# zoongahn/jodalroB-twoTower

Measured on AMD Instinct MI355X. Metric: training pairs/sec at batch 8192 (embedding-lookup HBM GB/s in roofline), higher is better.
Workload: dtype bf16 MFMA operands, f32 accumulate; f32 tables, master weights and activations (the tower input x, which the GEMMs round to bf16 anyway, is stored bf16)

## Files before the change

### include/twotower.h

```cpp
#ifndef TWOTOWER_H_
#define TWOTOWER_H_

#include <stddef.h>
#include <stdint.h>

#ifdef __cplusplus
extern "C" {
#endif

#define TT_ABI_VERSION 2

#define TT_OK 0
#define TT_ERR_INVALID_ARG (-1)
#define TT_ERR_HIP (-2)
#define TT_ERR_WORKSPACE (-3)
#define TT_ERR_UNSUPPORTED (-4)
#define TT_ERR_DEVICE (-5)

#define TT_F32 0
#define TT_BF16 1

#define TT_MAX_SIDES 4
#define TT_MAX_HIDDEN 8

typedef struct tt_ctx tt_ctx;
typedef void* tt_stream;

int tt_abi_version(void);
int tt_ctx_create(int device, tt_ctx** out);
int tt_ctx_destroy(tt_ctx* ctx);
const char* tt_last_error_string(void);
int tt_ctx_num_cus(const tt_ctx* ctx);
uint64_t tt_launch_count(void);

#define TT_OPT_DEFER_SLAB_REDUCE 1
#define TT_OPT_KEYED_PARTS 2
#define TT_OPT_SCORE_BWD_ROWS_MIN 3
#define TT_OPT_DEFER_RIDERS 4
#define TT_OPT_FP8_GRAD 5
#define TT_OPT_CHAINED 6
#define TT_OPT_LOOKUP_NT 7
#define TT_OPT_CHAIN_SPIN 8
#define TT_OPT_RETRIEVE_SPLITS 9
int tt_ctx_set_option(tt_ctx* ctx, int32_t option, int32_t value);
#define TT_DEVERR_CHAIN_TIMEOUT 1u
#define TT_DEVERR_ROW_RANGE 2u
int tt_ctx_check_device_errors(tt_ctx* ctx, tt_stream stream);
int tt_handover_retarget(tt_ctx* ctx, void* graph_exec, void* node);
int tt_handover_captured_node(tt_ctx* ctx, void** node);
int tt_flush_deferred(tt_ctx* ctx, tt_stream stream);
int tt_flush_deferred_slabs(tt_ctx* ctx, tt_stream stream);
int tt_deferred_pending(const tt_ctx* ctx);

typedef struct tt_embed_side {
  const int64_t* ids;
  const int64_t* key_row_offset;
  const int64_t* key_vocab;
  void* out;
  int64_t ld_out;
  int32_t K;
  int32_t out_dtype;
} tt_embed_side;

int tt_embed_lookup_set_profile(tt_ctx* ctx, uint64_t* ring_dev, int32_t n_slots);
int tt_embed_lookup_fwd(tt_ctx* ctx, const float* table, int64_t table_rows, int32_t E,
                        const tt_embed_side* sides, int32_t n_sides, int64_t B, int32_t* rows_out,
                        tt_stream stream);
int tt_embed_lookup_rows_fwd(tt_ctx* ctx, const float* table, int64_t table_rows, int32_t E,
                             const tt_embed_side* sides, int32_t n_sides, int64_t B, const int32_t* rows,
                             tt_stream stream);

size_t tt_dedup_workspace_bytes(int64_t M);
int tt_dedup_plan(tt_ctx* ctx, const int32_t* rows, int64_t M, int64_t table_rows,
                  int32_t* sorted_src, int32_t* unique_rows, int32_t* seg_offsets, int32_t* n_unique,
                  void* workspace, size_t workspace_bytes, tt_stream stream);

size_t tt_dedup_keyed_workspace_bytes(int64_t M, int32_t n_keys);
int tt_dedup_plan_keyed(tt_ctx* ctx, const int32_t* rows, const int32_t* side_K ,
                        int32_t n_sides, int64_t B, int32_t* sorted_src, int32_t* unique_rows,
                        int32_t* seg_offsets, int32_t* n_unique, void* workspace, size_t workspace_bytes,
                        tt_stream stream);

int tt_dedup_plan_keyed_km(tt_ctx* ctx, const int32_t* rows_km, const int32_t* side_K ,
                           int32_t n_sides, int64_t B, int32_t* sorted_src, int32_t* unique_rows,
                           int32_t* seg_offsets, int32_t* n_unique, void* workspace, size_t workspace_bytes,
                           tt_stream stream);

int tt_dedup_plan_keyed_long(tt_ctx* ctx, const int32_t* rows, int32_t rows_key_major, const int32_t* side_K ,
                             int32_t n_sides, int64_t B, int32_t E, int32_t* sorted_src, int32_t* unique_rows,
                             int32_t* seg_offsets, int32_t* n_unique, void* grad_workspace, size_t grad_workspace_bytes,
                             void* workspace, size_t workspace_bytes, tt_stream stream);

#define TT_GRAD_SPARSE 0
#define TT_GRAD_DENSE_SET 1
#define TT_GRAD_DENSE_ACC 2
#define TT_GRAD_SHORT_SEGMENTS 0x100
#define TT_GRAD_PLANNED 0x200
#define TT_GRAD_DEFER_FINISH 0x400

typedef struct tt_grad_src {
  const void* d_out;
  int64_t ld;
  int32_t K;
  int32_t dtype;
} tt_grad_src;

size_t tt_embed_grad_workspace_bytes(int64_t M, int32_t E);
int tt_embed_grad_bwd(tt_ctx* ctx, const tt_grad_src* srcs, int32_t n_srcs, int64_t B, int32_t E,
                      const int32_t* sorted_src, const int32_t* seg_offsets,
                      const int32_t* unique_rows, const int32_t* n_unique, int64_t M, int32_t mode,
                      float* out, int32_t* counters, void* workspace, size_t workspace_bytes, tt_stream stream);

void tt_adam_hparams(int64_t step, float lr, float beta1, float beta2, float eps, float weight_decay,
                     float out6[6]);
int tt_adam_dense_step(tt_ctx* ctx, float* p, const float* g, float* m, float* v, int64_t n,
                       int64_t step, float lr, float beta1, float beta2, float eps,
                       float weight_decay, const float* hparams_dev, tt_stream stream);
typedef struct tt_adam_tensor {
  float* p;
  const float* g;
  float* m;
  float* v;
  int64_t n;
} tt_adam_tensor;
int tt_adam_multi_step(tt_ctx* ctx, const tt_adam_tensor* tensors , int32_t n_tensors,
                       int64_t step, float lr, float beta1, float beta2, float eps,
                       float weight_decay, const float* hparams_dev, tt_stream stream);
int tt_sparse_adam_step(tt_ctx* ctx, float* table, float* m, float* v, int64_t table_rows, int32_t E,
                        const int32_t* unique_rows, const float* grad_rows, const int32_t* n_unique,
                        int64_t M, int64_t step, float lr, float beta1, float beta2, float eps,
                        float weight_decay, const float* hparams_dev, tt_stream stream);

int tt_adam_fused_step(tt_ctx* ctx, const tt_adam_tensor* tensors, int32_t n_tensors, float* table, float* m, float* v,
                       int64_t table_rows, int32_t E, const int32_t* unique_rows, const float* grad_rows, const int32_t* n_unique, int64_t M,
                       int64_t step, float lr, float beta1, float beta2, float eps, float weight_decay,
                       const float* hparams_dev, tt_stream stream);

int tt_adam_fused_step_finish(tt_ctx* ctx, const tt_adam_tensor* tensors, int32_t n_tensors, float* table, float* m, float* v,
                              int64_t table_rows, int32_t E, const int32_t* unique_rows, float* grad_rows, const int32_t* n_unique,
                              int64_t M, const int32_t* seg_offsets, void* grad_workspace, size_t grad_workspace_bytes,
                              int64_t step, float lr, float beta1, float beta2, float eps, float weight_decay,
                              const float* hparams_dev, tt_stream stream);

int tt_rowwise_adagrad_sparse_step(tt_ctx* ctx, float* table, float* sum, int64_t table_rows, int32_t E,
                                   const int32_t* unique_rows, const float* grad_rows, const int32_t* n_unique, int64_t M,
                                   float lr, float eps, float weight_decay, const float* hparams_dev, tt_stream stream);
int tt_rowwise_adagrad_dense_step(tt_ctx* ctx, float* table, float* sum, const float* grad, int64_t table_rows, int32_t E,
                                  float lr, float eps, float weight_decay, const float* hparams_dev, tt_stream stream);
int tt_adam_rowwise_adagrad_fused_step(tt_ctx* ctx, const tt_adam_tensor* tensors, int32_t n_tensors, int64_t step, float lr,
                                       float beta1, float beta2, float eps, float weight_decay, const float* hparams_dev,
                                       float* table, float* sum, int64_t table_rows, int32_t E, const int32_t* unique_rows,
                                       const float* grad_rows, const int32_t* n_unique, int64_t M, float table_lr,
                                       float table_eps, float table_weight_decay, const float* table_hparams_dev,
                                       tt_stream stream);
int tt_adam_rowwise_adagrad_fused_step_finish(tt_ctx* ctx, const tt_adam_tensor* tensors, int32_t n_tensors, int64_t step,
                                              float lr, float beta1, float beta2, float eps, float weight_decay,
                                              const float* hparams_dev, float* table, float* sum, int64_t table_rows, int32_t E,
                                              const int32_t* unique_rows, float* grad_rows, const int32_t* n_unique, int64_t M,
                                              const int32_t* seg_offsets, void* grad_workspace, size_t grad_workspace_bytes,
                                              float table_lr, float table_eps, float table_weight_decay,
                                              const float* table_hparams_dev, tt_stream stream);
int tt_embed_grad_finish(tt_ctx* ctx, int32_t E, const int32_t* seg_offsets, int64_t M, float* out, void* workspace,
                         size_t workspace_bytes, tt_stream stream);

typedef struct tt_tower_params {
  int32_t din, h0, kcat_e, n_hidden, d_out;
  int32_t hidden[TT_MAX_HIDDEN];
  const float* w_proj;
  const float* b_proj;
  const float* w[TT_MAX_HIDDEN];
  const float* b[TT_MAX_HIDDEN];
  const float* bn_w[TT_MAX_HIDDEN];
  const float* bn_b[TT_MAX_HIDDEN];
  float* bn_rm[TT_MAX_HIDDEN];
  float* bn_rv[TT_MAX_HIDDEN];
  int64_t* bn_nbt[TT_MAX_HIDDEN];
  const float* w_out;
  const float* b_out;
  int32_t compute_dtype;
  int32_t x_dtype;
  int32_t dx_dtype;
  int32_t flags;
  int32_t sync_phase;
  int32_t sync_ranks;
  int64_t rng_row_offset;
  const void* w_proj_bf16;
  const void* w_bf16[TT_MAX_HIDDEN];
} tt_tower_params;
#define TT_TOWER_UNFUSED_TAIL 1
#define TT_TOWER_UNFUSED_FRONT 2
#define TT_TOWER_UNFUSED_BACK 4

typedef struct tt_tower_acts {
  const float* dense;
  void* x;
  float* pre[TT_MAX_HIDDEN];
  float* act[TT_MAX_HIDDEN];
  float* mean[TT_MAX_HIDDEN];
  float* rstd[TT_MAX_HIDDEN];
  float* y;
  float* emb;
  void* emb_packed;
  float emb_pack_scale;
  float* bn_sync_local;
  const float* bn_sync_all;
  int64_t bn_sync_stride;
} tt_tower_acts;

typedef struct tt_tower_grads {
  float* w_proj;
  float* b_proj;
  float* w[TT_MAX_HIDDEN];
  float* b[TT_MAX_HIDDEN];
  float* bn_w[TT_MAX_HIDDEN];
  float* bn_b[TT_MAX_HIDDEN];
  float* w_out;
  float* b_out;
  void* d_x;
  float* scratch[TT_MAX_HIDDEN];
  float* d_y;
  float* s_sync_local;
  const float* s_sync_all;
  int64_t s_sync_stride;
} tt_tower_grads;

size_t tt_tower_workspace_bytes(const tt_tower_params* p, int64_t B);
int tt_tower_mlp_fwd(tt_ctx* ctx, const tt_tower_params* p, const tt_tower_acts* a, int64_t B,
                     int32_t train, float dropout_p, uint64_t seed, const uint64_t* seed_dev,
                     void* workspace, size_t workspace_bytes, tt_stream stream);
int tt_tower_mlp_bwd(tt_ctx* ctx, const tt_tower_params* p, const tt_tower_acts* a,
                     const float* d_emb, const tt_tower_grads* g, int64_t B, int32_t train,
                     float dropout_p, uint64_t seed, const uint64_t* seed_dev, void* workspace,
                     size_t workspace_bytes, tt_stream stream);

int tt_towers_mlp_fwd(tt_ctx* ctx, int32_t n, const tt_tower_params* const* p, const tt_tower_acts* const* a,
                      int64_t B, int32_t train, float dropout_p, uint64_t seed, const uint64_t* seed_dev,
                      void* const* workspaces, const size_t* workspace_bytes, tt_stream stream);
int tt_towers_mlp_bwd(tt_ctx* ctx, int32_t n, const tt_tower_params* const* p, const tt_tower_acts* const* a,
                      const float* const* d_emb, const tt_tower_grads* const* g, int64_t B, int32_t train,
                      float dropout_p, uint64_t seed, const uint64_t* seed_dev, void* const* workspaces,
                      const size_t* workspace_bytes, tt_stream stream);

int tt_score_dir_fwd(tt_ctx* ctx, const float* A, const float* Bm, int64_t Ra, int64_t Rb, int32_t D,
                     float inv_t, float shift, int64_t diag_offset, float* sumexp, float* diag,
                     int32_t* rank, float* sumscore ,
                     tt_stream stream);
int tt_score_loss_finish(tt_ctx* ctx, int64_t B, float shift, const float* rowsum,
                         const float* colsum, const float* diag, const int32_t* row_rank,
                         const int32_t* col_rank, const float* sumscore, float* out8,
                         float* loss_out , tt_stream stream);
int tt_score_dir_bwd(tt_ctx* ctx, const float* A, const float* Bm, int64_t Ra, int64_t Rb, int32_t D,
                     float inv_t, float shift, int64_t diag_offset, const float* sumexp_a,
                     const float* sumexp_b, const float* d_loss, float scale, float* dA,
                     tt_stream stream);
typedef struct tt_score_fwd_dir {
  const void* A_packed;
  const void* B_packed;
  int64_t Ra, Rb, diag_offset;
  float* sumexp;
  float* diag;
  int32_t* rank;
  float* sumscore;
  int32_t rank_mode;
  float ab_scale;
  float* inv_sumexp;
} tt_score_fwd_dir;
typedef struct tt_score_bwd_dir {
  const void* A_packed;
  const void* B_packed;
  int64_t Ra, Rb, diag_offset;
  const float* sumexp_a;
  const float* sumexp_b;
  float* dA;
  float ab_scale;
  float b_scale;
  const float* inv_a;
  const float* inv_b;
} tt_score_bwd_dir;
size_t tt_score_pack_bytes(int64_t R, int32_t D);
float tt_score_unit_scale(float inv_t);
int tt_score_pack_bf16(tt_ctx* ctx, const float* X, int64_t R, int32_t D, float scale, void* packed, tt_stream stream);
int tt_score_pack2_bf16(tt_ctx* ctx, const float* X0, int64_t R0, void* packed0, const float* X1, int64_t R1,
                        void* packed1, int32_t D, float scale0, float scale1, tt_stream stream);
int tt_score_fwd_bf16(tt_ctx* ctx, const tt_score_fwd_dir* dirs, int32_t n_dirs, int32_t D, float inv_t,
                      float shift, tt_stream stream);
int tt_score_bwd_bf16(tt_ctx* ctx, const tt_score_bwd_dir* dirs, int32_t n_dirs, int32_t D, float inv_t,
                      float shift, const float* d_loss, float scale, tt_stream stream);
size_t tt_score_fwd_sym_workspace_bytes(int64_t B, int32_t D);
int tt_score_fwd_sym_bf16(tt_ctx* ctx, const void* N_packed, const void* C_packed, int64_t B, int32_t D, float inv_t,
                          float shift, float ab_scale, int32_t want_rank, float* rowsum, float* colsum, float* inv_row,
                          float* inv_col, float* diag, int32_t* row_rank, float* out8, float* loss_out, void* workspace,
                          size_t workspace_bytes, tt_stream stream);
size_t tt_score_pack_fp8_bytes(int64_t R, int32_t D);
int tt_score_pack2_fp8(tt_ctx* ctx, const float* X0, int64_t R0, void* packed0, const float* X1, int64_t R1,
                       void* packed1, int32_t D, float scale0, float scale1, tt_stream stream);
// ... 118 lines not shown
```

### jodalrob-twotower_amd/_lib.py

```python
from __future__ import annotations

import ctypes as C
from pathlib import Path
from typing import Optional

import torch

_PKG = Path(__file__).resolve().parent
LIB_PATH = _PKG / "libtwotower_hip.so"

TT_F32, TT_BF16 = 0, 1
TT_MAX_SIDES, TT_MAX_HIDDEN = 4, 8
TT_GRAD_SPARSE, TT_GRAD_DENSE_SET, TT_GRAD_DENSE_ACC = 0, 1, 2
TT_TOWER_UNFUSED_TAIL = 1
TT_TOWER_UNFUSED_FRONT = 2
TT_TOWER_UNFUSED_BACK = 4
TT_GRAD_SHORT_SEGMENTS = 0x100
TT_GRAD_PLANNED = 0x200
TT_GRAD_DEFER_FINISH = 0x400

vp = C.c_void_p
i32, i64, f32, u64, sz = C.c_int32, C.c_int64, C.c_float, C.c_uint64, C.c_size_t


class EmbedSide(C.Structure):
    _fields_ = [("ids", vp), ("key_row_offset", vp), ("key_vocab", vp), ("out", vp), ("ld_out", i64),
                ("K", i32), ("out_dtype", i32)]


class StoreSide(C.Structure):
    _fields_ = [("entity", vp), ("entity_stride", i64), ("dense_store", vp), ("cat_store", vp), ("dense_out", vp), ("ids_out", vp),
                ("dense_dim", i32), ("n_rows", i32)]


TT_MAX_CVT = 8


class CvtList(C.Structure):
    _fields_ = [("n", i32), ("reserved", i32), ("src", vp * TT_MAX_CVT), ("dst", vp * TT_MAX_CVT), ("count", i64 * TT_MAX_CVT)]


class IngestLookup(C.Structure):
    _fields_ = [("table", vp), ("table_rows", i64), ("E", i32), ("reserved", i32)]


class GradSrc(C.Structure):
    _fields_ = [("d_out", vp), ("ld", i64), ("K", i32), ("dtype", i32)]


class AdamTensor(C.Structure):
    _fields_ = [("p", vp), ("g", vp), ("m", vp), ("v", vp), ("n", i64)]


class ScoreFwdDir(C.Structure):
    _fields_ = [("A_packed", vp), ("B_packed", vp), ("Ra", i64), ("Rb", i64), ("diag_offset", i64),
                ("sumexp", vp), ("diag", vp), ("rank", vp), ("sumscore", vp), ("rank_mode", i32), ("ab_scale", f32), ("inv_sumexp", vp)]


class ScoreBwdDir(C.Structure):
    _fields_ = [("A_packed", vp), ("B_packed", vp), ("Ra", i64), ("Rb", i64), ("diag_offset", i64),
                ("sumexp_a", vp), ("sumexp_b", vp), ("dA", vp), ("ab_scale", f32), ("b_scale", f32), ("inv_a", vp), ("inv_b", vp)]


_H = vp * TT_MAX_HIDDEN


class TowerParams(C.Structure):
    _fields_ = [("din", i32), ("h0", i32), ("kcat_e", i32), ("n_hidden", i32), ("d_out", i32),
                ("hidden", i32 * TT_MAX_HIDDEN),
                ("w_proj", vp), ("b_proj", vp), ("w", _H), ("b", _H), ("bn_w", _H), ("bn_b", _H),
                ("bn_rm", _H), ("bn_rv", _H), ("bn_nbt", _H), ("w_out", vp), ("b_out", vp), ("compute_dtype", i32),
                ("x_dtype", i32), ("dx_dtype", i32), ("flags", i32),
                ("sync_phase", i32), ("sync_ranks", i32), ("rng_row_offset", i64),
                ("w_proj_bf16", vp), ("w_bf16", _H)]


class TowerActs(C.Structure):
    _fields_ = [("dense", vp), ("x", vp), ("pre", _H), ("act", _H), ("mean", _H), ("rstd", _H), ("y", vp), ("emb", vp), ("emb_packed", vp), ("emb_pack_scale", f32),
                ("bn_sync_local", vp), ("bn_sync_all", vp), ("bn_sync_stride", i64)]


class TowerGrads(C.Structure):
    _fields_ = [("w_proj", vp), ("b_proj", vp), ("w", _H), ("b", _H), ("bn_w", _H), ("bn_b", _H),
                ("w_out", vp), ("b_out", vp), ("d_x", vp), ("scratch", _H), ("d_y", vp), ("s_sync_local", vp), ("s_sync_all", vp), ("s_sync_stride", i64)]


SIGNATURES = {
    "tt_abi_version": (C.c_int, []),
    "tt_ctx_create": (C.c_int, [C.c_int, C.POINTER(vp)]),
    "tt_ctx_destroy": (C.c_int, [vp]),
    "tt_last_error_string": (C.c_char_p, []),
    "tt_ctx_num_cus": (C.c_int, [vp]),
    "tt_embed_lookup_set_profile": (C.c_int, [vp, vp, i32]),
    "tt_embed_lookup_fwd": (C.c_int, [vp, vp, i64, i32, C.POINTER(EmbedSide), i32, i64, vp, vp]),
    "tt_embed_lookup_rows_fwd": (C.c_int, [vp, vp, i64, i32, C.POINTER(EmbedSide), i32, i64, vp, vp]),
    "tt_dedup_workspace_bytes": (sz, [i64]),
    "tt_dedup_plan": (C.c_int, [vp, vp, i64, i64, vp, vp, vp, vp, vp, sz, vp]),
    "tt_dedup_keyed_workspace_bytes": (sz, [i64, i32]),
    "tt_dedup_plan_keyed": (C.c_int, [vp, vp, C.POINTER(i32), i32, i64, vp, vp, vp, vp, vp, sz, vp]),
    "tt_dedup_plan_keyed_km": (C.c_int, [vp, vp, C.POINTER(i32), i32, i64, vp, vp, vp, vp, vp, sz, vp]),
    "tt_dedup_plan_keyed_long": (C.c_int, [vp, vp, i32, C.POINTER(i32), i32, i64, i32, vp, vp, vp, vp, vp, sz, vp, sz, vp]),
    "tt_embed_grad_workspace_bytes": (sz, [i64, i32]),
    "tt_embed_grad_bwd": (C.c_int, [vp, C.POINTER(GradSrc), i32, i64, i32, vp, vp, vp, vp, i64, i32, vp, vp, vp, sz, vp]),
    "tt_adam_hparams": (None, [i64, f32, f32, f32, f32, f32, C.POINTER(f32 * 6)]),
    "tt_adam_dense_step": (C.c_int, [vp, vp, vp, vp, vp, i64, i64, f32, f32, f32, f32, f32, vp, vp]),
    "tt_adam_multi_step": (C.c_int, [vp, C.POINTER(AdamTensor), i32, i64, f32, f32, f32, f32, f32, vp, vp]),
    "tt_sparse_adam_step": (C.c_int, [vp, vp, vp, vp, i64, i32, vp, vp, vp, i64, i64, f32, f32, f32, f32, f32, vp, vp]),
    "tt_adam_fused_step": (C.c_int, [vp, C.POINTER(AdamTensor), i32, vp, vp, vp, i64, i32, vp, vp, vp, i64, i64, f32, f32, f32, f32,
                                     f32, vp, vp]),
    "tt_adam_fused_step_finish": (C.c_int, [vp, C.POINTER(AdamTensor), i32, vp, vp, vp, i64, i32, vp, vp, vp, i64, vp, vp, sz, i64, f32,
                                            f32, f32, f32, f32, vp, vp]),
    "tt_rowwise_adagrad_sparse_step": (C.c_int, [vp, vp, vp, i64, i32, vp, vp, vp, i64, f32, f32, f32, vp, vp]),
    "tt_rowwise_adagrad_dense_step": (C.c_int, [vp, vp, vp, vp, i64, i32, f32, f32, f32, vp, vp]),
    "tt_adam_rowwise_adagrad_fused_step": (C.c_int, [vp, C.POINTER(AdamTensor), i32, i64, f32, f32, f32, f32, f32, vp, vp, vp, i64, i32,
                                                     vp, vp, vp, i64, f32, f32, f32, vp, vp]),
    "tt_adam_rowwise_adagrad_fused_step_finish": (C.c_int, [vp, C.POINTER(AdamTensor), i32, i64, f32, f32, f32, f32, f32, vp, vp, vp,
                                                            i64, i32, vp, vp, vp, i64, vp, vp, sz, f32, f32, f32, vp, vp]),
    "tt_embed_grad_finish": (C.c_int, [vp, i32, vp, i64, vp, vp, sz, vp]),
    "tt_ctx_set_option": (C.c_int, [vp, i32, i32]),
    "tt_flush_deferred": (C.c_int, [vp, vp]),
    "tt_ctx_check_device_errors": (C.c_int, [vp, vp]),
    "tt_handover_retarget": (C.c_int, [vp, vp, vp]),
    "tt_handover_captured_node": (C.c_int, [vp, C.POINTER(vp)]),
    "tt_deferred_pending": (C.c_int, [vp]),
    "tt_launch_count": (C.c_uint64, []),
    "tt_flush_deferred_slabs": (C.c_int, [vp, vp]),
    "tt_tower_workspace_bytes": (sz, [C.POINTER(TowerParams), i64]),
    "tt_tower_mlp_fwd": (C.c_int, [vp, C.POINTER(TowerParams), C.POINTER(TowerActs), i64, i32, f32, u64, vp, vp, sz, vp]),
    "tt_tower_mlp_bwd": (C.c_int, [vp, C.POINTER(TowerParams), C.POINTER(TowerActs), vp, C.POINTER(TowerGrads), i64, i32,
                                   f32, u64, vp, vp, sz, vp]),
    "tt_towers_mlp_fwd": (C.c_int, [vp, i32, C.POINTER(C.POINTER(TowerParams)), C.POINTER(C.POINTER(TowerActs)), i64, i32, f32, u64,
                                    vp, C.POINTER(vp), C.POINTER(sz), vp]),
    "tt_towers_mlp_bwd": (C.c_int, [vp, i32, C.POINTER(C.POINTER(TowerParams)), C.POINTER(C.POINTER(TowerActs)), C.POINTER(vp),
                                    C.POINTER(C.POINTER(TowerGrads)), i64, i32, f32, u64, vp, C.POINTER(vp), C.POINTER(sz), vp]),
    "tt_score_dir_fwd": (C.c_int, [vp, vp, vp, i64, i64, i32, f32, f32, i64, vp, vp, vp, vp, vp]),
    "tt_score_loss_finish": (C.c_int, [vp, i64, f32, vp, vp, vp, vp, vp, vp, vp, vp, vp]),
    "tt_score_dir_bwd": (C.c_int, [vp, vp, vp, i64, i64, i32, f32, f32, i64, vp, vp, vp, f32, vp, vp]),
    "tt_score_pack_bytes": (sz, [i64, i32]),
    "tt_score_unit_scale": (f32, [f32]),
    "tt_score_pack_bf16": (C.c_int, [vp, vp, i64, i32, f32, vp, vp]),
    "tt_score_pack2_bf16": (C.c_int, [vp, vp, i64, vp, vp, i64, vp, i32, f32, f32, vp]),
    "tt_score_fwd_bf16": (C.c_int, [vp, C.POINTER(ScoreFwdDir), i32, i32, f32, f32, vp]),
    "tt_score_bwd_bf16": (C.c_int, [vp, C.POINTER(ScoreBwdDir), i32, i32, f32, f32, vp, f32, vp]),
    "tt_score_pack_fp8_bytes": (sz, [i64, i32]),
    "tt_score_pack2_fp8": (C.c_int, [vp, vp, i64, vp, vp, i64, vp, i32, f32, f32, vp]),
    "tt_score_fwd_sym_fp8": (C.c_int, [vp, vp, vp, i64, i32, f32, f32, f32, i32, vp, vp, vp, vp, vp, vp, vp, vp, vp, sz, vp]),
    "tt_score_bwd_fp8": (C.c_int, [vp, C.POINTER(ScoreBwdDir), i32, i32, f32, f32, vp, f32, vp]),
    "tt_score_fwd_sym_workspace_bytes": (sz, [i64, i32]),
    "tt_score_fwd_sym_bf16": (C.c_int, [vp, vp, vp, i64, i32, f32, f32, f32, i32, vp, vp, vp, vp, vp, vp, vp, vp, vp, sz, vp]),
    "tt_score_pack_x3_bytes": (sz, [i64, i32]),
    "tt_score_pack2_bf16x3": (C.c_int, [vp, vp, i64, vp, vp, i64, vp, i32, f32, f32, vp]),
    "tt_score_fwd_sym_bf16x3": (C.c_int, [vp, vp, vp, i64, i32, f32, f32, f32, i32, vp, vp, vp, vp, vp, vp, vp, vp, vp, sz, vp]),
    "tt_score_fwd_bf16x3": (C.c_int, [vp, C.POINTER(ScoreFwdDir), i32, i32, f32, f32, vp]),
    "tt_score_bwd_bf16x3": (C.c_int, [vp, C.POINTER(ScoreBwdDir), i32, i32, f32, f32, vp, f32, vp]),
    "tt_score_matrix": (C.c_int, [vp, vp, vp, i64, i64, i32, f32, vp, i64, vp]),
    "tt_score_dense_workspace_bytes": (sz, [i64, i32]),
    "tt_score_dense_fwd": (C.c_int, [vp, vp, vp, i64, i32, f32, i32, f32, vp, vp, vp, vp, vp, vp]),
    "tt_score_dense_bwd": (C.c_int, [vp, vp, vp, i64, i32, f32, i32, f32, vp, vp, vp, vp, vp, vp, sz, vp]),
    "tt_diag_rank_rows": (C.c_int, [vp, vp, i64, i64, i64, i64, vp, vp]),
    "tt_topk_rows": (C.c_int, [vp, vp, i64, i64, i64, i32, vp, vp, vp]),
    "tt_retrieve_workspace_bytes": (sz, [i64, i64, i32, i32]),
    "tt_retrieve_topk_bf16": (C.c_int, [vp, vp, i64, vp, i64, i32, i32, vp, i32, vp, vp, vp, vp, sz, vp]),
    "tt_retrieve_topk_f32": (C.c_int, [vp, vp, i64, vp, i64, i32, f32, i32, vp, i32, vp, vp, vp, vp, sz, vp]),
    "tt_linear_fwd": (C.c_int, [vp, vp, i64, vp, vp, vp, i64, i64, i32, i32, i32, vp]),
    "tt_route_workspace_bytes": (sz, [i64, i32]),
    "tt_route_bucket": (C.c_int, [vp, vp, vp, i64, i32, i32, C.POINTER(i32), i32, vp, vp, vp, vp, vp, vp, sz, vp]),
    "tt_route_expand": (C.c_int, [vp, vp, vp, vp, vp, i64, vp, vp]),
    "tt_route_bucket_expand": (C.c_int, [vp, vp, vp, i64, i32, i32, C.POINTER(i32), i32, vp, vp, vp, vp, vp, vp, sz, vp, vp, vp, vp]),
    "tt_dedup_plan_runs": (C.c_int, [vp, vp, i32, i64, i64, vp, vp, vp, vp, vp, sz, vp]),
    "tt_gather_rows": (C.c_int, [vp, vp, i64, i32, vp, i64, vp, i32, vp]),
    "tt_copy_multi": (C.c_int, [vp, i32, C.POINTER(vp), C.POINTER(vp), C.POINTER(i64), vp]),
    "tt_batch_ingest": (C.c_int, [vp, i32, C.POINTER(vp), C.POINTER(vp), C.POINTER(i64), C.POINTER(EmbedSide), i32, i64, vp, vp, i64, C.POINTER(CvtList), vp]),
    "tt_batch_gather": (C.c_int, [vp, vp, i64, vp, i32, vp, i32, vp, vp, vp]),
    "tt_batch_ingest_store": (C.c_int, [vp, i32, C.POINTER(vp), C.POINTER(vp), C.POINTER(i64), C.POINTER(EmbedSide), C.POINTER(StoreSide), i32,
                                        i64, vp, vp, vp, i64, C.POINTER(CvtList), vp]),
    "tt_batch_ingest_lookup": (C.c_int, [vp, i32, C.POINTER(vp), C.POINTER(vp), C.POINTER(i64), C.POINTER(EmbedSide), i32, i64, vp,
                                         C.POINTER(IngestLookup), C.POINTER(CvtList), vp]),
    "tt_batch_ingest_store_lookup": (C.c_int, [vp, i32, C.POINTER(vp), C.POINTER(vp), C.POINTER(i64), C.POINTER(EmbedSide), C.POINTER(StoreSide),
                                               i32, i64, vp, vp, C.POINTER(IngestLookup), C.POINTER(CvtList), vp]),
}

_lib: Optional[C.CDLL] = None
_ctxs: dict = {}
_defer_on: set = set()
_riders_on: dict = {}
_workspaces: dict = {}


class TwoTowerHipError(RuntimeError):
    pass


def load() -> C.CDLL:
    global _lib
    if _lib is None:
        if not LIB_PATH.exists():
            raise TwoTowerHipError(
                f"{LIB_PATH} is missing: build it with `python -c 'import __graft_entry__ as g; g.build()'` "
                "(hipcc --offload-arch=gfx950).  There is no CPU fallback for the two-tower hot path.")
        lib = C.CDLL(str(LIB_PATH))
        for name, (res, args) in SIGNATURES.items():
            fn = getattr(lib, name)
            fn.restype, fn.argtypes = res, args
        _lib = lib
    return _lib


def check(rc: int, what: str = ""):
    if rc != 0:
        msg = load().tt_last_error_string().decode("utf-8", "replace")
        raise TwoTowerHipError(f"{what or 'twotower call'} failed (status {rc}): {msg}")


def ctx(device: torch.device) -> vp:
    device = torch.device(device)
    if device.type != "cuda":
        raise TwoTowerHipError(f"the two-tower hot path runs on MI355X only; got tensors on '{device}' "
                               "(no CPU fallback exists)")
    idx = device.index if device.index is not None else torch.cuda.current_device()
    if idx not in _ctxs:
        h = vp()
        check(load().tt_ctx_create(idx, C.byref(h)), "tt_ctx_create")
        _ctxs[idx] = h
    return _ctxs[idx]


def stream(device: torch.device) -> vp:
    return vp(torch.cuda.current_stream(device).cuda_stream)


def ptr(t: Optional[torch.Tensor]) -> vp:
    return vp(0 if t is None else t.data_ptr())


TT_OPT_DEFER_SLAB_REDUCE = 1
TT_OPT_KEYED_PARTS = 2
TT_OPT_SCORE_BWD_ROWS_MIN = 3
TT_OPT_DEFER_RIDERS = 4
TT_OPT_FP8_GRAD = 5
TT_OPT_CHAINED = 6
TT_OPT_LOOKUP_NT = 7
TT_OPT_CHAIN_SPIN = 8
TT_OPT_RETRIEVE_SPLITS = 9


def set_option(device: torch.device, option: int, value: int):
    check(load().tt_ctx_set_option(ctx(device), int(option), int(value)), "tt_ctx_set_option")


def set_defer_slab_reduce(device: torch.device, on: bool):
    check(load().tt_ctx_set_option(ctx(device), TT_OPT_DEFER_SLAB_REDUCE, 1 if on else 0), "tt_ctx_set_option")
    idx = torch.device(device).index
    (_defer_on.add if on else _defer_on.discard)(idx if idx is not None else torch.cuda.current_device())
    if not on:
        flush_deferred(device)


def set_defer_riders(device: torch.device, on, loss_only: bool = False):
    mask = (2 if loss_only else 3) if on else 0
    check(load().tt_ctx_set_option(ctx(device), TT_OPT_DEFER_RIDERS, mask), "tt_ctx_set_option")
    idx = torch.device(device).index
    idx = idx if idx is not None else torch.cuda.current_device()
    if mask:
        _riders_on[idx] = mask
    else:
        _riders_on.pop(idx, None)
        flush_deferred(device)


def riders_deferred(device: torch.device, which: int = 3) -> bool:
    idx = torch.device(device).index
    return bool(_riders_on.get(idx if idx is not None else torch.cuda.current_device(), 0) & which)


def check_device_errors(device: torch.device):
    device = torch.device(device)
    idx = device.index if device.index is not None else (torch.cuda.current_device() if device.type == "cuda" else None)
    if device.type != "cuda" or idx not in _ctxs:
        return
    check(load().tt_ctx_check_device_errors(_ctxs[idx], stream(device)), "tt_ctx_check_device_errors")


def handover_captured_node(device: torch.device) -> Optional[int]:
    h = vp()
    check(load().tt_handover_captured_node(ctx(device), C.byref(h)), "tt_handover_captured_node")
    return h.value


class handover_retarget:

    def __init__(self, device: torch.device, graph_exec: int, node: int):
        self.device, self.exec, self.node = device, graph_exec, node

    def __enter__(self):
        check(load().tt_handover_retarget(ctx(self.device), vp(self.exec), vp(self.node)), "tt_handover_retarget")
        return self

    def __exit__(self, *exc):
        check(load().tt_handover_retarget(ctx(self.device), vp(0), vp(0)), "tt_handover_retarget")
        return False


def flush_deferred(device: torch.device):
    lib = load()
    c = ctx(device)
    if lib.tt_deferred_pending(c):
        check(lib.tt_flush_deferred(c, stream(device)), "tt_flush_deferred")


def workspace(device: torch.device, nbytes: int) -> torch.Tensor:
    if _defer_on:
        lib, c = load(), ctx(device)
        if lib.tt_deferred_pending(c) & 1:
            check(lib.tt_flush_deferred_slabs(c, stream(device)), "tt_flush_deferred_slabs")
    key = (torch.device(device).index, torch.cuda.current_stream(device).cuda_stream)
    buf = _workspaces.get(key)
    if buf is None or buf.numel() < nbytes:
        buf = torch.empty(max(int(nbytes), 1 << 20), dtype=torch.uint8, device=device)
        _workspaces[key] = buf
    return buf


def num_cus(device: torch.device) -> int:
    return int(load().tt_ctx_num_cus(ctx(device)))


def no_dynamo(fn):
    try:
        import torch._dynamo as _d
        return _d.disable(fn)
    except Exception:
        return fn
```

### jodalrob-twotower_amd/cat_embed.py

```python
from __future__ import annotations

from pathlib import Path
from typing import Dict, List, Optional, Union

import torch
from ._lib import no_dynamo as _no_dynamo
import torch.nn as nn

from . import ops
from .config import settings
from .schema import category_counts


class EmbeddingStore:

    def __init__(self, E: int, device, grad_mode: str = "dense"):
        if grad_mode not in ("dense", "sparse"):
            raise ValueError(f"embedding_grad must be 'dense' or 'sparse', got {grad_mode!r}")
        self.E = E
        self.device = torch.device(device)
        self.grad_mode = grad_mode
        self.weight: Optional[torch.Tensor] = None
        self.grad: Optional[torch.Tensor] = None
        self.sparse_grad = None
        self.defer_long_finish = False
        self.members: List["CategoricalEmbedder"] = []
        self.version = 0
        self._grad_counters = None
        self.ingest = None
        self.ingest_x_fresh = False

    def rows_km_for(self, id_tensors) -> Optional[torch.Tensor]:
        reg = self.ingest
        if reg is None or len(reg[0]) != len(id_tensors):
            return None
        for t, r, v in zip(id_tensors, reg[0], reg[1]):
            if t.data_ptr() != r.data_ptr() or t.numel() != r.numel() or r._version != v:
                return None
        return reg[2]

    def rows_sm_for(self, id_tensors) -> Optional[torch.Tensor]:
        reg = self.ingest
        if reg is None or len(reg) < 5 or reg[4] is None or self.rows_km_for(id_tensors) is None:
            return None
        return reg[4]

    def x_for(self, id_tensors, shapes) -> Optional[list]:
        reg = self.ingest
        if reg is None or len(reg) < 4 or reg[3] is None or not self.ingest_x_fresh or self.rows_km_for(id_tensors) is None:
            return None
        xs = reg[3]
        if len(xs) != len(shapes) or any(tuple(x.shape) != (b, w) or x.dtype != dt for x, (b, w, dt) in zip(xs, shapes)):
            return None
        self.ingest_x_fresh = False
        return xs

    def grad_counters(self) -> Optional[torch.Tensor]:
        if self._grad_counters is None or self._grad_counters.device != self.device:
            if self.device.type != "cuda" or torch.cuda.is_current_stream_capturing():
                return None
            self._grad_counters = torch.zeros(4, dtype=torch.int32, device=self.device)
        return self._grad_counters

    @property
    def rows(self) -> int:
        return 0 if self.weight is None else self.weight.shape[0]

    def append_rows(self, n: int) -> int:
        new = torch.empty((n, self.E), dtype=torch.float32, device=self.device)
        nn.init.normal_(new)
        base = self.rows
        self.weight = new if self.weight is None else torch.cat([self.weight, new])
        self.grad, self.sparse_grad = None, None
        self.version += 1
        return base

    def apply(self, fn):
        new = fn(self.weight)
        if new is not self.weight:
            if new.dtype != torch.float32:
                raise TypeError("embedding tables are kept in float32")
            self.weight = new
            self.device = new.device
            self.grad = None if self.grad is None else fn(self.grad)
            self.sparse_grad = None
            self.version += 1

    @staticmethod
    def fuse(stores: List["EmbeddingStore"]) -> "EmbeddingStore":
        uniq = []
        for s in stores:
            if all(s is not u for u in uniq):
                uniq.append(s)
        if len(uniq) == 1:
            return uniq[0]
        first = uniq[0]
        if any(s.E != first.E for s in uniq):
            raise ValueError("cannot fuse embedding stores of different embedding_dim")
        fused = EmbeddingStore(first.E, first.device, first.grad_mode)
        fused.weight = torch.cat([s.weight.to(first.device) for s in uniq])
        base = 0
        for s in uniq:
            for m in s.members:
                m._rebind(fused, m.row_base + base)
            base += s.rows
        return fused

    def optim_parameters(self):
        return [p for m in self.members for p in m.table_parameters()]

    def bind_grads(self):
        for m in self.members:
            m._bind_grads()

    def accumulate_grad(self, plan: ops.DedupPlan, srcs, B: int, short_segments: bool = False):
        if self.grad_mode == "sparse":
            grad_rows = torch.empty((max(plan.M, 1), self.E), dtype=torch.float32, device=self.device)
            ops.embed_grad(plan, srcs, B, self.E, ops.TT_GRAD_SPARSE, grad_rows, short_segments, self.grad_counters(),
                           defer_finish=self.defer_long_finish)
            self.sparse_grad = (plan, grad_rows)
            return
        params = self.optim_parameters()
        fresh = any(p.grad is None for p in params) or self.grad is None
        if self.grad is None:
            self.grad = torch.empty_like(self.weight)
        if fresh:
            self.grad.zero_()
            ops.embed_grad(plan, srcs, B, self.E, ops.TT_GRAD_DENSE_SET, self.grad, counters=self.grad_counters())
            self.bind_grads()
        else:
            ops.embed_grad(plan, srcs, B, self.E, ops.TT_GRAD_DENSE_ACC, self.grad, counters=self.grad_counters())


class _Table(nn.Module):

    def __init__(self, view: torch.Tensor):
        super().__init__()
        self.weight = nn.Parameter(view)

    @property
    def num_embeddings(self):
        return self.weight.shape[0]

    @property
    def embedding_dim(self):
        return self.weight.shape[1]


class CategoricalEmbedder(nn.Module):
    def __init__(self, keys: List[str], metadata_path: Union[str, Path], table_name: str, embedding_dim: int = 64,
                 device: Optional[str] = "cuda:0", safety_margin: int = 10, embedding_grad: Optional[str] = None,
                 materialize: bool = True):
        super().__init__()
        self.keys = list(keys)
        self.materialize = materialize
        self.embedding_dim = embedding_dim
        self.device_str = str(device or "cuda:0")
        self.safety_margin = safety_margin
        self.vocab_sizes = self._extract_vocab_sizes(metadata_path, table_name, self.keys)
        print(f"[CategoricalEmbedder] Initializing with {len(self.keys)} features")
        mode = embedding_grad or settings.embedding_grad
        self.store = EmbeddingStore(embedding_dim, torch.device(self.device_str), mode)
        self.embeddings = nn.ModuleDict()
        offs = []
        if materialize:
            self.row_base = self.store.append_rows(sum(self.vocab_sizes[k] for k in self.keys)) if self.keys else 0
            self.store.members.append(self)
            off = self.row_base
            for k in self.keys:
                v = self.vocab_sizes[k]
                self.embeddings[k] = _Table(self.store.weight[off:off + v])
                offs.append(off)
                off += v
        else:
            self.row_base, off = 0, 0
            for k in self.keys:
                offs.append(off)
                off += self.vocab_sizes[k]
        dev = self.store.device
        self.register_buffer("_key_row_offset", torch.tensor(offs, dtype=torch.int64, device=dev), persistent=False)
        self.register_buffer("_key_vocab", torch.tensor([self.vocab_sizes[k] for k in self.keys], dtype=torch.int64,
                                                        device=dev), persistent=False)
        self._bound_version = self.store.version

    def _extract_vocab_sizes(self, metadata_path, table_name: str, keys: List[str]) -> Dict[str, int]:
        try:
            counts = category_counts(table_name, metadata_path)
        except Exception as e:
            print(f"[ERROR] Failed to extract vocab_sizes from metadata: {e}")
            print("[FALLBACK] Using default vocab_size=1000 for all keys")
            return {k: 1000 for k in keys}
        out = {}
        for k in keys:
            if k not in counts:
                print(f"[WARNING] Column '{k}' not found in metadata, using default vocab_size=1000")
                out[k] = 1000
            elif counts[k] is None:
                print(f"[WARNING] No category count info for '{k}', using default vocab_size=1000")
                out[k] = 1000
            else:
                out[k] = int(counts[k]) + self.safety_margin
        return out

    def table_parameters(self):
        return [self.embeddings[k].weight for k in self.keys] if self.materialize else []

    @property
    def total_rows(self) -> int:
        return sum(self.vocab_sizes[k] for k in self.keys)

    def set_row_base(self, base: int):
        off, offs = base, []
        for k in self.keys:
            offs.append(off)
            off += self.vocab_sizes[k]
        self.row_base = base
        self._key_row_offset = torch.tensor(offs, dtype=torch.int64, device=self._key_row_offset.device)

    def _rebind(self, store: Optional[EmbeddingStore] = None, row_base: Optional[int] = None):
        if store is not None and store is not self.store:
            self.store = store
            if self not in store.members:
                store.members.append(self)
        if row_base is not None:
            self.row_base = row_base
        off = self.row_base
        offs = []
        for k in self.keys:
            v = self.vocab_sizes[k]
            self.embeddings[k].weight.data = self.store.weight[off:off + v]
            self.embeddings[k].weight.grad = None
            offs.append(off)
            off += v
        dev = self.store.device
        self._key_row_offset = torch.tensor(offs, dtype=torch.int64, device=dev)
        self._key_vocab = self._key_vocab.to(dev)
        self._bound_version = self.store.version
        if self.store.grad is not None:
            self._bind_grads()

    def _bind_grads(self):
        off = self.row_base
        for k in self.keys:
            v = self.vocab_sizes[k]
            self.embeddings[k].weight.grad = self.store.grad[off:off + v]
            off += v

    def _apply(self, fn, recurse=True):
        if not self.materialize:
            dev = fn(torch.empty(0, device=self._key_vocab.device)).device
            self._key_row_offset, self._key_vocab = self._key_row_offset.to(dev), self._key_vocab.to(dev)
            self.store.device = dev
            return self
        self.store.apply(fn)
        for s_member in self.store.members:
            if s_member._bound_version != s_member.store.version:
                s_member._rebind()
        self._key_row_offset = self._key_row_offset.to(self.store.device)
        self._key_vocab = self._key_vocab.to(self.store.device)
        return self

    def load_state_dict(self, state_dict, strict: bool = True, assign: bool = False):
        return super().load_state_dict(state_dict, strict=strict, assign=False)

    def lookup_side(self, values: torch.Tensor, out_view: torch.Tensor) -> ops.LookupSide:
        return ops.LookupSide(values, self._key_row_offset, self._key_vocab, out_view, len(self.keys))

    @_no_dynamo
    def forward(self, kjt, return_dict: bool = True):
        K, E = len(self.keys), self.embedding_dim
        if kjt is None:
            dev = self.store.device
# ... 39 lines not shown
```

### jodalrob-twotower_amd/csrc/tt_common.h

```cpp
#pragma once
#include <hip/hip_runtime.h>
#include <stdint.h>
#include <stdio.h>
#include <stdarg.h>
#include <atomic>

#include "twotower.h"

struct tt_ctx {
  int device;
  int num_cus;
  size_t lds_per_block;
  unsigned long long* lookup_stamps;
  int lookup_stamp_slots;
  int defer_slab_reduce;
  struct TnPending* deferred;
  int keyed_parts;
  int score_bwd_rows_min;
  int defer_riders;
  int fp8_grad;
  struct tt_riders* riders;
  uint32_t* chain;
  int chain_words;
  void* chain_stream[16];
  int chain_used;
  int chained;
  uint32_t* dev_err;
  int chain_spin;
  int retrieve_splits;
  int lookup_nt;
  void* ho_exec;
  void* ho_node;
  void* ho_last;
};

constexpr uint32_t kChainReady = 0x80000000u;
constexpr int kChainWords = 1 << 16, kChainSlices = 16;
uint32_t* tt_chain_for(tt_ctx* ctx, hipStream_t stream);

void tt_set_error(const char* fmt, ...);

#define TT_CHECK_ARG(cond, ...)         \
  do {                                  \
    if (!(cond)) {                      \
      tt_set_error(__VA_ARGS__);        \
      return TT_ERR_INVALID_ARG;        \
    }                                   \
  } while (0)

#define TT_HIP(expr)                                                                   \
  do {                                                                                 \
    hipError_t _e = (expr);                                                            \
    if (_e != hipSuccess) {                                                            \
      tt_set_error("%s failed: %s (%s:%d)", #expr, hipGetErrorString(_e), __FILE__, __LINE__); \
      return TT_ERR_HIP;                                                               \
    }                                                                                  \
  } while (0)

extern std::atomic<uint64_t> tt_launches;
#define TT_LAUNCH_CHECK()                                    \
  do {                                                       \
    tt_launches.fetch_add(1, std::memory_order_relaxed);     \
    TT_HIP(hipGetLastError());                               \
  } while (0)

#define TT_LDS_ONCE(bytes, ...)                                                                                     \
  do {                                                                                                              \
    static std::atomic<uint64_t> tt_lds_done{0};                                                                    \
    const uint64_t tt_bit = 1ull << (ctx->device & 63);                                                             \
    if (!(tt_lds_done.load(std::memory_order_acquire) & tt_bit)) {                                                  \
      TT_HIP(hipFuncSetAttribute(reinterpret_cast<const void*>(__VA_ARGS__), hipFuncAttributeMaxDynamicSharedMemorySize, (int)(bytes))); \
      tt_lds_done.fetch_or(tt_bit, std::memory_order_release);                                                      \
    }                                                                                                               \
  } while (0)

static inline int64_t tt_cdiv(int64_t a, int64_t b) { return (a + b - 1) / b; }
static inline bool tt_aligned(const void* p, size_t a) { return (reinterpret_cast<uintptr_t>(p) % a) == 0; }

__device__ __forceinline__ uint16_t tt_f2bf(float x) {
  __bf16 b = static_cast<__bf16>(x);
  return __builtin_bit_cast(uint16_t, b);
}
__device__ __forceinline__ float tt_bf2f(uint16_t h) {
  return __builtin_bit_cast(float, static_cast<uint32_t>(h) << 16);
}

__device__ __forceinline__ uint32_t tt_mix32(uint32_t x) {
  x ^= x >> 16;
  x *= 0x7feb352dU;
  x ^= x >> 15;
  x *= 0x846ca68bU;
  x ^= x >> 16;
  return x;
}
__device__ __forceinline__ float tt_uniform01(uint64_t seed, uint64_t idx) {
  const uint32_t lo = static_cast<uint32_t>(idx), hi = static_cast<uint32_t>(idx >> 32);
  const uint32_t h = tt_mix32(lo ^ static_cast<uint32_t>(seed) ^ ((hi ^ static_cast<uint32_t>(seed >> 32)) * 0x9E3779B9U));
  return static_cast<float>(h >> 8) * (1.0f / 16777216.0f);
}
```

### jodalrob-twotower_amd/csrc/tt_ctx.hip

```cpp
#include "tt_common.h"
#include "tt_gemm.h"
#include "tt_riders.h"

#include <mutex>

#include <string.h>

static thread_local char g_err[512] = "";
std::atomic<uint64_t> tt_launches{0};

namespace {
__global__ __launch_bounds__(kRiderThreads) void riders_kernel(tt_riders r) {
  if ((int)blockIdx.x < r.c_wg) compact_body(r.c, blockIdx.x);
  else finish2_body(r.f);
}
}

uint32_t* tt_chain_for(tt_ctx* ctx, hipStream_t stream) {
  static std::mutex mu;
  if (!ctx || !ctx->chained || !ctx->chain) return nullptr;
  std::lock_guard<std::mutex> lock(mu);
  for (int i = 0; i < ctx->chain_used; ++i)
    if (ctx->chain_stream[i] == static_cast<void*>(stream)) return ctx->chain + (size_t)i * kChainWords;
  if (ctx->chain_used == kChainSlices) return nullptr;
  ctx->chain_stream[ctx->chain_used] = static_cast<void*>(stream);
  return ctx->chain + (size_t)(ctx->chain_used++) * kChainWords;
}

int tt_riders_flush(tt_ctx* ctx, hipStream_t st) {
  if (!ctx || !ctx->riders || (ctx->riders->c_wg == 0 && ctx->riders->f_wg == 0)) return TT_OK;
  riders_kernel<<<ctx->riders->c_wg + ctx->riders->f_wg, kRiderThreads, 0, st>>>(*ctx->riders);
  ctx->riders->c_wg = ctx->riders->f_wg = 0;
  TT_LAUNCH_CHECK();
  return TT_OK;
}

void tt_set_error(const char* fmt, ...) {
  va_list ap;
  va_start(ap, fmt);
  vsnprintf(g_err, sizeof(g_err), fmt, ap);
  va_end(ap);
}

extern "C" {

int tt_abi_version(void) { return TT_ABI_VERSION; }

const char* tt_last_error_string(void) { return g_err; }

int tt_ctx_create(int device, tt_ctx** out) {
  TT_CHECK_ARG(out != nullptr, "tt_ctx_create: out is NULL");
  int n = 0;
  TT_HIP(hipGetDeviceCount(&n));
  TT_CHECK_ARG(device >= 0 && device < n, "tt_ctx_create: device %d out of range (%d devices)", device, n);
  hipDeviceProp_t prop;
  TT_HIP(hipGetDeviceProperties(&prop, device));
  if (strncmp(prop.gcnArchName, "gfx950", 6) != 0) {
    tt_set_error("tt_ctx_create: device %d is %s; this library is built for gfx950 (MI355X) only", device,
                 prop.gcnArchName);
    return TT_ERR_UNSUPPORTED;
  }
  tt_ctx* c = new tt_ctx();
  c->device = device;
  c->num_cus = prop.multiProcessorCount;
  c->lds_per_block = prop.sharedMemPerBlock;
  c->lookup_stamps = nullptr;
  c->lookup_stamp_slots = 0;
  c->defer_slab_reduce = 0;
  c->deferred = nullptr;
  c->keyed_parts = 0;
  c->score_bwd_rows_min = 32768;
  c->defer_riders = 0;
  c->fp8_grad = 1;
  c->riders = new tt_riders();
  c->riders->c_wg = c->riders->f_wg = 0;
  c->chain = nullptr;
  c->chain_words = 0;
  c->chain_used = 0;
  c->chained = 1;
  c->chain_spin = 1 << 22;
  c->retrieve_splits = 0;
  c->dev_err = nullptr;
  c->ho_exec = c->ho_node = c->ho_last = nullptr;
  {
    int prev = 0;
    TT_HIP(hipGetDevice(&prev));
    TT_HIP(hipSetDevice(device));
    hipError_t e = hipMalloc(reinterpret_cast<void**>(&c->chain), sizeof(uint32_t) * (kChainWords * kChainSlices + 64));
    if (e == hipSuccess) e = hipMemset(c->chain, 0, sizeof(uint32_t) * (kChainWords * kChainSlices + 64));
    if (e == hipSuccess) c->dev_err = c->chain + (size_t)kChainWords * kChainSlices;
    (void)hipSetDevice(prev);
    if (e != hipSuccess) {
      tt_set_error("tt_ctx_create: %s", hipGetErrorString(e));
      delete c->riders;
      delete c;
      return TT_ERR_HIP;
    }
    c->chain_words = kChainWords;
  }
  *out = c;
  return TT_OK;
}

int tt_ctx_destroy(tt_ctx* ctx) {
  if (ctx && ctx->deferred) tt_gemm_tn_pending_destroy(ctx->deferred);
  if (ctx) delete ctx->riders;
  if (ctx && ctx->chain) (void)hipFree(ctx->chain);
  delete ctx;
  return TT_OK;
}

int tt_ctx_set_option(tt_ctx* ctx, int32_t option, int32_t value) {
  TT_CHECK_ARG(ctx != nullptr, "tt_ctx_set_option: NULL context");
  switch (option) {
    case TT_OPT_DEFER_SLAB_REDUCE: ctx->defer_slab_reduce = value != 0; break;
    case TT_OPT_KEYED_PARTS:
      TT_CHECK_ARG(value >= 0, "tt_ctx_set_option: TT_OPT_KEYED_PARTS needs a value >= 0");
      ctx->keyed_parts = value;
      break;
    case TT_OPT_SCORE_BWD_ROWS_MIN:
      TT_CHECK_ARG(value >= 1, "tt_ctx_set_option: TT_OPT_SCORE_BWD_ROWS_MIN needs a value >= 1");
      ctx->score_bwd_rows_min = value;
      break;
    case TT_OPT_DEFER_RIDERS:
      TT_CHECK_ARG(value >= 0 && value <= 3, "tt_ctx_set_option: TT_OPT_DEFER_RIDERS takes 0 .. 3");
      ctx->defer_riders = value == 1 ? 3 : value;
      break;
    case TT_OPT_FP8_GRAD: ctx->fp8_grad = value != 0; break;
    case TT_OPT_CHAINED: ctx->chained = value != 0; break;
    case TT_OPT_LOOKUP_NT: ctx->lookup_nt = value != 0; break;
    case TT_OPT_CHAIN_SPIN:
      TT_CHECK_ARG(value >= 1, "tt_ctx_set_option: TT_OPT_CHAIN_SPIN needs a value >= 1");
      ctx->chain_spin = value;
      break;
    case TT_OPT_RETRIEVE_SPLITS:
      TT_CHECK_ARG(value >= 0, "tt_ctx_set_option: TT_OPT_RETRIEVE_SPLITS needs a value >= 0");
      ctx->retrieve_splits = value;
      break;
    default: tt_set_error("tt_ctx_set_option: unknown option %d", option); return TT_ERR_INVALID_ARG;
  }
  return TT_OK;
}

int tt_ctx_check_device_errors(tt_ctx* ctx, tt_stream stream) {
  TT_CHECK_ARG(ctx != nullptr, "tt_ctx_check_device_errors: NULL context");
  if (!ctx->dev_err) return TT_OK;
  hipStream_t st = reinterpret_cast<hipStream_t>(stream);
  uint32_t word = 0;
  TT_HIP(hipMemcpyAsync(&word, ctx->dev_err, sizeof(word), hipMemcpyDeviceToHost, st));
  TT_HIP(hipStreamSynchronize(st));
  if (word == 0) return TT_OK;
  TT_HIP(hipMemsetAsync(ctx->chain, 0, sizeof(uint32_t) * ((size_t)kChainWords * kChainSlices + 64), st));
  TT_HIP(hipStreamSynchronize(st));
  tt_set_error("device error word 0x%x:%s%s the steps since the last check are invalid (they must be rejected)", word,
               (word & TT_DEVERR_CHAIN_TIMEOUT) ? " a chained segment-head launch gave up waiting for a predecessor tile (tt_dedup_plan / tt_dedup_plan_runs);" : "",
               (word & TT_DEVERR_ROW_RANGE) ? " a lookup decoded rows outside its table (key offsets / vocabularies that belong to another table; tt_embed_lookup_fwd / "
                                              "tt_embed_lookup_rows_fwd / tt_batch_ingest_lookup) and read the last row instead;" : "");
  return TT_ERR_DEVICE;
}

int tt_handover_retarget(tt_ctx* ctx, void* graph_exec, void* node) {
  TT_CHECK_ARG(ctx != nullptr && ((graph_exec == nullptr) == (node == nullptr)), "tt_handover_retarget: NULL context / one of (graph_exec, node) NULL");
  ctx->ho_exec = graph_exec;
  ctx->ho_node = node;
  return TT_OK;
}

int tt_handover_captured_node(tt_ctx* ctx, void** node) {
  TT_CHECK_ARG(ctx != nullptr && node != nullptr, "tt_handover_captured_node: NULL argument");
  *node = ctx->ho_last;
  ctx->ho_last = nullptr;
  return TT_OK;
}

int tt_flush_deferred(tt_ctx* ctx, tt_stream stream) {
  TT_CHECK_ARG(ctx != nullptr, "tt_flush_deferred: NULL context");
  if (int rc = tt_riders_flush(ctx, reinterpret_cast<hipStream_t>(stream))) return rc;
  return tt_gemm_deferred_flush(ctx, reinterpret_cast<hipStream_t>(stream));
}

int tt_flush_deferred_slabs(tt_ctx* ctx, tt_stream stream) {
  TT_CHECK_ARG(ctx != nullptr, "tt_flush_deferred_slabs: NULL context");
  return tt_gemm_deferred_flush(ctx, reinterpret_cast<hipStream_t>(stream));
}

int tt_deferred_pending(const tt_ctx* ctx) {
  if (!ctx) return 0;
  return ((ctx->deferred && ctx->deferred->n > 0) ? 1 : 0) | ((ctx->riders && (ctx->riders->c_wg > 0 || ctx->riders->f_wg > 0)) ? 2 : 0);
}

int tt_ctx_num_cus(const tt_ctx* ctx) { return ctx ? ctx->num_cus : 0; }

uint64_t tt_launch_count(void) { return tt_launches.load(std::memory_order_relaxed); }

}
```

### jodalrob-twotower_amd/csrc/tt_embed.hip

```cpp
#include "tt_common.h"
#include "tt_gemm.h"
#include "tt_riders.h"

#include <stdlib.h>
#include <type_traits>

namespace {

constexpr int kThreads = 256;

struct SideDev {
  const int64_t* ids;
  const int64_t* off;
  const int64_t* vocab;
  char* out;
  int64_t ld;
  uint32_t slot_base;
  int32_t K;
  int32_t dtype;
  uint32_t magic;
};

struct SideSet {
  SideDev s[TT_MAX_SIDES];
// ... 670 lines not shown
    __syncthreads();
    for (int d = tid; d < 16 * 256; d += kKeyedThreads) (&peers_mask[0][0])[d] = 0ull;
    __syncthreads();
  }
  if (!sorted_by_buckets) {
    e_lo = 0;
    e_hi = part == 0 ? B : 0;
    if (part != 0) {
      if (tid == 0) { ucount[blockIdx.x] = 0; ubase[blockIdx.x] = ki * B; uend[blockIdx.x] = ki * B; }
      return;
    }
  }
  for (int p = 0; p < (sorted_by_buckets ? 0 : passes); ++p) {
    const int shift = dbits * p;
    for (int d = tid; d < 16 * 256; d += kKeyedThreads) (&whist[0][0])[d] = 0;
    uint32_t kreg[NB];
    uint16_t vreg[NB];
#pragma unroll
    for (int q = 0; q < NB; ++q) {
      const int i = wlo + q * 64 + lane;
      kreg[q] = i < whi ? keys[cur][i] : 0u;
      vreg[q] = i < whi ? vals[cur][i] : (uint16_t)0;
    }
    uint64_t peers[NB];
#pragma unroll
    for (int q = 0; q < NB; ++q) {
      const bool valid = wlo + q * 64 + lane < whi;
      const uint32_t d = ((kreg[q] - lo) >> shift) & dmask;
      if (valid) __hip_atomic_fetch_or(const_cast<unsigned long long*>(&pm[wave][d]), 1ull << lane, __ATOMIC_RELAXED, __HIP_MEMORY_SCOPE_WAVEFRONT);
      __builtin_amdgcn_wave_barrier();
      peers[q] = valid ? pm[wave][d] : 0ull;
      __builtin_amdgcn_wave_barrier();
      if (valid) pm[wave][d] = 0ull;
      __builtin_amdgcn_wave_barrier();
    }
    __syncthreads();
#pragma unroll
    for (int q = 0; q < NB; ++q) {
      const uint32_t d = ((kreg[q] - lo) >> shift) & dmask;
      const bool leader = peers[q] != 0ull && (peers[q] & lt_mask) == 0ull;
      if (leader) atomicAdd(&whist[wave][d], (uint32_t)__popcll(peers[q]));
    }
    __syncthreads();
    {
      const int d = tid >> 2, w0 = (tid & 3) * 4;
      uint32_t c4[4], tot = 0;
#pragma unroll
      for (int j = 0; j < 4; ++j) { c4[j] = whist[w0 + j][d]; tot += c4[j]; }
      uint32_t x = tot;
#pragma unroll
      for (int o = 1; o < 64; o <<= 1) {
        const uint32_t y = __shfl_up(x, o);
        if (lane >= o) x += y;
      }
      if (lane == 63) red[wave] = x;
      __syncthreads();
      uint32_t run = x - tot;
      for (int w = 0; w < wave; ++w) run += red[w];
#pragma unroll
      for (int j = 0; j < 4; ++j) { whist[w0 + j][d] = run; run += c4[j]; }
    }
    __syncthreads();
    uint32_t base[NB];
#pragma unroll
    for (int q = 0; q < NB; ++q) {
      const uint32_t d = ((kreg[q] - lo) >> shift) & dmask;
      const bool leader = peers[q] != 0ull && (peers[q] & lt_mask) == 0ull;
      base[q] = 0;
      if (leader) base[q] = atomicAdd(const_cast<uint32_t*>(&wh[wave][d]), (uint32_t)__popcll(peers[q]));
    }
#pragma unroll
    for (int q = 0; q < NB; ++q) {
      const bool valid = peers[q] != 0ull;
      const int leader_lane = valid ? (int)__builtin_ctzll(peers[q]) : lane;
      const uint32_t b0 = (uint32_t)__builtin_amdgcn_ds_bpermute(leader_lane << 2, (int)base[q]);
      if (valid) {
        const uint32_t pos = b0 + (uint32_t)__popcll(peers[q] & lt_mask);
        keys[cur ^ 1][pos] = kreg[q];
        vals[cur ^ 1][pos] = vreg[q];
      }
    }
    __syncthreads();
    cur ^= 1;
  }
  const int64_t gbase = (int64_t)ki * B;
  constexpr int PER = kKeyedB / kKeyedThreads;
  const int i_lo = e_lo + tid * PER;
  uint32_t flags = 0, c = 0;
#pragma unroll
  for (int j = 0; j < PER; ++j) {
    const int i = i_lo + j;
    if (i < e_hi) {
      sorted_src[gbase + i] = sbase + (int)vals[cur][i] * K + k;
      if (i == e_lo || keys[cur][i] != keys[cur][i - 1]) { flags |= 1u << j; ++c; }
    }
  }
  uint32_t x = c;
#pragma unroll
  for (int o = 1; o < 64; o <<= 1) {
    const uint32_t y = __shfl_up(x, o);
    if (lane >= o) x += y;
  }
  __syncthreads();
  if (lane == 63) red[wave] = x;
  __syncthreads();
  uint32_t u = x - c;
  for (int w = 0; w < wave; ++w) u += red[w];
#pragma unroll
  for (int j = 0; j < PER; ++j) {
    if (flags & (1u << j)) {
      uniq_stage[gbase + e_lo + u] = (int32_t)keys[cur][i_lo + j];
      seg_stage[gbase + e_lo + u] = (int32_t)(gbase + i_lo + j);
      ++u;
    }
  }
  if (tid == kKeyedThreads - 1) {
    ucount[blockIdx.x] = (int32_t)u;
    ubase[blockIdx.x] = (int32_t)(gbase + e_lo);
    uend[blockIdx.x] = (int32_t)(gbase + e_hi);
  }
}

__global__ __launch_bounds__(kKeyedThreads) void keyed_compact_kernel(CompactRider cr) { compact_body(cr, blockIdx.x); }

constexpr int kLongSeg = 64;
static_assert(kPlanLongSeg == kLongSeg, "the plan's compaction and the reduction must cut long rows into the same chunks");

struct GradWs {
  int32_t* counters;
  int32_t* long_row;
  int32_t* long_base;
  int32_t* chunk_lo;
  int32_t* chunk_hi;
  float* chunk_partial;
};

__global__ void zero_words_kernel(int32_t* __restrict__ p, int n) {
  if ((int)threadIdx.x < n) p[threadIdx.x] = 0;
}
__global__ void zero_two_words_kernel(int32_t* __restrict__ a, int32_t* __restrict__ b) {
  if (threadIdx.x == 0) a[0] = 0;
  if (threadIdx.x == 1) b[0] = 0;
}

template <int VEC>
struct Acc {
  float v[VEC];
  __device__ __forceinline__ void zero() {
#pragma unroll
    for (int i = 0; i < VEC; ++i) v[i] = 0.f;
  }
};

template <int VEC, int ESZ>
__device__ __forceinline__ const char* grad_addr(const SideSet& a, uint32_t slot, uint32_t chunk) {
  const char* base = a.s[0].out;
  int64_t ld = a.s[0].ld;
  uint32_t sb = 0, K = (uint32_t)a.s[0].K, magic = a.s[0].magic;
#pragma unroll
  for (int i = 1; i < TT_MAX_SIDES; ++i) {
    const bool sel = i < a.n && slot >= a.s[i].slot_base;
    base = sel ? a.s[i].out : base;
    ld = sel ? a.s[i].ld : ld;
    sb = sel ? a.s[i].slot_base : sb;
    K = sel ? (uint32_t)a.s[i].K : K;
    magic = sel ? a.s[i].magic : magic;
  }
  const uint32_t local = slot - sb;
  uint32_t b = __umulhi(local, magic);
  uint32_t k = local - b * K;
  if (k >= K) { k -= K; ++b; }
  return base + ((int64_t)b * ld + (int64_t)(k * (uint32_t)a.E + chunk * VEC)) * ESZ;
}

template <int VEC, int DT>
__device__ __forceinline__ void load_grad_chunk(const SideSet& a, uint32_t slot, uint32_t chunk, float* o) {
  if (DT == TT_F32) {
    const float* p = reinterpret_cast<const float*>(grad_addr<VEC, 4>(a, slot, chunk));
    if (VEC == 4) {
      const float4 t = *reinterpret_cast<const float4*>(p);
      o[0] = t.x; o[1 % VEC] = t.y; o[2 % VEC] = t.z; o[3 % VEC] = t.w;
    } else {
      o[0] = p[0];
    }
  } else {
    const uint16_t* p = reinterpret_cast<const uint16_t*>(grad_addr<VEC, 2>(a, slot, chunk));
    if (VEC == 4) {
      const ushort4 t = *reinterpret_cast<const ushort4*>(p);
      o[0] = tt_bf2f(t.x); o[1 % VEC] = tt_bf2f(t.y); o[2 % VEC] = tt_bf2f(t.z); o[3 % VEC] = tt_bf2f(t.w);
    } else {
      o[0] = tt_bf2f(p[0]);
    }
  }
}

constexpr int kBatch = 16;
#define TT_GLOBAL __attribute__((address_space(1)))
using tt_u32x4 = __attribute__((ext_vector_type(4))) uint32_t;
using tt_u32x2 = __attribute__((ext_vector_type(2))) uint32_t;

__device__ __forceinline__ uint64_t shfl_u64(uint64_t v, int src, int width) {
  const uint32_t lo = __shfl((uint32_t)v, src, width), hi = __shfl((uint32_t)(v >> 32), src, width);
  return ((uint64_t)hi << 32) | lo;
}

template <int VEC, int DT, int LGT>
__device__ __forceinline__ void sum_range(const SideSet& a, const int32_t* __restrict__ sorted_src, int32_t lo, int32_t hi,
                                          uint32_t chunk, uint32_t lig, Acc<VEC>& acc) {
  constexpr int ESZ = DT == TT_F32 ? 4 : 2;
  if (LGT > 0) {
    constexpr int PER = LGT > 0 ? kBatch / (LGT > 0 ? LGT : 1) : 1;
    int32_t idx[PER];
#pragma unroll
    for (int p = 0; p < PER; ++p) {
      const int32_t s = lo + p * LGT + (int32_t)lig;
      idx[p] = s < hi ? sorted_src[s] : 0;
    }
    for (int32_t i = lo; i < hi; i += kBatch) {
      const int32_t n = hi - i;
      uint64_t mine[PER];
#pragma unroll
      for (int p = 0; p < PER; ++p) mine[p] = reinterpret_cast<uint64_t>(grad_addr<VEC, ESZ>(a, (uint32_t)idx[p], 0));
#pragma unroll
      for (int p = 0; p < PER; ++p) {
        const int32_t s = i + kBatch + p * LGT + (int32_t)lig;
        idx[p] = s < hi ? sorted_src[s] : 0;
      }
      constexpr int RW = VEC * ESZ >= 4 ? VEC * ESZ / 4 : 1;
      uint32_t raw[kBatch][RW];
#pragma unroll
      for (int j = 0; j < kBatch; ++j) {
        const uint64_t ptr = shfl_u64(mine[j / LGT], j % LGT, LGT) + (uint64_t)chunk * VEC * ESZ;
        if (j < n) {
          if (RW == 4) {
            const tt_u32x4 q = *reinterpret_cast<const TT_GLOBAL tt_u32x4*>(ptr);
            raw[j][0] = q.x; raw[j][1 % RW] = q.y; raw[j][2 % RW] = q.z; raw[j][3 % RW] = q.w;
          } else if (RW == 2) {
            const tt_u32x2 q = *reinterpret_cast<const TT_GLOBAL tt_u32x2*>(ptr);
            raw[j][0] = q.x; raw[j][1 % RW] = q.y;
          } else if (ESZ == 4) {
            raw[j][0] = *reinterpret_cast<const TT_GLOBAL uint32_t*>(ptr);
          } else {
            raw[j][0] = *reinterpret_cast<const TT_GLOBAL uint16_t*>(ptr);
          }
        } else {
#pragma unroll
          for (int e = 0; e < RW; ++e) raw[j][e] = 0u;
        }
      }
#pragma unroll
      for (int j = 0; j < kBatch; ++j)
        if (j < n) {
#pragma unroll
          for (int e = 0; e < VEC; ++e) {
            float f;
            if (DT == TT_F32) f = __uint_as_float(raw[j][e % RW]);
            else f = __uint_as_float((e & 1) ? (raw[j][(e / 2) % RW] & 0xffff0000u) : (raw[j][(e / 2) % RW] << 16));
            acc.v[e] += f;
          }
        }
    }
    return;
  }
  int32_t i = lo;
  if (i + kBatch <= hi) {
    int32_t idx[kBatch];
#pragma unroll
    for (int j = 0; j < kBatch; ++j) idx[j] = sorted_src[i + j];
    for (; i + kBatch <= hi; i += kBatch) {
      float t[kBatch][VEC];
#pragma unroll
      for (int j = 0; j < kBatch; ++j) load_grad_chunk<VEC, DT>(a, (uint32_t)idx[j], chunk, t[j]);
      if (i + 2 * kBatch <= hi) {
#pragma unroll
        for (int j = 0; j < kBatch; ++j) idx[j] = sorted_src[i + kBatch + j];
      }
#pragma unroll
      for (int j = 0; j < kBatch; ++j)
#pragma unroll
        for (int e = 0; e < VEC; ++e) acc.v[e] += t[j][e];
    }
  }
  for (; i + 4 <= hi; i += 4) {
    float t[4][VEC];
#pragma unroll
    for (int j = 0; j < 4; ++j) load_grad_chunk<VEC, DT>(a, (uint32_t)sorted_src[i + j], chunk, t[j]);
#pragma unroll
    for (int j = 0; j < 4; ++j)
#pragma unroll
      for (int e = 0; e < VEC; ++e) acc.v[e] += t[j][e];
  }
  for (; i < hi; ++i) {
    float t[VEC];
    load_grad_chunk<VEC, DT>(a, (uint32_t)sorted_src[i], chunk, t);
#pragma unroll
    for (int e = 0; e < VEC; ++e) acc.v[e] += t[e];
  }
}

template <int VEC>
__device__ __forceinline__ void write_row(float* __restrict__ out, int64_t row, int32_t E, uint32_t chunk, const Acc<VEC>& acc,
                                          bool accumulate) {
  float* p = out + row * E + chunk * VEC;
  if (VEC == 4) {
    float4 t = make_float4(acc.v[0], acc.v[1 % VEC], acc.v[2 % VEC], acc.v[3 % VEC]);
    if (accumulate) {
      const float4 q = *reinterpret_cast<float4*>(p);
      t.x += q.x; t.y += q.y; t.z += q.z; t.w += q.w;
    }
    *reinterpret_cast<float4*>(p) = t;
  } else {
    p[0] = accumulate ? p[0] + acc.v[0] : acc.v[0];
  }
}

template <int VEC, int DT, int LGT>
__device__ __forceinline__ void seg_reduce_body(const SideSet& a, const int32_t* __restrict__ sorted_src,
                                                const int32_t* __restrict__ seg, const int32_t* __restrict__ unique_rows,
                                                const int32_t* __restrict__ n_unique, int32_t mode,
                                                float* __restrict__ out, const GradWs& ws, uint32_t LG, bool all_short, bool planned,
                                                uint32_t bid, uint32_t nblocks) {
  const uint32_t U = (uint32_t)*n_unique;
  const uint32_t gthread = bid * blockDim.x + threadIdx.x;
  const uint32_t lig = gthread % LG;
  const uint32_t ngroups = nblocks * blockDim.x / LG;
  for (uint32_t u = gthread / LG; u < U; u += ngroups) {
    const int32_t s0 = seg[u], s1 = seg[u + 1];
    if (planned && s1 - s0 > kLongSeg) continue;
    if (!all_short && s1 - s0 > kLongSeg) {
      const int32_t nch = (s1 - s0 + kLongSeg - 1) / kLongSeg;
      int32_t base = 0;
      if (lig == 0) {
        base = atomicAdd(&ws.counters[0], nch);
        const int32_t li = atomicAdd(&ws.counters[1], 1);
        ws.long_row[li] = (int32_t)u;
        ws.long_base[li] = base;
      }
      base = __shfl(base, 0, (int)LG);
      for (int32_t c = (int32_t)lig; c < nch; c += (int32_t)LG) {
        ws.chunk_lo[base + c] = s0 + c * kLongSeg;
        ws.chunk_hi[base + c] = min(s1, s0 + (c + 1) * kLongSeg);
      }
      continue;
    }
    const int64_t orow = mode == TT_GRAD_SPARSE ? (int64_t)u : (int64_t)unique_rows[u];
    for (uint32_t chunk = lig; chunk < a.C; chunk += LG) {
      Acc<VEC> acc;
      acc.zero();
      sum_range<VEC, DT, LGT>(a, sorted_src, s0, s1, chunk, lig, acc);
      write_row<VEC>(out, orow, a.E, chunk, acc, mode == TT_GRAD_DENSE_ACC);
    }
  }
}

template <int VEC, int DT, int LGT>
__global__ __launch_bounds__(kThreads) void seg_reduce_kernel(SideSet a, const int32_t* __restrict__ sorted_src,
                                                             const int32_t* __restrict__ seg, const int32_t* __restrict__ unique_rows,
                                                             const int32_t* __restrict__ n_unique, int32_t mode,
                                                             float* __restrict__ out, GradWs ws, uint32_t LG, bool all_short) {
  seg_reduce_body<VEC, DT, LGT>(a, sorted_src, seg, unique_rows, n_unique, mode, out, ws, LG, all_short, false, blockIdx.x, gridDim.x);
}

template <int VEC, int DT, int LGT>
__device__ __forceinline__ void seg_chunk_body(const SideSet& a, const int32_t* __restrict__ sorted_src, const GradWs& ws, uint32_t LG,
                                               uint32_t bid, uint32_t nblocks) {
  const uint32_t nchunks = (uint32_t)ws.counters[0];
  if (bid == 0 && threadIdx.x == 0) ws.counters[2] = ws.counters[1];
  const uint32_t gthread = bid * blockDim.x + threadIdx.x;
  const uint32_t lig = gthread % LG;
  const uint32_t ngroups = nblocks * blockDim.x / LG;
  for (uint32_t c = gthread / LG; c < nchunks; c += ngroups) {
    for (uint32_t chunk = lig; chunk < a.C; chunk += LG) {
      Acc<VEC> acc;
      acc.zero();
      sum_range<VEC, DT, LGT>(a, sorted_src, ws.chunk_lo[c], ws.chunk_hi[c], chunk, lig, acc);
      write_row<VEC>(ws.chunk_partial, (int64_t)c, a.E, chunk, acc, false);
    }
  }
}

template <int VEC, int DT, int LGT>
__global__ __launch_bounds__(kThreads) void seg_chunk_kernel(SideSet a, const int32_t* __restrict__ sorted_src, GradWs ws, uint32_t LG) {
  seg_chunk_body<VEC, DT, LGT>(a, sorted_src, ws, LG, blockIdx.x, gridDim.x);
}

template <int VEC, int DT, int LGT>
__global__ __launch_bounds__(kThreads) void seg_reduce_chunk_kernel(SideSet a, const int32_t* __restrict__ sorted_src,
                                                                   const int32_t* __restrict__ seg, const int32_t* __restrict__ unique_rows,
                                                                   const int32_t* __restrict__ n_unique, int32_t mode,
                                                                   float* __restrict__ out, GradWs ws, uint32_t LG, uint32_t g1) {
  if (blockIdx.x < g1) seg_reduce_body<VEC, DT, LGT>(a, sorted_src, seg, unique_rows, n_unique, mode, out, ws, LG, false, true, blockIdx.x, g1);
  else seg_chunk_body<VEC, DT, LGT>(a, sorted_src, ws, LG, blockIdx.x - g1, gridDim.x - g1);
}

#ifdef TT_SEG_STAMPS
__device__ unsigned long long g_seg_stamps[4096 * 4];
#define TT_SEG_STAMP(i, role) do { __builtin_amdgcn_s_waitcnt(0); __syncthreads(); if (threadIdx.x == 0 && blockIdx.x < 4096) { \
  g_seg_stamps[blockIdx.x * 4 + (i)] = __builtin_amdgcn_s_memrealtime(); g_seg_stamps[blockIdx.x * 4 + 2] = (role) + 1; } } while (0)
#else
#define TT_SEG_STAMP(i, role) do { } while (0)
#endif

constexpr uint32_t kChunkFirst = 8;
#ifndef TT_SEG_THREADS
#define TT_SEG_THREADS 256
#endif
constexpr int kSegThreads = TT_SEG_THREADS;
#ifdef TT_SEG_WAVES
#define TT_SEG_OCC __attribute__((amdgpu_waves_per_eu(1, TT_SEG_WAVES)))
#else
#define TT_SEG_OCC
#endif
template <int VEC, int DT, int LGT>
__global__ __launch_bounds__(kSegThreads) TT_SEG_OCC void seg_reduce_chunk_slab_kernel(SideSet a, const int32_t* __restrict__ sorted_src,
                                                                        const int32_t* __restrict__ seg, const int32_t* __restrict__ unique_rows,
                                                                        const int32_t* __restrict__ n_unique, int32_t mode,
                                                                        float* __restrict__ out, GradWs ws, uint32_t LG, uint32_t g1,
                                                                        SlabBatch sb, uint32_t nsx, uint32_t n_items, uint32_t ns) {
  const uint32_t g2 = gridDim.x - g1 - ns;
  const uint32_t gc = g2 < kChunkFirst ? g2 : kChunkFirst;
#ifndef TT_SEG_LAYOUT
#define TT_SEG_LAYOUT 4
#endif
  const uint32_t r1 = TT_SEG_LAYOUT == 2 ? (g1 + 1) / 2 : (TT_SEG_LAYOUT == 3 ? g1 : 0u);
  uint32_t b = blockIdx.x;
  if (b < gc) {
    TT_SEG_STAMP(0, 2);
    seg_chunk_body<VEC, DT, LGT>(a, sorted_src, ws, LG, b, g2);
    TT_SEG_STAMP(1, 2);
    return;
  }
  b -= gc;
  if (b < r1) {
    TT_SEG_STAMP(0, 1);
    seg_reduce_body<VEC, DT, LGT>(a, sorted_src, seg, unique_rows, n_unique, mode, out, ws, LG, false, true, b, g1);
    TT_SEG_STAMP(1, 1);
    return;
  }
  b -= r1;
  if (b < ns) {
    TT_SEG_STAMP(0, 0);
    int item, bx;
    if (slab_role_locate(sb, (int)n_items, (int)nsx, (int)b, item, bx)) slab_reduce_block(sb, bx, (int)nsx, item);
    TT_SEG_STAMP(1, 0);
    return;
  }
  b -= ns;
  if (b < g1 - r1) {
    TT_SEG_STAMP(0, 1);
    seg_reduce_body<VEC, DT, LGT>(a, sorted_src, seg, unique_rows, n_unique, mode, out, ws, LG, false, true, r1 + b, g1);
    TT_SEG_STAMP(1, 1);
    return;
  }
  b -= g1 - r1;
  TT_SEG_STAMP(0, 2);
  seg_chunk_body<VEC, DT, LGT>(a, sorted_src, ws, LG, gc + b, g2);
  TT_SEG_STAMP(1, 2);
}

constexpr int kFinishMaxFloats = 4096;
struct NoRowDone {
  __device__ void operator()(int32_t) const {}
};
template <int VEC, typename EMIT, typename DONE = NoRowDone>
__device__ __forceinline__ void long_rows_finish(int32_t E, uint32_t C, const int32_t* __restrict__ seg, const GradWs& ws, uint32_t LG,
                                                 uint32_t bid, uint32_t nblocks, float* __restrict__ part, EMIT&& emit,
                                                 DONE&& done = DONE{}) {
  const uint32_t nlong = (uint32_t)ws.counters[2];
  const uint32_t grp = threadIdx.x / LG, lig = threadIdx.x % LG, ngrp = blockDim.x / LG;
  for (uint32_t li = bid; li < nlong; li += nblocks) {
    const int32_t u = ws.long_row[li], base = ws.long_base[li];
    const int32_t nch = (seg[u + 1] - seg[u] + kLongSeg - 1) / kLongSeg;
    const int32_t per = (nch + (int32_t)ngrp - 1) / (int32_t)ngrp;
    const int32_t c0 = min(nch, (int32_t)grp * per), c1 = min(nch, c0 + per);
    for (uint32_t chunk = lig; chunk < C; chunk += LG) {
      Acc<VEC> acc;
      acc.zero();
      const float* p0 = ws.chunk_partial + (int64_t)base * E + chunk * VEC;
      int32_t c = c0;
      for (; c + 8 <= c1; c += 8) {
        float t[8][VEC];
#pragma unroll
        for (int j = 0; j < 8; ++j)
#pragma unroll
          for (int e = 0; e < VEC; ++e) t[j][e] = p0[(int64_t)(c + j) * E + e];
#pragma unroll
        for (int j = 0; j < 8; ++j)
#pragma unroll
          for (int e = 0; e < VEC; ++e) acc.v[e] += t[j][e];
      }
      for (; c < c1; ++c) {
#pragma unroll
        for (int e = 0; e < VEC; ++e) acc.v[e] += p0[(int64_t)c * E + e];
      }
#pragma unroll
      for (int e = 0; e < VEC; ++e) part[grp * E + chunk * VEC + e] = acc.v[e];
    }
    __syncthreads();
    for (int32_t col = threadIdx.x; col < E; col += blockDim.x) {
      float tot = 0.f;
      for (uint32_t g = 0; g < ngrp; ++g) tot += part[g * E + col];
      emit(u, col, tot);
    }
    __syncthreads();
    done(u);
  }
}

template <int VEC>
__global__ __launch_bounds__(kThreads) void seg_long_finish_kernel(int32_t E, uint32_t C, const int32_t* __restrict__ seg,
                                                                  const int32_t* __restrict__ unique_rows, int32_t mode,
                                                                  float* __restrict__ out, GradWs ws, uint32_t LG) {
  __shared__ float part[kFinishMaxFloats];
  if (blockIdx.x == 0 && threadIdx.x == 0) { ws.counters[0] = 0; ws.counters[1] = 0; }
  long_rows_finish<VEC>(E, C, seg, ws, LG, blockIdx.x, gridDim.x, part, [&](int32_t u, int32_t col, float tot) {
    const int64_t orow = mode == TT_GRAD_SPARSE ? (int64_t)u : (int64_t)unique_rows[u];
    float* o = out + orow * E + col;
    *o = mode == TT_GRAD_DENSE_ACC ? *o + tot : tot;
  });
}

struct AdamK {
  float lr_over_bc1, inv_sqrt_bc2, b1, b2, eps, wd;
  const float* dev;
};

__device__ __forceinline__ AdamK adam_resolve(const AdamK& k) {
  if (k.dev == nullptr) return k;
  AdamK r;
  r.lr_over_bc1 = k.dev[0]; r.inv_sqrt_bc2 = k.dev[1]; r.b1 = k.dev[2]; r.b2 = k.dev[3]; r.eps = k.dev[4]; r.wd = k.dev[5];
  r.dev = nullptr;
  return r;
}

__device__ __forceinline__ void adam1(float& p, float g, float& m, float& v, const AdamK& k) {
  g = k.wd != 0.f ? __builtin_fmaf(k.wd, p, g) : g;
  m = __builtin_fmaf(k.b1, m, (1.f - k.b1) * g);
  v = __builtin_fmaf(k.b2, v, (1.f - k.b2) * g * g);
  const float denom = __builtin_fmaf(sqrtf(v), k.inv_sqrt_bc2, k.eps);
  p = __builtin_fmaf(-k.lr_over_bc1, m / denom, p);
}

__global__ __launch_bounds__(kThreads) void adam_dense_kernel(float* __restrict__ p, const float* __restrict__ g,
                                                             float* __restrict__ m, float* __restrict__ v, int64_t n, AdamK k0) {
  const AdamK k = adam_resolve(k0);
  const int64_t stride = (int64_t)gridDim.x * blockDim.x;
  for (int64_t i = (int64_t)blockIdx.x * blockDim.x + threadIdx.x; i < n; i += stride) {
    float pp = p[i], mm = m[i], vv = v[i];
    adam1(pp, g[i], mm, vv, k);
    p[i] = pp; m[i] = mm; v[i] = vv;
  }
}

__global__ __launch_bounds__(kThreads) void adam_dense_vec4_kernel(float4* __restrict__ p, const float4* __restrict__ g,
                                                                  float4* __restrict__ m, float4* __restrict__ v, int64_t n4, AdamK k0) {
  const AdamK k = adam_resolve(k0);
  const int64_t stride = (int64_t)gridDim.x * blockDim.x;
  for (int64_t i = (int64_t)blockIdx.x * blockDim.x + threadIdx.x; i < n4; i += stride) {
    float4 pp = p[i], mm = m[i], vv = v[i];
    const float4 gg = g[i];
    adam1(pp.x, gg.x, mm.x, vv.x, k); adam1(pp.y, gg.y, mm.y, vv.y, k);
    adam1(pp.z, gg.z, mm.z, vv.z, k); adam1(pp.w, gg.w, mm.w, vv.w, k);
    p[i] = pp; m[i] = mm; v[i] = vv;
  }
}

constexpr int kAdamMulti = 32;
struct AdamMultiArgs {
  tt_adam_tensor t[kAdamMulti];
};

__global__ __launch_bounds__(kThreads) void adam_multi_kernel(AdamMultiArgs a, AdamK k0) {
  const AdamK k = adam_resolve(k0);
  const tt_adam_tensor& t = a.t[blockIdx.y];
  const int64_t stride = (int64_t)gridDim.x * blockDim.x;
  for (int64_t i = (int64_t)blockIdx.x * blockDim.x + threadIdx.x; i < t.n; i += stride) {
    float pp = t.p[i], mm = t.m[i], vv = t.v[i];
    adam1(pp, t.g[i], mm, vv, k);
    t.p[i] = pp; t.m[i] = mm; t.v[i] = vv;
  }
}

template <int VEC>
__global__ __launch_bounds__(kThreads) void adam_sparse_kernel(float* __restrict__ table, float* __restrict__ m, float* __restrict__ v,
                                                              int32_t E, uint32_t C, const int32_t* __restrict__ unique_rows,
                                                              const float* __restrict__ grad_rows, const int32_t* __restrict__ n_unique,
                                                              AdamK k0, uint32_t LG, int64_t table_rows) {
  const AdamK k = adam_resolve(k0);
  const uint32_t U = (uint32_t)*n_unique;
  const uint32_t gthread = blockIdx.x * blockDim.x + threadIdx.x;
  const uint32_t lig = gthread % LG;
  const uint32_t ngroups = gridDim.x * blockDim.x / LG;
  for (uint32_t u = gthread / LG; u < U; u += ngroups) {
    const int64_t row = unique_rows[u];
    if (row >= table_rows) continue;
    for (uint32_t chunk = lig; chunk < C; chunk += LG) {
      const int64_t o = row * E + chunk * VEC;
      const float* gp = grad_rows + (int64_t)u * E + chunk * VEC;
      if (VEC == 4) {
        float4 pp = *reinterpret_cast<float4*>(table + o), mm = *reinterpret_cast<float4*>(m + o),
               vv = *reinterpret_cast<float4*>(v + o);
        const float4 gg = *reinterpret_cast<const float4*>(gp);
        adam1(pp.x, gg.x, mm.x, vv.x, k); adam1(pp.y, gg.y, mm.y, vv.y, k);
        adam1(pp.z, gg.z, mm.z, vv.z, k); adam1(pp.w, gg.w, mm.w, vv.w, k);
        *reinterpret_cast<float4*>(table + o) = pp;
        *reinterpret_cast<float4*>(m + o) = mm;
        *reinterpret_cast<float4*>(v + o) = vv;
      } else {
        float pp = table[o], mm = m[o], vv = v[o];
        adam1(pp, gp[0], mm, vv, k);
        table[o] = pp; m[o] = mm; v[o] = vv;
      }
    }
  }
}

struct AdamFusedArgs {
  tt_adam_tensor t[kAdamMulti];
  int32_t blk0[kAdamMulti + 1];
  int32_t n;
};

template <int VEC, bool LONG>
__global__ __launch_bounds__(kThreads) void adam_fused_kernel(AdamFusedArgs a, float* __restrict__ table, float* __restrict__ m,
                                                             float* __restrict__ v, int32_t E, uint32_t C,
                                                             const int32_t* __restrict__ unique_rows, float* __restrict__ grad_rows,
                                                             const int32_t* __restrict__ n_unique, AdamK k0, uint32_t LG, int64_t table_rows,
                                                             const int32_t* __restrict__ seg, GradWs ws, int nlb) {
  const AdamK k = adam_resolve(k0);
  const int nd = a.blk0[a.n];
  if ((int)blockIdx.x < nd) {
    int ti = 0;
    for (int i = 1; i < a.n; ++i)
      if ((int)blockIdx.x >= a.blk0[i]) ti = i;
    const tt_adam_tensor t = a.t[ti];
    const int64_t nb = a.blk0[ti + 1] - a.blk0[ti];
    const int64_t stride = nb * blockDim.x;
    for (int64_t i = (int64_t)((int)blockIdx.x - a.blk0[ti]) * blockDim.x + threadIdx.x; i < t.n; i += stride) {
      float pp = t.p[i], mm = t.m[i], vv = t.v[i];
      adam1(pp, t.g[i], mm, vv, k);
      t.p[i] = pp; t.m[i] = mm; t.v[i] = vv;
    }
    return;
  }
  const int first = nd + (LONG ? nlb : 0);
  if (LONG && (int)blockIdx.x < first) {
    __shared__ float part[kFinishMaxFloats];
    long_rows_finish<VEC>(E, C, seg, ws, LG, blockIdx.x - nd, (uint32_t)nlb, part, [&](int32_t u, int32_t col, float tot) {
      grad_rows[(int64_t)u * E + col] = tot;
      const int64_t row = unique_rows[u];
      if (row >= table_rows) return;
      const int64_t o = row * E + col;
      float pp = table[o], mm = m[o], vv = v[o];
      adam1(pp, tot, mm, vv, k);
      table[o] = pp; m[o] = mm; v[o] = vv;
    });
    return;
  }
  const uint32_t U = (uint32_t)*n_unique;
  const uint32_t gthread = (blockIdx.x - first) * blockDim.x + threadIdx.x;
  const uint32_t lig = gthread % LG;
  const uint32_t ngroups = (gridDim.x - first) * blockDim.x / LG;
  for (uint32_t u = gthread / LG; u < U; u += ngroups) {
    const int64_t row = unique_rows[u];
    if (row >= table_rows) continue;
    if (LONG && seg[u + 1] - seg[u] > kLongSeg) continue;
    for (uint32_t chunk = lig; chunk < C; chunk += LG) {
      const int64_t o = row * E + chunk * VEC;
      const float* gp = grad_rows + (int64_t)u * E + chunk * VEC;
      if (VEC == 4) {
        float4 pp = *reinterpret_cast<float4*>(table + o), mm = *reinterpret_cast<float4*>(m + o),
               vv = *reinterpret_cast<float4*>(v + o);
        const float4 gg = *reinterpret_cast<const float4*>(gp);
        adam1(pp.x, gg.x, mm.x, vv.x, k); adam1(pp.y, gg.y, mm.y, vv.y, k);
        adam1(pp.z, gg.z, mm.z, vv.z, k); adam1(pp.w, gg.w, mm.w, vv.w, k);
        *reinterpret_cast<float4*>(table + o) = pp;
        *reinterpret_cast<float4*>(m + o) = mm;
        *reinterpret_cast<float4*>(v + o) = vv;
      } else {
        float pp = table[o], mm = m[o], vv = v[o];
        adam1(pp, gp[0], mm, vv, k);
        table[o] = pp; m[o] = mm; v[o] = vv;
      }
    }
  }
}

struct AdagradK {
  float lr, eps, wd;
  const float* dev;
};

__device__ __forceinline__ AdagradK adagrad_resolve(const AdagradK& k) {
// ... 807 lines not shown
  TT_CHECK_ARG(table_rows >= 1 && table_rows <= INT32_MAX, "tt_dedup_plan: table_rows=%lld out of range", (long long)table_rows);
  hipStream_t st = reinterpret_cast<hipStream_t>(stream);
  if (M == 0) {
    zero_two_words_kernel<<<1, 64, 0, st>>>(n_unique, seg_offsets);
    TT_LAUNCH_CHECK();
    return TT_OK;
  }
  TT_CHECK_ARG(rows && workspace, "tt_dedup_plan: NULL rows/workspace");
  if (workspace_bytes < tt_dedup_workspace_bytes(M)) {
    tt_set_error("tt_dedup_plan: workspace %zu < required %zu", workspace_bytes, tt_dedup_workspace_bytes(M));
    return TT_ERR_WORKSPACE;
  }
  DedupWs w = dedup_layout(reinterpret_cast<char*>(workspace), M);
  const uint32_t nblk = (uint32_t)tt_cdiv(M, kSortTile);
  int bits = 1;
  while (((int64_t)1 << bits) < table_rows) ++bits;
  int digit = 8, passes = (bits + 7) / 8;
  if ((bits + 10) / 11 < passes) { digit = 11; passes = (bits + 10) / 11; }
  const uint32_t* kin = reinterpret_cast<const uint32_t*>(rows);
  const uint32_t* vin = nullptr;
  for (int p = 0; p < passes; ++p) {
    const bool last_to_A = ((passes - 1 - p) % 2) == 0;
    uint32_t* kout = last_to_A ? w.keysA : w.keysB;
    uint32_t* vout = last_to_A ? reinterpret_cast<uint32_t*>(sorted_src) : w.valsB;
    int rc = digit == 8 ? sort_pass<8>(st, kin, vin, kout, vout, (uint32_t)M, p * digit, w.hist, w.total, nblk)
                        : sort_pass<11>(st, kin, vin, kout, vout, (uint32_t)M, p * digit, w.hist, w.total, nblk);
    if (rc != TT_OK) return rc;
    kin = kout;
    vin = vout;
  }
  return launch_heads(ctx, st, w, M, nblk, n_unique, unique_rows, seg_offsets, 0xFFFFFFFFu);
}

int tt_dedup_plan_runs(tt_ctx* ctx, const int32_t* rows, int32_t G, int64_t C, int64_t row_limit, int32_t* sorted_src,
                       int32_t* unique_rows, int32_t* seg_offsets, int32_t* n_unique, void* workspace, size_t workspace_bytes,
                       tt_stream stream) {
  TT_CHECK_ARG(ctx && rows && sorted_src && unique_rows && seg_offsets && n_unique && workspace, "tt_dedup_plan_runs: NULL argument");
  TT_CHECK_ARG(G >= 1 && G <= TT_MAX_RANKS && C >= 1 && (int64_t)G * C < ((int64_t)1 << 31) - kSortTile, "tt_dedup_plan_runs: bad G / C");
  const int64_t M = (int64_t)G * C;
  if (workspace_bytes < tt_dedup_workspace_bytes(M)) {
    tt_set_error("tt_dedup_plan_runs: workspace %zu < required %zu", workspace_bytes, tt_dedup_workspace_bytes(M));
    return TT_ERR_WORKSPACE;
  }
  hipStream_t st = reinterpret_cast<hipStream_t>(stream);
  DedupWs w = dedup_layout(reinterpret_cast<char*>(workspace), M);
  const uint32_t nblk = (uint32_t)tt_cdiv(M, kSortTile);
  merge_runs_kernel<<<grid_for(ctx, M), kThreads, 0, st>>>(rows, (uint32_t)G, (uint32_t)C, w.keysA, sorted_src);
  TT_LAUNCH_CHECK();
  return launch_heads(ctx, st, w, M, nblk, n_unique, unique_rows, seg_offsets,
                      row_limit > 0 && row_limit < (int64_t)0xFFFFFFFFll ? (uint32_t)row_limit : 0xFFFFFFFFu);
}

size_t tt_dedup_keyed_workspace_bytes(int64_t M, int32_t n_keys) {
  return align256(sizeof(int32_t) * (size_t)(M > 0 ? M : 1)) * 2 +
         3 * align256(sizeof(int32_t) * (size_t)(n_keys > 0 ? n_keys : 1) * kKeyedMaxParts);
}

static int dedup_plan_keyed_impl(tt_ctx* ctx, const int32_t* rows, const int32_t* side_K, int32_t n_sides, int64_t B, int32_t* sorted_src,
                                 int32_t* unique_rows, int32_t* seg_offsets, int32_t* n_unique, void* workspace, size_t workspace_bytes,
                                 tt_stream stream, bool key_major, int32_t E = 0, void* grad_ws = nullptr, size_t grad_ws_bytes = 0) {
  TT_CHECK_ARG(ctx && rows && side_K && sorted_src && unique_rows && seg_offsets && n_unique && workspace, "tt_dedup_plan_keyed: NULL argument");
  TT_CHECK_ARG(n_sides >= 1 && n_sides <= TT_MAX_SIDES, "tt_dedup_plan_keyed: n_sides=%d", n_sides);
  if (B < 1 || B > kKeyedB) {
    tt_set_error("tt_dedup_plan_keyed: B=%lld not in [1, %d]; use tt_dedup_plan", (long long)B, kKeyedB);
    return TT_ERR_UNSUPPORTED;
  }
  KeyedArgs a{};
  a.n_sides = n_sides;
  a.B = (int32_t)B;
  int n_keys = 0;
  int64_t slots = 0;
  for (int i = 0; i < n_sides; ++i) {
    TT_CHECK_ARG(side_K[i] >= 0, "tt_dedup_plan_keyed: negative K");
    a.side_base[i] = (int32_t)slots;
    a.key_base[i] = n_keys;
    a.K[i] = side_K[i];
    n_keys += side_K[i];
    slots += B * side_K[i];
  }
  a.side_base[n_sides] = (int32_t)slots;
  a.key_base[n_sides] = n_keys;
  TT_CHECK_ARG(slots < ((int64_t)1 << 31), "tt_dedup_plan_keyed: too many slots");
  hipStream_t st = reinterpret_cast<hipStream_t>(stream);
  if (n_keys == 0) {
    zero_two_words_kernel<<<1, 64, 0, st>>>(n_unique, seg_offsets);
    TT_LAUNCH_CHECK();
    return TT_OK;
  }
  if (workspace_bytes < tt_dedup_keyed_workspace_bytes(slots, n_keys)) {
    tt_set_error("tt_dedup_plan_keyed: workspace %zu < required %zu", workspace_bytes, tt_dedup_keyed_workspace_bytes(slots, n_keys));
    return TT_ERR_WORKSPACE;
  }
  char* w = reinterpret_cast<char*>(workspace);
  int32_t* uniq_stage = reinterpret_cast<int32_t*>(w);
  int32_t* seg_stage = reinterpret_cast<int32_t*>(w + align256(sizeof(int32_t) * (size_t)slots));
  int32_t* ucount = reinterpret_cast<int32_t*>(w + 2 * align256(sizeof(int32_t) * (size_t)slots));
  int32_t* ubase = reinterpret_cast<int32_t*>(w + 2 * align256(sizeof(int32_t) * (size_t)slots) +
                                              align256(sizeof(int32_t) * (size_t)n_keys * kKeyedMaxParts));
  int32_t* uend = reinterpret_cast<int32_t*>(w + 2 * align256(sizeof(int32_t) * (size_t)slots) +
                                             2 * align256(sizeof(int32_t) * (size_t)n_keys * kKeyedMaxParts));
  PlanLong pl{};
  if (grad_ws) {
    if (E < 1 || grad_ws_bytes < tt_embed_grad_workspace_bytes(slots, E)) {
      tt_set_error("tt_dedup_plan_keyed_long: gradient workspace %zu < required %zu", grad_ws_bytes, tt_embed_grad_workspace_bytes(slots, E));
      return TT_ERR_WORKSPACE;
    }
    const GradLayout gl = grad_layout(reinterpret_cast<char*>(grad_ws), slots, E);
    pl = PlanLong{gl.ws.counters, gl.ws.long_row, gl.ws.long_base, gl.ws.chunk_lo, gl.ws.chunk_hi};
  }
  int parts = ctx->keyed_parts > 0 ? ctx->keyed_parts : (B >= 2048 ? 6 : 1);
  if (parts > kKeyedMaxParts) parts = kKeyedMaxParts;
  while (parts > 1 && (int64_t)n_keys * parts > (int64_t)ctx->num_cus) --parts;
  a.parts = parts;
  keyed_sort_kernel<<<n_keys * parts, kKeyedThreads, 0, st>>>(a, rows, sorted_src, uniq_stage, seg_stage, ucount, ubase, uend, key_major,
                                                              pl.counters);
  TT_LAUNCH_CHECK();
  const CompactRider cr{uniq_stage, seg_stage, ucount, ubase, uend, pl, n_keys * parts, slots, unique_rows, seg_offsets, n_unique};
  if (ctx->defer_riders & 1) {
    if (ctx->riders->c_wg > 0)
      if (int rc = tt_riders_flush(ctx, st)) return rc;
    ctx->riders->c = cr;
    ctx->riders->c_wg = n_keys * parts;
    return TT_OK;
  }
  keyed_compact_kernel<<<n_keys * parts, kKeyedThreads, 0, st>>>(cr);
  TT_LAUNCH_CHECK();
  return TT_OK;
}

int tt_dedup_plan_keyed(tt_ctx* ctx, const int32_t* rows, const int32_t* side_K, int32_t n_sides, int64_t B, int32_t* sorted_src,
                        int32_t* unique_rows, int32_t* seg_offsets, int32_t* n_unique, void* workspace, size_t workspace_bytes,
                        tt_stream stream) {
  return dedup_plan_keyed_impl(ctx, rows, side_K, n_sides, B, sorted_src, unique_rows, seg_offsets, n_unique, workspace, workspace_bytes,
                               stream, false);
}

int tt_dedup_plan_keyed_long(tt_ctx* ctx, const int32_t* rows, int32_t rows_key_major, const int32_t* side_K, int32_t n_sides, int64_t B,
                             int32_t E, int32_t* sorted_src, int32_t* unique_rows, int32_t* seg_offsets, int32_t* n_unique,
                             void* grad_workspace, size_t grad_workspace_bytes, void* workspace, size_t workspace_bytes, tt_stream stream) {
  TT_CHECK_ARG(grad_workspace, "tt_dedup_plan_keyed_long: NULL gradient workspace");
  return dedup_plan_keyed_impl(ctx, rows, side_K, n_sides, B, sorted_src, unique_rows, seg_offsets, n_unique, workspace, workspace_bytes,
                               stream, rows_key_major != 0, E, grad_workspace, grad_workspace_bytes);
}

int tt_dedup_plan_keyed_km(tt_ctx* ctx, const int32_t* rows_km, const int32_t* side_K, int32_t n_sides, int64_t B, int32_t* sorted_src,
                           int32_t* unique_rows, int32_t* seg_offsets, int32_t* n_unique, void* workspace, size_t workspace_bytes,
                           tt_stream stream) {
  return dedup_plan_keyed_impl(ctx, rows_km, side_K, n_sides, B, sorted_src, unique_rows, seg_offsets, n_unique, workspace, workspace_bytes,
                               stream, true);
}

size_t tt_embed_grad_workspace_bytes(int64_t M, int32_t E) { return grad_layout(nullptr, M > 0 ? M : 1, E > 0 ? E : 1).bytes; }

int tt_embed_grad_bwd(tt_ctx* ctx, const tt_grad_src* srcs, int32_t n_srcs, int64_t B, int32_t E, const int32_t* sorted_src,
                      const int32_t* seg_offsets, const int32_t* unique_rows, const int32_t* n_unique, int64_t M, int32_t mode,
                      float* out, int32_t* counters, void* workspace, size_t workspace_bytes, tt_stream stream) {
  TT_CHECK_ARG(ctx && srcs && out, "tt_embed_grad_bwd: NULL argument");
  TT_CHECK_ARG(n_srcs >= 1 && n_srcs <= TT_MAX_SIDES, "tt_embed_grad_bwd: n_srcs=%d", n_srcs);
  const bool all_short = (mode & TT_GRAD_SHORT_SEGMENTS) != 0;
  const bool planned = (mode & TT_GRAD_PLANNED) != 0 && !all_short;
  const bool defer = (mode & TT_GRAD_DEFER_FINISH) != 0;
  mode &= ~(TT_GRAD_SHORT_SEGMENTS | TT_GRAD_PLANNED | TT_GRAD_DEFER_FINISH);
  TT_CHECK_ARG(!defer || (planned && mode == TT_GRAD_SPARSE), "tt_embed_grad_bwd: TT_GRAD_DEFER_FINISH needs TT_GRAD_PLANNED | TT_GRAD_SPARSE");
  TT_CHECK_ARG(mode >= TT_GRAD_SPARSE && mode <= TT_GRAD_DENSE_ACC, "tt_embed_grad_bwd: bad mode %d", mode);
  TT_CHECK_ARG(E >= 1 && B >= 0, "tt_embed_grad_bwd: bad E/B");
  if (M == 0) return TT_OK;
  TT_CHECK_ARG(sorted_src && seg_offsets && unique_rows && n_unique && workspace, "tt_embed_grad_bwd: NULL plan/workspace");
  if (workspace_bytes < tt_embed_grad_workspace_bytes(M, E)) {
    tt_set_error("tt_embed_grad_bwd: workspace %zu < required %zu", workspace_bytes, tt_embed_grad_workspace_bytes(M, E));
    return TT_ERR_WORKSPACE;
  }
  SideSet a{};
  a.n = n_srcs;
  a.E = E;
  bool vec4 = (E % 4 == 0) && tt_aligned(out, 16);
  int64_t slots = 0;
  for (int i = 0; i < n_srcs; ++i) {
    const tt_grad_src& s = srcs[i];
    TT_CHECK_ARG(s.K == 0 || s.d_out, "tt_embed_grad_bwd: src %d NULL", i);
    TT_CHECK_ARG(s.dtype == TT_F32 || s.dtype == TT_BF16, "tt_embed_grad_bwd: src %d bad dtype", i);
    TT_CHECK_ARG(s.dtype == srcs[0].dtype, "tt_embed_grad_bwd: all sources must share one dtype (src %d differs)", i);
    a.s[i] = SideDev{nullptr, nullptr, nullptr, const_cast<char*>(reinterpret_cast<const char*>(s.d_out)), s.ld, (uint32_t)slots, s.K, s.dtype, s.K > 1 ? (uint32_t)(0x100000000ull / (uint64_t)s.K) : 0xFFFFFFFFu};
    const size_t esz = s.dtype == TT_BF16 ? 2 : 4;
    vec4 = vec4 && (s.ld % 4 == 0) && tt_aligned(s.d_out, 4 * esz);
    slots += B * s.K;
  }
  TT_CHECK_ARG(slots == M, "tt_embed_grad_bwd: sum(B*K)=%lld != M=%lld", (long long)slots, (long long)M);
  a.C = (uint32_t)(vec4 ? E / 4 : E);
  a.total_slots = (uint32_t)slots;
  const uint32_t LG = pow2_at_least(a.C) > 64 ? 64 : pow2_at_least(a.C);
  const int dt = srcs[0].dtype;
  GradLayout gl = grad_layout(reinterpret_cast<char*>(workspace), M, E);
  hipStream_t st = reinterpret_cast<hipStream_t>(stream);
  if (int rc = tt_riders_flush(ctx, st)) return rc;
  if (planned) {
  } else if (counters) {
    gl.ws.counters = counters;
  } else if (!all_short) {
    zero_words_kernel<<<1, 64, 0, st>>>(gl.ws.counters, 2);
    TT_LAUNCH_CHECK();
  }
  TnPending* slabs = (ctx->deferred && ctx->deferred->n > 0) ? ctx->deferred : nullptr;
  if (slabs && !planned) {
    if (int rc = tt_gemm_deferred_flush(ctx, st)) return rc;
    slabs = nullptr;
  }
  const int nsx = slabs ? tt_slab_role_blocks_x(slabs) : 0;
  const int g1 = grid_for(ctx, M * LG);
  const int g2 = grid_for(ctx, gl.max_chunks * LG);
  const int g3 = (int)(gl.max_long < (int64_t)ctx->num_cus * 8 ? gl.max_long : (int64_t)ctx->num_cus * 8);
  if ((int64_t)(kThreads / LG) * E > kFinishMaxFloats) {
    tt_set_error("tt_embed_grad_bwd: E=%d too wide for the long-row finish (max %d)", E, kFinishMaxFloats * (int)LG / kThreads);
    return TT_ERR_UNSUPPORTED;
  }
#define TT_SEG_LAUNCH(V, D, G)                                                                                                  \
  do {                                                                                                                          \
    if (planned && slabs) {                                                                                                     \
      const int sc = kSegThreads / kThreads;                                                                                  \
      const int g1s = (int)tt_cdiv(g1, sc), g2s = (int)tt_cdiv(g2, sc), nsxs = (int)tt_cdiv(nsx, sc);                           \
      const int nss = tt_slab_role_blocks(slabs, nsxs);                                                                         \
      seg_reduce_chunk_slab_kernel<V, D, G><<<nss + g1s + g2s, kSegThreads, 0, st>>>(                                           \
          a, sorted_src, seg_offsets, unique_rows, n_unique, mode, out, gl.ws, LG, (uint32_t)g1s, slabs->sb, (uint32_t)nsxs,    \
          (uint32_t)slabs->n, (uint32_t)nss);                                                                                   \
      TT_LAUNCH_CHECK();                                                                                                        \
      slabs->n = 0;                                                                                                             \
      slabs->maxtotal = 1;                                                                                                      \
      if (!defer) seg_long_finish_kernel<V><<<g3, kThreads, 0, st>>>(E, a.C, seg_offsets, unique_rows, mode, out, gl.ws, LG);   \
      break;                                                                                                                    \
    }                                                                                                                           \
    if (planned) {                                                                                                              \
      seg_reduce_chunk_kernel<V, D, G><<<g1 + g2, kThreads, 0, st>>>(a, sorted_src, seg_offsets, unique_rows, n_unique, mode,   \
                                                                     out, gl.ws, LG, (uint32_t)g1);                             \
      TT_LAUNCH_CHECK();                                                                                                        \
      if (!defer) seg_long_finish_kernel<V><<<g3, kThreads, 0, st>>>(E, a.C, seg_offsets, unique_rows, mode, out, gl.ws, LG);   \
      break;                                                                                                                    \
    }                                                                                                                           \
    seg_reduce_kernel<V, D, G><<<g1, kThreads, 0, st>>>(a, sorted_src, seg_offsets, unique_rows, n_unique, mode, out, gl.ws, LG, \
                                                        all_short);                                                             \
    TT_LAUNCH_CHECK();                                                                                                          \
    if (all_short) break;                                                                                                       \
    seg_chunk_kernel<V, D, G><<<g2, kThreads, 0, st>>>(a, sorted_src, gl.ws, LG);                                                \
    TT_LAUNCH_CHECK();                                                                                                          \
    seg_long_finish_kernel<V><<<g3, kThreads, 0, st>>>(E, a.C, seg_offsets, unique_rows, mode, out, gl.ws, LG);                 \
  } while (0)
#define TT_SEG_LAUNCH_G(V, D)                              \
  do {                                                     \
    if (lgt == 8) TT_SEG_LAUNCH(V, D, 8);                  \
    else if (lgt == 16) TT_SEG_LAUNCH(V, D, 16);           \
    else if (lgt == 4) TT_SEG_LAUNCH(V, D, 4);             \
    else TT_SEG_LAUNCH(V, D, 0);                           \
  } while (0)
  const int lgt = (vec4 && a.C == LG && (LG == 4 || LG == 8 || LG == 16)) ? (int)LG : 0;
  if (vec4 && dt == TT_F32) TT_SEG_LAUNCH_G(4, TT_F32);
  else if (vec4) TT_SEG_LAUNCH_G(4, TT_BF16);
  else if (dt == TT_F32) TT_SEG_LAUNCH(1, TT_F32, 0);
  else TT_SEG_LAUNCH(1, TT_BF16, 0);
#undef TT_SEG_LAUNCH_G
#undef TT_SEG_LAUNCH
  TT_LAUNCH_CHECK();
  return TT_OK;
}

void tt_adam_hparams(int64_t step, float lr, float beta1, float beta2, float eps, float weight_decay, float out6[6]) {
  const AdamK k = make_adam(step < 1 ? 1 : step, lr, beta1, beta2, eps, weight_decay, nullptr);
  out6[0] = k.lr_over_bc1; out6[1] = k.inv_sqrt_bc2; out6[2] = k.b1; out6[3] = k.b2; out6[4] = k.eps; out6[5] = k.wd;
}

int tt_adam_dense_step(tt_ctx* ctx, float* p, const float* g, float* m, float* v, int64_t n, int64_t step, float lr, float beta1,
                       float beta2, float eps, float weight_decay, const float* hparams_dev, tt_stream stream) {
  if (int rc = tt_riders_flush(ctx, reinterpret_cast<hipStream_t>(stream))) return rc;
  if (ctx && ctx->deferred && ctx->deferred->n > 0)
    if (int rc = tt_gemm_deferred_flush(ctx, reinterpret_cast<hipStream_t>(stream))) return rc;
  TT_CHECK_ARG(ctx && (n == 0 || (p && g && m && v)), "tt_adam_dense_step: NULL argument");
  TT_CHECK_ARG(step >= 1 && n >= 0, "tt_adam_dense_step: step must be >= 1");
  if (n == 0) return TT_OK;
  const AdamK k = make_adam(step, lr, beta1, beta2, eps, weight_decay, hparams_dev);
  hipStream_t st = reinterpret_cast<hipStream_t>(stream);
  if (n % 4 == 0 && tt_aligned(p, 16) && tt_aligned(g, 16) && tt_aligned(m, 16) && tt_aligned(v, 16)) {
    adam_dense_vec4_kernel<<<grid_for(ctx, n / 4), kThreads, 0, st>>>(reinterpret_cast<float4*>(p), reinterpret_cast<const float4*>(g),
                                                                      reinterpret_cast<float4*>(m), reinterpret_cast<float4*>(v), n / 4, k);
  } else {
    adam_dense_kernel<<<grid_for(ctx, n), kThreads, 0, st>>>(p, g, m, v, n, k);
  }
  TT_LAUNCH_CHECK();
  return TT_OK;
}

int tt_adam_multi_step(tt_ctx* ctx, const tt_adam_tensor* tensors, int32_t n_tensors, int64_t step, float lr, float beta1,
                       float beta2, float eps, float weight_decay, const float* hparams_dev, tt_stream stream) {
  if (int rc = tt_riders_flush(ctx, reinterpret_cast<hipStream_t>(stream))) return rc;
  if (ctx && ctx->deferred && ctx->deferred->n > 0)
    if (int rc = tt_gemm_deferred_flush(ctx, reinterpret_cast<hipStream_t>(stream))) return rc;
  TT_CHECK_ARG(ctx && (n_tensors == 0 || tensors), "tt_adam_multi_step: NULL argument");
  TT_CHECK_ARG(step >= 1 && n_tensors >= 0, "tt_adam_multi_step: step must be >= 1");
  const AdamK k = make_adam(step, lr, beta1, beta2, eps, weight_decay, hparams_dev);
  hipStream_t st = reinterpret_cast<hipStream_t>(stream);
  for (int base = 0; base < n_tensors; base += kAdamMulti) {
    AdamMultiArgs a{};
    const int cnt = n_tensors - base < kAdamMulti ? n_tensors - base : kAdamMulti;
    int64_t nmax = 1;
    for (int i = 0; i < cnt; ++i) {
      const tt_adam_tensor& t = tensors[base + i];
      TT_CHECK_ARG(t.n >= 0 && (t.n == 0 || (t.p && t.g && t.m && t.v)), "tt_adam_multi_step: tensor %d has NULL pointers", base + i);
      a.t[i] = t;
      nmax = t.n > nmax ? t.n : nmax;
    }
    int64_t gx = tt_cdiv(nmax, kThreads);
    if (gx > 64) gx = 64;
    adam_multi_kernel<<<dim3((unsigned)gx, (unsigned)cnt), kThreads, 0, st>>>(a, k);
    TT_LAUNCH_CHECK();
  }
  return TT_OK;
}

int tt_sparse_adam_step(tt_ctx* ctx, float* table, float* m, float* v, int64_t table_rows, int32_t E, const int32_t* unique_rows,
                        const float* grad_rows, const int32_t* n_unique, int64_t M, int64_t step, float lr, float beta1, float beta2, float eps,
                        float weight_decay, const float* hparams_dev, tt_stream stream) {
  if (int rc = tt_riders_flush(ctx, reinterpret_cast<hipStream_t>(stream))) return rc;
  if (ctx && ctx->deferred && ctx->deferred->n > 0)
    if (int rc = tt_gemm_deferred_flush(ctx, reinterpret_cast<hipStream_t>(stream))) return rc;
  TT_CHECK_ARG(ctx && table && m && v, "tt_sparse_adam_step: NULL state");
  TT_CHECK_ARG(step >= 1 && E >= 1 && M >= 0 && table_rows >= 1, "tt_sparse_adam_step: bad step/E/M/table_rows");
  if (M == 0) return TT_OK;
  TT_CHECK_ARG(unique_rows && grad_rows && n_unique, "tt_sparse_adam_step: NULL plan");
  const AdamK k = make_adam(step, lr, beta1, beta2, eps, weight_decay, hparams_dev);
  const bool vec4 = (E % 4 == 0) && tt_aligned(table, 16) && tt_aligned(m, 16) && tt_aligned(v, 16) && tt_aligned(grad_rows, 16);
  const uint32_t C = vec4 ? E / 4 : E;
  const uint32_t LG = pow2_at_least(C) > 64 ? 64 : pow2_at_least(C);
  hipStream_t st = reinterpret_cast<hipStream_t>(stream);
  const int grid = grid_for(ctx, M * LG);
  if (vec4) adam_sparse_kernel<4><<<grid, kThreads, 0, st>>>(table, m, v, E, C, unique_rows, grad_rows, n_unique, k, LG, table_rows);
  else adam_sparse_kernel<1><<<grid, kThreads, 0, st>>>(table, m, v, E, C, unique_rows, grad_rows, n_unique, k, LG, table_rows);
  TT_LAUNCH_CHECK();
  return TT_OK;
}

static int adam_fused_impl(tt_ctx* ctx, const tt_adam_tensor* tensors, int32_t n_tensors, float* table, float* m, float* v,
                           int64_t table_rows, int32_t E, const int32_t* unique_rows, float* grad_rows, const int32_t* n_unique, int64_t M,
                           const int32_t* seg_offsets, void* grad_workspace, size_t grad_workspace_bytes, int64_t step, float lr,
                           float beta1, float beta2, float eps, float weight_decay, const float* hparams_dev, tt_stream stream,
                           const char* who) {
  if (int rc = tt_riders_flush(ctx, reinterpret_cast<hipStream_t>(stream))) return rc;
  if (ctx && ctx->deferred && ctx->deferred->n > 0)
    if (int rc = tt_gemm_deferred_flush(ctx, reinterpret_cast<hipStream_t>(stream))) return rc;
  TT_CHECK_ARG(ctx && tensors && table && m && v && unique_rows && grad_rows && n_unique, "%s: NULL argument", who);
  TT_CHECK_ARG(n_tensors >= 1 && n_tensors <= kAdamMulti, "%s: n_tensors=%d not in [1,%d]", who, n_tensors, kAdamMulti);
  TT_CHECK_ARG(step >= 1 && E >= 1 && M >= 1 && table_rows >= 1, "%s: bad step/E/M/table_rows", who);
  AdamFusedArgs a{};
  a.n = n_tensors;
  int nd = 0;
  for (int i = 0; i < n_tensors; ++i) {
    const tt_adam_tensor& t = tensors[i];
    TT_CHECK_ARG(t.n >= 0 && (t.n == 0 || (t.p && t.g && t.m && t.v)), "%s: tensor %d has NULL pointers", who, i);
    a.t[i] = t;
    a.blk0[i] = nd;
    int64_t nb = tt_cdiv(t.n > 0 ? t.n : 1, kThreads);
    nd += (int)(nb > 64 ? 64 : nb);
  }
  a.blk0[n_tensors] = nd;
  const AdamK k = make_adam(step, lr, beta1, beta2, eps, weight_decay, hparams_dev);
  const bool vec4 = (E % 4 == 0) && tt_aligned(table, 16) && tt_aligned(m, 16) && tt_aligned(v, 16) && tt_aligned(grad_rows, 16);
  const uint32_t C = vec4 ? E / 4 : E;
  const uint32_t LG = pow2_at_least(C) > 64 ? 64 : pow2_at_least(C);
  hipStream_t st = reinterpret_cast<hipStream_t>(stream);
  if (grad_workspace) {
    TT_CHECK_ARG(seg_offsets, "%s: NULL seg_offsets", who);
    if (grad_workspace_bytes < tt_embed_grad_workspace_bytes(M, E)) {
      tt_set_error("%s: gradient workspace %zu < required %zu", who, grad_workspace_bytes, tt_embed_grad_workspace_bytes(M, E));
      return TT_ERR_WORKSPACE;
    }
    if ((int64_t)(kThreads / LG) * E > kFinishMaxFloats) {
      tt_set_error("%s: E=%d too wide for the long-row finish (max %d)", who, E, kFinishMaxFloats * (int)LG / kThreads);
      return TT_ERR_UNSUPPORTED;
    }
    const GradLayout gl = grad_layout(reinterpret_cast<char*>(grad_workspace), M, E);
    const int nlb = (int)(gl.max_long < (int64_t)ctx->num_cus * 8 ? gl.max_long : (int64_t)ctx->num_cus * 8);
    const int grid = nd + nlb + grid_for(ctx, M * LG);
    if (vec4) adam_fused_kernel<4, true><<<grid, kThreads, 0, st>>>(a, table, m, v, E, C, unique_rows, grad_rows, n_unique, k, LG, table_rows, seg_offsets, gl.ws, nlb);
    else adam_fused_kernel<1, true><<<grid, kThreads, 0, st>>>(a, table, m, v, E, C, unique_rows, grad_rows, n_unique, k, LG, table_rows, seg_offsets, gl.ws, nlb);
    TT_LAUNCH_CHECK();
    return TT_OK;
  }
  const int grid = nd + grid_for(ctx, M * LG);
  if (vec4) adam_fused_kernel<4, false><<<grid, kThreads, 0, st>>>(a, table, m, v, E, C, unique_rows, grad_rows, n_unique, k, LG, table_rows, nullptr, GradWs{}, 0);
  else adam_fused_kernel<1, false><<<grid, kThreads, 0, st>>>(a, table, m, v, E, C, unique_rows, grad_rows, n_unique, k, LG, table_rows, nullptr, GradWs{}, 0);
  TT_LAUNCH_CHECK();
  return TT_OK;
}

int tt_adam_fused_step(tt_ctx* ctx, const tt_adam_tensor* tensors, int32_t n_tensors, float* table, float* m, float* v, int64_t table_rows,
                       int32_t E,
                       const int32_t* unique_rows, const float* grad_rows, const int32_t* n_unique, int64_t M, int64_t step, float lr,
                       float beta1, float beta2, float eps, float weight_decay, const float* hparams_dev, tt_stream stream) {
  return adam_fused_impl(ctx, tensors, n_tensors, table, m, v, table_rows, E, unique_rows, const_cast<float*>(grad_rows), n_unique, M,
                         nullptr, nullptr, 0, step, lr, beta1, beta2, eps, weight_decay, hparams_dev, stream, "tt_adam_fused_step");
}

int tt_adam_fused_step_finish(tt_ctx* ctx, const tt_adam_tensor* tensors, int32_t n_tensors, float* table, float* m, float* v,
                              int64_t table_rows, int32_t E, const int32_t* unique_rows, float* grad_rows, const int32_t* n_unique,
                              int64_t M, const int32_t* seg_offsets, void* grad_workspace, size_t grad_workspace_bytes, int64_t step,
                              float lr, float beta1, float beta2, float eps, float weight_decay, const float* hparams_dev,
                              tt_stream stream) {
  TT_CHECK_ARG(grad_workspace, "tt_adam_fused_step_finish: NULL gradient workspace");
  return adam_fused_impl(ctx, tensors, n_tensors, table, m, v, table_rows, E, unique_rows, grad_rows, n_unique, M, seg_offsets,
                         grad_workspace, grad_workspace_bytes, step, lr, beta1, beta2, eps, weight_decay, hparams_dev, stream,
                         "tt_adam_fused_step_finish");
}

static AdagradK make_adagrad(float lr, float eps, float wd, const float* dev) {
  AdagradK k;
  k.lr = lr; k.eps = eps; k.wd = wd;
  k.dev = dev;
  return k;
}

static bool adagrad_mapping(const char* who, int32_t E, bool vec4, uint32_t* C, uint32_t* LG) {
  *C = vec4 ? E / 4 : E;
  *LG = pow2_at_least(*C) > 64 ? 64 : pow2_at_least(*C);
  if (*C > (uint32_t)kAdagradMaxChunks * *LG) {
    tt_set_error("%s: E=%d too wide (max %d, or %d when E %% 4 != 0)", who, E, kAdagradMaxChunks * 64 * 4, kAdagradMaxChunks * 64);
    return false;
  }
  return true;
}

static int flush_before_optimiser(tt_ctx* ctx, tt_stream stream) {
  if (int rc = tt_riders_flush(ctx, reinterpret_cast<hipStream_t>(stream))) return rc;
  if (ctx && ctx->deferred && ctx->deferred->n > 0)
    if (int rc = tt_gemm_deferred_flush(ctx, reinterpret_cast<hipStream_t>(stream))) return rc;
  return TT_OK;
}

int tt_rowwise_adagrad_sparse_step(tt_ctx* ctx, float* table, float* sum, int64_t table_rows, int32_t E, const int32_t* unique_rows,
                                   const float* grad_rows, const int32_t* n_unique, int64_t M, float lr, float eps, float weight_decay,
                                   const float* hparams_dev, tt_stream stream) {
  if (int rc = flush_before_optimiser(ctx, stream)) return rc;
  TT_CHECK_ARG(ctx && table && sum, "tt_rowwise_adagrad_sparse_step: NULL state");
  TT_CHECK_ARG(E >= 1 && M >= 0 && table_rows >= 1, "tt_rowwise_adagrad_sparse_step: bad E/M/table_rows");
  if (M == 0) return TT_OK;
  TT_CHECK_ARG(unique_rows && grad_rows && n_unique, "tt_rowwise_adagrad_sparse_step: NULL plan");
  const AdagradK k = make_adagrad(lr, eps, weight_decay, hparams_dev);
  const bool vec4 = (E % 4 == 0) && tt_aligned(table, 16) && tt_aligned(grad_rows, 16);
  uint32_t C, LG;
  if (!adagrad_mapping("tt_rowwise_adagrad_sparse_step", E, vec4, &C, &LG)) return TT_ERR_UNSUPPORTED;
  hipStream_t st = reinterpret_cast<hipStream_t>(stream);
  const int grid = grid_for(ctx, M * LG);
  if (vec4) adagrad_sparse_kernel<4><<<grid, kThreads, 0, st>>>(table, sum, E, C, unique_rows, grad_rows, n_unique, k, LG, table_rows);
  else adagrad_sparse_kernel<1><<<grid, kThreads, 0, st>>>(table, sum, E, C, unique_rows, grad_rows, n_unique, k, LG, table_rows);
  TT_LAUNCH_CHECK();
  return TT_OK;
}

int tt_rowwise_adagrad_dense_step(tt_ctx* ctx, float* table, float* sum, const float* grad, int64_t table_rows, int32_t E, float lr,
                                  float eps, float weight_decay, const float* hparams_dev, tt_stream stream) {
  if (int rc = flush_before_optimiser(ctx, stream)) return rc;
  TT_CHECK_ARG(ctx && table && sum && grad, "tt_rowwise_adagrad_dense_step: NULL state");
  TT_CHECK_ARG(E >= 1 && table_rows >= 1, "tt_rowwise_adagrad_dense_step: bad E/table_rows");
  const AdagradK k = make_adagrad(lr, eps, weight_decay, hparams_dev);
  const bool vec4 = (E % 4 == 0) && tt_aligned(table, 16) && tt_aligned(grad, 16);
  uint32_t C, LG;
  if (!adagrad_mapping("tt_rowwise_adagrad_dense_step", E, vec4, &C, &LG)) return TT_ERR_UNSUPPORTED;
  hipStream_t st = reinterpret_cast<hipStream_t>(stream);
  const int grid = grid_for(ctx, table_rows * LG);
  if (vec4) adagrad_dense_kernel<4><<<grid, kThreads, 0, st>>>(table, sum, grad, table_rows, E, C, k, LG);
  else adagrad_dense_kernel<1><<<grid, kThreads, 0, st>>>(table, sum, grad, table_rows, E, C, k, LG);
  TT_LAUNCH_CHECK();
  return TT_OK;
}

static int adam_adagrad_fused_impl(tt_ctx* ctx, const tt_adam_tensor* tensors, int32_t n_tensors, int64_t step, float lr, float beta1,
                                   float beta2, float eps, float weight_decay, const float* hparams_dev, float* table, float* sum,
                                   int64_t table_rows, int32_t E, const int32_t* unique_rows, float* grad_rows, const int32_t* n_unique,
                                   int64_t M, const int32_t* seg_offsets, void* grad_workspace, size_t grad_workspace_bytes,
                                   float table_lr, float table_eps, float table_weight_decay, const float* table_hparams_dev,
                                   tt_stream stream, const char* who) {
  if (int rc = flush_before_optimiser(ctx, stream)) return rc;
  TT_CHECK_ARG(ctx && tensors && table && sum && unique_rows && grad_rows && n_unique, "%s: NULL argument", who);
  TT_CHECK_ARG(n_tensors >= 1 && n_tensors <= kAdamMulti, "%s: n_tensors=%d not in [1,%d]", who, n_tensors, kAdamMulti);
  TT_CHECK_ARG(step >= 1 && E >= 1 && M >= 1 && table_rows >= 1, "%s: bad step/E/M/table_rows", who);
  AdamFusedArgs a{};
  a.n = n_tensors;
  int nd = 0;
  for (int i = 0; i < n_tensors; ++i) {
    const tt_adam_tensor& t = tensors[i];
    TT_CHECK_ARG(t.n >= 0 && (t.n == 0 || (t.p && t.g && t.m && t.v)), "%s: tensor %d has NULL pointers", who, i);
    a.t[i] = t;
    a.blk0[i] = nd;
    int64_t nb = tt_cdiv(t.n > 0 ? t.n : 1, kThreads);
    nd += (int)(nb > 64 ? 64 : nb);
  }
  a.blk0[n_tensors] = nd;
  const AdamK ak = make_adam(step, lr, beta1, beta2, eps, weight_decay, hparams_dev);
  const AdagradK gk = make_adagrad(table_lr, table_eps, table_weight_decay, table_hparams_dev);
  const bool vec4 = (E % 4 == 0) && tt_aligned(table, 16) && tt_aligned(grad_rows, 16);
  uint32_t C, LG;
  if (!adagrad_mapping(who, E, vec4, &C, &LG)) return TT_ERR_UNSUPPORTED;
  hipStream_t st = reinterpret_cast<hipStream_t>(stream);
  if (grad_workspace) {
    TT_CHECK_ARG(seg_offsets, "%s: NULL seg_offsets", who);
    if (grad_workspace_bytes < tt_embed_grad_workspace_bytes(M, E)) {
      tt_set_error("%s: gradient workspace %zu < required %zu", who, grad_workspace_bytes, tt_embed_grad_workspace_bytes(M, E));
      return TT_ERR_WORKSPACE;
    }
    if ((int64_t)(kThreads / LG) * E > kFinishMaxFloats) {
      tt_set_error("%s: E=%d too wide for the long-row finish (max %d)", who, E, kFinishMaxFloats * (int)LG / kThreads);
      return TT_ERR_UNSUPPORTED;
    }
    const GradLayout gl = grad_layout(reinterpret_cast<char*>(grad_workspace), M, E);
    const int nlb = (int)(gl.max_long < (int64_t)ctx->num_cus * 8 ? gl.max_long : (int64_t)ctx->num_cus * 8);
    const int grid = nd + nlb + grid_for(ctx, M * LG);
    if (vec4) adam_adagrad_fused_kernel<4, true><<<grid, kThreads, 0, st>>>(a, ak, table, sum, E, C, unique_rows, grad_rows, n_unique, gk, LG, table_rows, seg_offsets, gl.ws, nlb);
    else adam_adagrad_fused_kernel<1, true><<<grid, kThreads, 0, st>>>(a, ak, table, sum, E, C, unique_rows, grad_rows, n_unique, gk, LG, table_rows, seg_offsets, gl.ws, nlb);
    TT_LAUNCH_CHECK();
    return TT_OK;
  }
  const int grid = nd + grid_for(ctx, M * LG);
  if (vec4) adam_adagrad_fused_kernel<4, false><<<grid, kThreads, 0, st>>>(a, ak, table, sum, E, C, unique_rows, grad_rows, n_unique, gk, LG, table_rows, nullptr, GradWs{}, 0);
  else adam_adagrad_fused_kernel<1, false><<<grid, kThreads, 0, st>>>(a, ak, table, sum, E, C, unique_rows, grad_rows, n_unique, gk, LG, table_rows, nullptr, GradWs{}, 0);
  TT_LAUNCH_CHECK();
  return TT_OK;
}

int tt_adam_rowwise_adagrad_fused_step(tt_ctx* ctx, const tt_adam_tensor* tensors, int32_t n_tensors, int64_t step, float lr,
                                       float beta1, float beta2, float eps, float weight_decay, const float* hparams_dev, float* table,
                                       float* sum, int64_t table_rows, int32_t E, const int32_t* unique_rows, const float* grad_rows,
                                       const int32_t* n_unique, int64_t M, float table_lr, float table_eps, float table_weight_decay,
                                       const float* table_hparams_dev, tt_stream stream) {
  return adam_adagrad_fused_impl(ctx, tensors, n_tensors, step, lr, beta1, beta2, eps, weight_decay, hparams_dev, table, sum, table_rows,
                                 E, unique_rows, const_cast<float*>(grad_rows), n_unique, M, nullptr, nullptr, 0, table_lr, table_eps,
                                 table_weight_decay, table_hparams_dev, stream, "tt_adam_rowwise_adagrad_fused_step");
}

int tt_adam_rowwise_adagrad_fused_step_finish(tt_ctx* ctx, const tt_adam_tensor* tensors, int32_t n_tensors, int64_t step, float lr,
                                              float beta1, float beta2, float eps, float weight_decay, const float* hparams_dev,
                                              float* table, float* sum, int64_t table_rows, int32_t E, const int32_t* unique_rows,
                                              float* grad_rows, const int32_t* n_unique, int64_t M, const int32_t* seg_offsets,
                                              void* grad_workspace, size_t grad_workspace_bytes, float table_lr, float table_eps,
                                              float table_weight_decay, const float* table_hparams_dev, tt_stream stream) {
  TT_CHECK_ARG(grad_workspace, "tt_adam_rowwise_adagrad_fused_step_finish: NULL gradient workspace");
  return adam_adagrad_fused_impl(ctx, tensors, n_tensors, step, lr, beta1, beta2, eps, weight_decay, hparams_dev, table, sum, table_rows,
                                 E, unique_rows, grad_rows, n_unique, M, seg_offsets, grad_workspace, grad_workspace_bytes, table_lr,
                                 table_eps, table_weight_decay, table_hparams_dev, stream, "tt_adam_rowwise_adagrad_fused_step_finish");
}

int tt_embed_grad_finish(tt_ctx* ctx, int32_t E, const int32_t* seg_offsets, int64_t M, float* out, void* workspace,
                         size_t workspace_bytes, tt_stream stream) {
  TT_CHECK_ARG(ctx && seg_offsets && out && workspace, "tt_embed_grad_finish: NULL argument");
  TT_CHECK_ARG(E >= 1 && M >= 1, "tt_embed_grad_finish: bad E/M");
  if (workspace_bytes < tt_embed_grad_workspace_bytes(M, E)) {
    tt_set_error("tt_embed_grad_finish: workspace %zu < required %zu", workspace_bytes, tt_embed_grad_workspace_bytes(M, E));
    return TT_ERR_WORKSPACE;
  }
  const bool vec4 = (E % 4 == 0) && tt_aligned(out, 16);
  const uint32_t C = vec4 ? E / 4 : E;
  const uint32_t LG = pow2_at_least(C) > 64 ? 64 : pow2_at_least(C);
  const GradLayout gl = grad_layout(reinterpret_cast<char*>(workspace), M, E);
  const int g3 = (int)(gl.max_long < (int64_t)ctx->num_cus * 8 ? gl.max_long : (int64_t)ctx->num_cus * 8);
  hipStream_t st = reinterpret_cast<hipStream_t>(stream);
  if (vec4) seg_long_finish_kernel<4><<<g3, kThreads, 0, st>>>(E, C, seg_offsets, nullptr, TT_GRAD_SPARSE, out, gl.ws, LG);
// ... 316 lines not shown
```

### jodalrob-twotower_amd/graph.py

```python
from __future__ import annotations

from typing import Dict, Optional

import torch

from . import _lib as L
from . import ops
from .config import settings
from .kjt import KeyedJaggedTensor
from .optim import FusedAdam


class GraphedTrainStep:
    _steps_per_replay = 1

    def __init__(self, task, optimizer: FusedAdam, example_batch: Dict, return_metrics: bool = True, warmup: int = 3,
                 defer_long: bool = True, defer_slabs: bool = True, defer_riders: bool = True, preserve_state: bool = True,
                 accumulate_metrics: bool = False, metric_sums: Optional[torch.Tensor] = None):
        if not isinstance(optimizer, FusedAdam):
            raise TypeError("GraphedTrainStep needs jodalrob_twotower_amd.optim.FusedAdam (device-side hyper-parameters)")
        self.task, self.opt, self.return_metrics = task, optimizer, return_metrics
        self._defer_long, self._defer_slabs, self._defer_riders = bool(defer_long), bool(defer_slabs), bool(defer_riders)
        dev = example_batch["notice"]["dense"].device
        self.static = {side: {"dense": example_batch[side]["dense"].clone(),
                              "kjt": KeyedJaggedTensor(example_batch[side]["kjt"].keys(), example_batch[side]["kjt"].values().clone())}
                       for side in ("notice", "company")}
        ng = len(optimizer.param_groups)
        self._n_scalar = ng * 8 + 2
        self._slot_len = (self._n_scalar + 3) // 4 * 4
        self._ring = 64
        self._host_ring = torch.zeros(self._ring, self._slot_len, dtype=torch.float32).pin_memory()
        self._slot_events = [None] * self._ring
        self._slot = 0
        self._unmarked = []
        self._host = self._host_ring[0, :self._n_scalar]
        self._dev = torch.zeros(ng * 8 + 2, dtype=torch.float32, device=dev)
        self._hp_dev = self._dev[:ng * 8].view(ng, 8)
        self._seed_dev = self._dev[ng * 8:].view(torch.int64)
        self._ones = torch.ones((), dtype=torch.float32, device=dev)
        self._towers = [m for m in task.modules() if hasattr(m, "_seed_dev") and hasattr(m, "dense_parameters")]
        self.metric_sums = torch.zeros(8, dtype=torch.float32, device=dev) if (accumulate_metrics and return_metrics) else None
        sums_before = None
        if metric_sums is not None and self.metric_sums is not None:
            self.metric_sums, sums_before = metric_sums, metric_sums.clone()
        self._ingest = self._setup_ingest()
        self._shadows = self._setup_shadows()
        if self._ingest is not None:
            self._run_ingest([], None)
        snap = self._snapshot_state() if (preserve_state and warmup > 0) else None
        side = torch.cuda.Stream(device=dev)
        side.wait_stream(torch.cuda.current_stream(dev))
        with torch.cuda.stream(side):
            for _ in range(warmup):
                self._eager_once()
        torch.cuda.current_stream(dev).wait_stream(side)
        torch.cuda.synchronize(dev)
        if snap is not None:
            self._restore_state(snap)
        if self.metric_sums is not None:
            self.metric_sums.zero_() if sums_before is None else self.metric_sums.copy_(sums_before)
        if self._ingest is not None:
            self._run_ingest([], None)
        self._push_scalars()
        for t in self._towers:
            t._seed_dev = self._seed_dev
        optimizer._hp_dev = self._hp_dev
        self.graph = None
        import torch.distributed as _dist
        mode = "thread_local" if (_dist.is_available() and _dist.is_initialized()) else "global"
        n0 = L.load().tt_launch_count()
        try:
            self._capture(mode)
        finally:
            self.library_launches = int(L.load().tt_launch_count() - n0) + 1
            optimizer._hp_dev = None
            for t in self._towers:
                t._seed_dev = None
        optimizer.advance_steps(-self._steps_per_replay)

    def _capture(self, mode: str):
        self.graph = torch.cuda.CUDAGraph()
        with torch.cuda.graph(self.graph, capture_error_mode=mode):
            self.result = self._body()

    def _replay_graph(self):
        self.graph.replay()

    def _setup_ingest(self):
        self._x_static, self._rows_sm = None, None
        if not settings.graph_ingest:
            return None
        model = getattr(self.task, "two_tower_model", None)
        towers = [getattr(model, n, None) for n in ("notice_tower", "company_tower")]
        if model is None or any(t is None for t in towers):
            return None
        embs = [t.categorical_embedder for t in towers]
        ex = getattr(self.task, "exchange", None)
        if ex is not None:
            store = getattr(ex, "store", None)
            ids = [self.static[side]["kjt"].values() for side in ("notice", "company")]
            B = self.static["notice"]["dense"].shape[0]
            if store is None or not hasattr(ex, "poll_overflow") or not (0 < B <= ops.KEYED_MAX_B) or \
                    any(len(e.keys) == 0 or len(e.keys) > 64 or v.dtype != torch.int64 or not v.is_contiguous() for e, v in zip(embs, ids)):
                return None
            rows_km = torch.empty(sum(v.numel() for v in ids), dtype=torch.int32, device=ids[0].device)
            return store, embs, rows_km, ids, B
        store = embs[0].store
        ids = [self.static[side]["kjt"].values() for side in ("notice", "company")]
        B = self.static["notice"]["dense"].shape[0]
        if any(e.store is not store for e in embs) or store.weight is None or not (0 < B <= ops.KEYED_MAX_B):
            return None
        if any(len(e.keys) == 0 or len(e.keys) > 64 or v.dtype != torch.int64 or not v.is_contiguous() or v.numel() != B * len(e.keys)
               for e, v in zip(embs, ids)):
            return None
        rows_km = torch.empty(sum(v.numel() for v in ids), dtype=torch.int32, device=ids[0].device)
        if settings.graph_ingest_lookup:
            xs = [torch.zeros((B, t.x_width), dtype=t.x_dtype, device=ids[0].device) for t in towers]
            outs = [ops.LookupSide(v, e._key_row_offset, e._key_vocab, x[:, t.tower_hidden_dims[0]:], len(e.keys))
                    for e, v, x, t in zip(embs, ids, xs, towers)]
            if ops.ingest_lookup_supported(store.weight, outs):
                self._x_static = xs
        if self._x_static is None and settings.graph_ingest_rows and store.weight.shape[1] % 4 == 0:
            self._rows_sm = torch.empty_like(rows_km)
        return store, embs, rows_km, ids, B

    def _setup_shadows(self):
        if not settings.graph_weight_shadows or self._ingest is None:
            return []
        out = []
        for t in self._towers:
            if getattr(t, "mlp_dtype", None) != "bf16" or t.n_hidden < 1:
                continue
            lins = [t.mlp[4 * i] for i in range(t.n_hidden)]
            ws = [t.dense_projection.weight] + [l.weight for l in lins]
            if any(w.dtype != torch.float32 or not w.is_contiguous() or w.numel() % 8 for w in ws):
                continue
            sh = [torch.empty(w.shape, dtype=torch.bfloat16, device=w.device) for w in ws]
            out.append((t, ws, sh))
        n = sum(len(ws) for _, ws, _ in out)
        return out if 0 < n <= L.TT_MAX_CVT else []

    def _cvt(self):
        return [(s_, w) for _, ws, sh in self._shadows for w, s_ in zip(ws, sh)]

    def _lookup_outs(self):
        towers = [self.task.two_tower_model.notice_tower, self.task.two_tower_model.company_tower]
        return [x[:, t.tower_hidden_dims[0]:] for x, t in zip(self._x_static, towers)]

    def _register(self, store, ids, rows_km):
        xs = getattr(self, "_x_static", None)
        store.ingest = (ids, [v._version for v in ids], rows_km, xs, getattr(self, "_rows_sm", None))
        store.ingest_x_fresh = xs is not None

    @staticmethod
    def _table_rows(store) -> int:
        g = getattr(store, "global_rows", None)
        return int(g) if g is not None else int(store.weight.shape[0])

    def _run_ingest(self, pairs, src_ids):
        store, embs, rows_km, ids, B = self._ingest
        src = ids if src_ids is None else src_ids
        xs = getattr(self, "_x_static", None)
        if xs is not None:
            sides = [ops.LookupSide(v, e._key_row_offset, e._key_vocab, o, len(e.keys)) for e, v, o in zip(embs, src, self._lookup_outs())]
            ops.batch_ingest(pairs, sides, B, rows_km, table=store.weight, cvt=self._cvt())
        else:
            sides = [ops.LookupSide(v, e._key_row_offset, e._key_vocab, None, len(e.keys)) for e, v in zip(embs, src)]
            ops.batch_ingest(pairs, sides, B, rows_km, rows_sm=getattr(self, "_rows_sm", None), cvt=self._cvt(), table_rows=self._table_rows(store))
        self._register(store, ids, rows_km)

    def _body(self):
        self.opt.zero_grad(set_to_none=True)
        defer = self._defer_long
        stores = list(getattr(self.opt, "_stores", ()))
        for st in stores:
            st.defer_long_finish = defer
        dev = self._dev.device
        ex = getattr(self.task, "exchange", None)
        slabs = self._defer_slabs
        riders = self._defer_riders and self._ingest is not None and (ex is None or not getattr(self.task, "sync_bn", False))
        for t, _, sh in self._shadows:
            t._w16 = (sh[0], sh[1:])
        try:
            if riders:
                L.set_defer_riders(dev, True, loss_only=ex is not None)
            res = self.task(self.static, return_metrics=self.return_metrics)
            loss = res["loss"] if isinstance(res, dict) else res
            if slabs:
                L.set_defer_slab_reduce(dev, True)
            try:
                loss.backward(self._ones)
            finally:
                if slabs:
                    L.set_defer_slab_reduce(dev, False)
            self.opt.step()
            for st in stores:
                if st.sparse_grad is not None:
                    ops.embed_grad_finish(st.sparse_grad[0])
            if self.metric_sums is not None:
                self.metric_sums.add_(res.out8)
        finally:
            for t, _, _ in self._shadows:
                t._w16 = None
            if riders:
                L.set_defer_riders(dev, False)
            for st in stores:
                st.defer_long_finish = False
        return res

    def _eager_once(self):
        if self._ingest is not None:
            self._run_ingest([], None)
        self._body()

    def _touched_rows(self, store):
        model = getattr(self.task, "two_tower_model", None)
        if model is None or getattr(self.task, "exchange", None) is not None:
            return None
        rows = []
        for name, side in (("notice_tower", "notice"), ("company_tower", "company")):
            tw = getattr(model, name, None)
            if tw is None:
                return None
            e = tw.categorical_embedder
            if e.store is not store or not e.keys:
                continue
            ids = self.static[side]["kjt"].values().view(-1, len(e.keys))
            rows.append((ids.clamp(min=0).minimum(e._key_vocab - 1) + e._key_row_offset).reshape(-1))
        return torch.unique(torch.cat(rows)) if rows else None

    def _snapshot_state(self):
        opt = self.opt
        opt._flush_pending()
        table_ids = opt._table_param_ids()
        snap = {"buffers": [(b, b.detach().clone()) for b in self.task.buffers()], "dense": [], "stores": [], "steps": []}
        for group in opt.param_groups:
            for p in group["params"]:
                if id(p) in table_ids:
                    continue
                st = opt.state.get(p) or {}
                snap["dense"].append((p, p.detach().clone(), None if "exp_avg" not in st else
                                      (st["exp_avg"].clone(), st["exp_avg_sq"].clone(), st["step"].clone())))
        for store in getattr(opt, "_stores", ()):
            if store.weight is None or not store.optim_parameters():
                continue
            st = opt._state_of(store)
            keys = ("sum",) if "sum" in st else ("m", "v")
            rows = self._touched_rows(store) if store.grad_mode == "sparse" else None
            if rows is None and (store.weight.numel() + sum(st[k].numel() for k in keys)) * 4 > (8 << 30):
                rows = torch.empty(0, dtype=torch.int64, device=store.weight.device)
            pick = (lambda t: t[rows].clone()) if rows is not None else (lambda t: t.clone())
            snap["stores"].append((store, rows, pick(store.weight), {k: pick(st[k]) for k in keys}, st["step"]))
        snap["steps"] = [(st, st["step"].clone()) for st in opt.state.values() if "step" in st]
        return snap

    @torch.no_grad()
    def _restore_state(self, snap):
        opt = self.opt
        opt._flush_pending()
        for b, saved in snap["buffers"]:
            b.copy_(saved)
        for p, w, st0 in snap["dense"]:
            p.copy_(w)
            st = opt.state.get(p)
            if st and "exp_avg" in st:
                if st0 is None:
                    st["exp_avg"].zero_(); st["exp_avg_sq"].zero_(); st["step"] = torch.tensor(0.0)
                else:
                    st["exp_avg"].copy_(st0[0]); st["exp_avg_sq"].copy_(st0[1]); st["step"] = st0[2].clone()
        for store, rows, w, saved, step in snap["stores"]:
            st = opt._state_of(store)
            if rows is None:
                store.weight.copy_(w)
                for k, t in saved.items():
                    st[k].copy_(t)
            elif rows.numel():
                store.weight[rows] = w
                for k, t in saved.items():
                    st[k][rows] = t
            st["step"] = step
        known = {id(st): val for st, val in snap["steps"]}
        for st in opt.state.values():
            if "step" in st:
                st["step"] = known[id(st)].clone() if id(st) in known else torch.tensor(0.0)
        opt._step_cache = None
        opt.zero_grad(set_to_none=True)

    def _fill_slot(self, ahead: int = 0):
        self._slot = (self._slot + 1) % self._ring
        self._unmarked.append(self._slot)
        ev = self._slot_events[self._slot]
        if ev is not None:
            ev.synchronize()
        host = self._host_ring[self._slot, :self._n_scalar]
        ng = len(self.opt.param_groups)
        step = self.opt.peek_step() + 1 + ahead
        for gi, g in enumerate(self.opt.param_groups):
            if g.get("table_optimizer", "adam") == "rowwise_adagrad":
                host[gi * 8: gi * 8 + 3] = torch.tensor([float(g["lr"]), g["eps"], g["weight_decay"]])
                continue
            hp = ops.adam_hparams(step, float(g["lr"]), g["betas"][0], g["betas"][1], g["eps"], g["weight_decay"])
            host[gi * 8: gi * 8 + 6] = torch.tensor(hp)
        host[ng * 8:].view(torch.int64).random_()
        return (self._dev, host)

    def _mark_slot(self):
        slots, self._unmarked = self._unmarked, []
        if not slots:
            return
        ev = self._slot_events[slots[0]]
        if ev is None or len(slots) > 1:
            ev = torch.cuda.Event()
        ev.record()
        for sl in slots:
            self._slot_events[sl] = ev

    def _push_scalars(self):
        ops.copy_multi([self._fill_slot()])
        self._mark_slot()

    def _handover_pairs(self, batch: Optional[Dict]):
        pairs, src_ids = [], []
        if batch is None:
            return pairs, None
        for side in ("notice", "company"):
            d, v = batch[side]["dense"], batch[side]["kjt"].values()
            sd, sv = self.static[side]["dense"], self.static[side]["kjt"].values()
            if d.device == sd.device and d.dtype == sd.dtype and v.dtype == sv.dtype and d.is_contiguous() and v.is_contiguous():
                pairs += [(sd, d), (sv, v)]
                src_ids.append(v)
            else:
                sd.copy_(d, non_blocking=True)
                sv.copy_(v, non_blocking=True)
                src_ids.append(sv)
        return pairs, src_ids

    def step(self, batch: Optional[Dict] = None):
        pairs, src_ids = self._handover_pairs(batch)
        if self._ingest is not None:
            self._run_ingest(pairs + [self._fill_slot()], src_ids)
            self._mark_slot()
        else:
            ops.copy_multi(pairs + [self._fill_slot()])
            self._mark_slot()
        return self._replay()

    def _replay(self):
        self._replay_graph()
        self.opt.advance_steps(self._steps_per_replay)
        ex = getattr(self.task, "exchange", None)
        if ex is not None and hasattr(ex, "poll_overflow"):
            ex.poll_overflow()
        return self.result

    def step_from_store(self, notice_store, company_store, pairs: torch.Tensor, order: Optional[torch.Tensor] = None, offset: int = 0):
        self._ingest_from_store(notice_store, company_store, pairs, order, offset)
        self._mark_slot()
        return self._replay()

    def _ingest_from_store(self, notice_store, company_store, pairs: torch.Tensor, order: Optional[torch.Tensor], offset: int, ahead: int = 0):
# ... 116 lines not shown
```

### jodalrob-twotower_amd/ops.py

```python
from __future__ import annotations

import ctypes as C
from dataclasses import dataclass
from typing import List, Optional, Sequence

import torch

from . import _lib as L
from .config import settings
from ._lib import TT_BF16, TT_F32, TT_GRAD_DENSE_ACC, TT_GRAD_DENSE_SET, TT_GRAD_SPARSE


class KernelTimer:

    def __init__(self, names=None):
        self.names = set(names) if names else None
        self.records = {}

    def wants(self, name):
        return self.names is None or name in self.names

    def summary(self):
        torch.cuda.synchronize()
        return {n: (len(ev), sum(a.elapsed_time(b) for a, b in ev) / max(len(ev), 1)) for n, ev in self.records.items()}


_TIMER: Optional[KernelTimer] = None
_SYNC_DEBUG = settings.sync_debug


def set_timer(t: Optional[KernelTimer]):
    global _TIMER
    _TIMER = t


class _timed:
    __slots__ = ("name", "a")

    def __init__(self, name):
        self.name = name
        self.a = None

    def __enter__(self):
        if _TIMER is not None and _TIMER.wants(self.name):
            self.a = torch.cuda.Event(enable_timing=True)
            self.a.record()
        return self

    def __exit__(self, *exc):
        if _SYNC_DEBUG and not torch.cuda.is_current_stream_capturing():
            import sys
            print(f"[tt] {self.name} ...", end="", file=sys.stderr, flush=True)
            torch.cuda.synchronize()
            print(" done", file=sys.stderr, flush=True)
        if self.a is not None:
            b = torch.cuda.Event(enable_timing=True)
            b.record()
            _TIMER.records.setdefault(self.name, []).append((self.a, b))
        return False


def _dt(t: torch.Tensor) -> int:
    if t.dtype == torch.float32:
        return TT_F32
    if t.dtype == torch.bfloat16:
        return TT_BF16
    raise TypeError(f"unsupported dtype {t.dtype}")


@dataclass
class LookupSide:
    ids: torch.Tensor
    key_row_offset: torch.Tensor
    key_vocab: torch.Tensor
    out: torch.Tensor
    K: int


def embed_lookup(table: Optional[torch.Tensor], sides: Sequence[LookupSide], B: int, want_rows: bool, E: int = 0,
                 table_rows: int = 0, tag: str = "") -> Optional[torch.Tensor]:
    dev = table.device if table is not None else sides[0].ids.device
    E = table.shape[1] if table is not None else E
    table_rows = table.shape[0] if table is not None else table_rows
    arr = (L.EmbedSide * len(sides))()
    M = 0
    for i, s in enumerate(sides):
        if s.ids.dtype != torch.int64 or not s.ids.is_contiguous() or s.ids.device != dev:
            raise ValueError("ids must be a contiguous int64 tensor on the table's device")
        if s.ids.numel() != B * s.K:
            raise ValueError(f"side {i}: {s.ids.numel()} ids for B={B}, K={s.K}")
        if s.out is not None:
            assert s.out.stride(1) == 1
            arr[i] = L.EmbedSide(L.ptr(s.ids), L.ptr(s.key_row_offset), L.ptr(s.key_vocab), L.ptr(s.out),
                                 s.out.stride(0), s.K, _dt(s.out))
        else:
            arr[i] = L.EmbedSide(L.ptr(s.ids), L.ptr(s.key_row_offset), L.ptr(s.key_vocab), None, s.K * E, s.K, TT_F32)
        M += B * s.K
    rows = torch.empty(M, dtype=torch.int32, device=dev) if want_rows else None
    with _timed("tt_embed_lookup_fwd" + tag):
        L.check(L.load().tt_embed_lookup_fwd(L.ctx(dev), L.ptr(table), table_rows, E, arr, len(sides), B,
                                             L.ptr(rows), L.stream(dev)), "tt_embed_lookup_fwd")
    return rows


def embed_lookup_rows(table: torch.Tensor, rows: torch.Tensor, sides: Sequence[LookupSide], B: int):
    dev, E = table.device, table.shape[1]
    arr = (L.EmbedSide * len(sides))()
    M = 0
    for i, s in enumerate(sides):
        assert s.out is not None and s.out.stride(1) == 1
        arr[i] = L.EmbedSide(None, None, None, L.ptr(s.out), s.out.stride(0), s.K, _dt(s.out))
        M += B * s.K
    if rows.dtype != torch.int32 or rows.numel() != M or not rows.is_contiguous() or rows.device != dev:
        raise ValueError("embed_lookup_rows: rows must be a contiguous int32 tensor of sum(B*K) elements on the table's device")
    with _timed("tt_embed_lookup_fwd"):
        L.check(L.load().tt_embed_lookup_rows_fwd(L.ctx(dev), L.ptr(table), table.shape[0], E, arr, len(sides), B, L.ptr(rows), L.stream(dev)),
                "tt_embed_lookup_rows_fwd")


class LookupProfile:

    MAX_WG = 8192

    def __init__(self, device, n_slots: int = 256):
        self.device, self.n = torch.device(device), n_slots
        self.ring = torch.zeros(self.MAX_WG + n_slots * self.MAX_WG * 2, dtype=torch.int64, device=self.device)
        L.check(L.load().tt_embed_lookup_set_profile(L.ctx(self.device), L.ptr(self.ring), n_slots), "tt_embed_lookup_set_profile")

    def reset(self):
        self.ring.zero_()

    def durations_us(self, first_wg: int = 0, last_wg: Optional[int] = None):
        torch.cuda.synchronize(self.device)
        r = self.ring.cpu()
        launches = int(r[0])
        pairs = r[self.MAX_WG:].view(self.n, self.MAX_WG, 2)
        same = r[:self.MAX_WG] == launches
        if first_wg or last_wg is not None:
            sel = torch.zeros_like(same)
            sel[first_wg:last_wg] = True
            same = same & sel
        out = []
        for n in range(max(0, launches - self.n), launches):
            blk = pairs[n % self.n]
            live = (blk[:, 1] > 0) & same
            if bool(live.any()):
                out.append(float(blk[live, 1].max() - blk[live, 0].min()) * 0.01)
        return out

    def close(self):
        L.check(L.load().tt_embed_lookup_set_profile(L.ctx(self.device), None, 0), "tt_embed_lookup_set_profile")

    def reopen(self):
        L.check(L.load().tt_embed_lookup_set_profile(L.ctx(self.device), L.ptr(self.ring), self.n), "tt_embed_lookup_set_profile")


@dataclass
class DedupPlan:
    sorted_src: torch.Tensor
    unique_rows: torch.Tensor
    seg_offsets: torch.Tensor
    n_unique: torch.Tensor
    M: int
    keep: object = None
    staging: object = None
    grad_ws: object = None
    finish_deferred: object = None


def dedup_plan(rows: torch.Tensor, table_rows: int) -> DedupPlan:
    dev, M = rows.device, rows.numel()
    buf = torch.empty(3 * M + 2, dtype=torch.int32, device=dev)
    plan = DedupPlan(buf[:M], buf[M:2 * M], buf[2 * M:3 * M + 1], buf[3 * M + 1:], M)
    lib = L.load()
    nb = lib.tt_dedup_workspace_bytes(M)
    ws = L.workspace(dev, nb)
    with _timed("tt_dedup_plan"):
        L.check(lib.tt_dedup_plan(L.ctx(dev), L.ptr(rows), M, table_rows, L.ptr(plan.sorted_src), L.ptr(plan.unique_rows),
                                  L.ptr(plan.seg_offsets), L.ptr(plan.n_unique), L.ptr(ws), ws.numel(), L.stream(dev)),
                "tt_dedup_plan")
    return plan


def dedup_plan_runs(rows: torch.Tensor, G: int, C: int, row_limit: int = 0) -> DedupPlan:
    dev, M = rows.device, G * C
    assert rows.numel() == M and rows.dtype == torch.int32
    buf = torch.empty(3 * M + 2, dtype=torch.int32, device=dev)
    plan = DedupPlan(buf[:M], buf[M:2 * M], buf[2 * M:3 * M + 1], buf[3 * M + 1:], M)
    lib = L.load()
    ws = L.workspace(dev, lib.tt_dedup_workspace_bytes(M))
    with _timed("tt_dedup_plan_runs"):
        L.check(lib.tt_dedup_plan_runs(L.ctx(dev), L.ptr(rows), G, C, row_limit, L.ptr(plan.sorted_src), L.ptr(plan.unique_rows),
                                       L.ptr(plan.seg_offsets), L.ptr(plan.n_unique), L.ptr(ws), ws.numel(), L.stream(dev)),
                "tt_dedup_plan_runs")
    return plan


KEYED_MAX_B = 8192


def dedup_plan_keyed(rows: torch.Tensor, side_K: Sequence[int], B: int, key_major: bool = False, E: int = 0) -> DedupPlan:
    dev, M = rows.device, rows.numel()
    assert M == B * sum(side_K)
    buf = torch.empty(3 * M + 2, dtype=torch.int32, device=dev)
    plan = DedupPlan(buf[:M], buf[M:2 * M], buf[2 * M:3 * M + 1], buf[3 * M + 1:], M)
    lib = L.load()
    nk = sum(side_K)
    if L.riders_deferred(dev, 1):
        ws = torch.empty(lib.tt_dedup_keyed_workspace_bytes(M, nk), dtype=torch.uint8, device=dev)
    else:
        ws = L.workspace(dev, lib.tt_dedup_keyed_workspace_bytes(M, nk))
    plan.staging = ws
    ks = (L.i32 * len(side_K))(*side_K)
    if E > 0 and settings.grad_planned:
        gws = torch.empty(lib.tt_embed_grad_workspace_bytes(M, E), dtype=torch.uint8, device=dev)
        with _timed("tt_dedup_plan_keyed"):
            L.check(lib.tt_dedup_plan_keyed_long(L.ctx(dev), L.ptr(rows), int(key_major), ks, len(side_K), B, E, L.ptr(plan.sorted_src),
                                                 L.ptr(plan.unique_rows), L.ptr(plan.seg_offsets), L.ptr(plan.n_unique), L.ptr(gws),
                                                 gws.numel(), L.ptr(ws), ws.numel(), L.stream(dev)), "tt_dedup_plan_keyed_long")
        plan.grad_ws = (gws, E)
        return plan
    fn = lib.tt_dedup_plan_keyed_km if key_major else lib.tt_dedup_plan_keyed
    with _timed("tt_dedup_plan_keyed"):
        L.check(fn(L.ctx(dev), L.ptr(rows), ks, len(side_K), B, L.ptr(plan.sorted_src), L.ptr(plan.unique_rows),
                   L.ptr(plan.seg_offsets), L.ptr(plan.n_unique), L.ptr(ws), ws.numel(), L.stream(dev)),
                "tt_dedup_plan_keyed")
    return plan


def embed_grad(plan: DedupPlan, srcs: Sequence[tuple], B: int, E: int, mode: int, out: torch.Tensor, short_segments: bool = False,
               counters: Optional[torch.Tensor] = None, defer_finish: bool = False):
    if short_segments:
        mode |= L.TT_GRAD_SHORT_SEGMENTS
    dev = out.device
    arr = (L.GradSrc * len(srcs))()
    for i, (d, K) in enumerate(srcs):
        assert d.stride(1) == 1
        arr[i] = L.GradSrc(L.ptr(d), d.stride(0), K, _dt(d))
    lib = L.load()
    nb = lib.tt_embed_grad_workspace_bytes(plan.M, E)
    if plan.grad_ws is not None and plan.grad_ws[1] == E and not short_segments:
        ws = plan.grad_ws[0]
        deferred = defer_finish and mode == L.TT_GRAD_SPARSE and plan.M >= 1
        mode |= L.TT_GRAD_PLANNED | (L.TT_GRAD_DEFER_FINISH if deferred else 0)
    else:
        ws = L.workspace(dev, nb)
        deferred = False
    with _timed("tt_embed_grad_bwd"):
        L.check(lib.tt_embed_grad_bwd(L.ctx(dev), arr, len(srcs), B, E, L.ptr(plan.sorted_src), L.ptr(plan.seg_offsets),
                                      L.ptr(plan.unique_rows), L.ptr(plan.n_unique), plan.M, mode, L.ptr(out),
                                      L.ptr(counters), L.ptr(ws), ws.numel(), L.stream(dev)), "tt_embed_grad_bwd")
    plan.finish_deferred = out if deferred else None


def embed_grad_finish(plan: DedupPlan):
    out = plan.finish_deferred
    if out is None:
        return
    ws, E = plan.grad_ws
    dev = out.device
    with _timed("tt_embed_grad_finish"):
        L.check(L.load().tt_embed_grad_finish(L.ctx(dev), E, L.ptr(plan.seg_offsets), plan.M, L.ptr(out), L.ptr(ws), ws.numel(),
                                              L.stream(dev)), "tt_embed_grad_finish")
    plan.finish_deferred = None


def adam_dense(p, g, m, v, step, lr, b1, b2, eps, wd, hp_dev=None):
    dev = p.device
    with _timed("tt_adam_dense_step"):
        L.check(L.load().tt_adam_dense_step(L.ctx(dev), L.ptr(p), L.ptr(g), L.ptr(m), L.ptr(v), p.numel(), step, lr, b1, b2,
                                            eps, wd, L.ptr(hp_dev), L.stream(dev)), "tt_adam_dense_step")


def adam_multi(items, step, lr, b1, b2, eps, wd, hp_dev=None):
    if not items:
        return
    dev = items[0][0].device
    arr = (L.AdamTensor * len(items))()
    for i, (p, g, m, v) in enumerate(items):
        arr[i] = L.AdamTensor(p.data_ptr(), g.data_ptr(), m.data_ptr(), v.data_ptr(), p.numel())
    with _timed("tt_adam_multi_step"):
        L.check(L.load().tt_adam_multi_step(L.ctx(dev), arr, len(items), step, lr, b1, b2, eps, wd, L.ptr(hp_dev), L.stream(dev)),
                "tt_adam_multi_step")


def adam_sparse(table, m, v, plan: DedupPlan, grad_rows, step, lr, b1, b2, eps, wd, hp_dev=None):
    dev = table.device
    embed_grad_finish(plan)
    with _timed("tt_sparse_adam_step"):
        L.check(L.load().tt_sparse_adam_step(L.ctx(dev), L.ptr(table), L.ptr(m), L.ptr(v), table.shape[0], table.shape[1],
                                             L.ptr(plan.unique_rows), L.ptr(grad_rows), L.ptr(plan.n_unique), plan.M, step,
                                             lr, b1, b2, eps, wd, L.ptr(hp_dev), L.stream(dev)), "tt_sparse_adam_step")


def adam_fused(items, table, m, v, plan: DedupPlan, grad_rows, step, lr, b1, b2, eps, wd, hp_dev=None):
    dev = table.device
    arr = (L.AdamTensor * len(items))()
    for i, (p, g, mm, vv) in enumerate(items):
        arr[i] = L.AdamTensor(p.data_ptr(), g.data_ptr(), mm.data_ptr(), vv.data_ptr(), p.numel())
    if plan.finish_deferred is not None:
        if plan.finish_deferred.data_ptr() != grad_rows.data_ptr():
            raise RuntimeError("adam_fused: the plan's deferred gradient is not the one handed to the optimiser")
        ws, E = plan.grad_ws
        with _timed("tt_adam_fused_step"):
            L.check(L.load().tt_adam_fused_step_finish(L.ctx(dev), arr, len(items), L.ptr(table), L.ptr(m), L.ptr(v), table.shape[0],
                                                       table.shape[1], L.ptr(plan.unique_rows), L.ptr(grad_rows), L.ptr(plan.n_unique),
                                                       plan.M, L.ptr(plan.seg_offsets), L.ptr(ws), ws.numel(), step, lr, b1, b2, eps, wd,
                                                       L.ptr(hp_dev), L.stream(dev)), "tt_adam_fused_step_finish")
        plan.finish_deferred = None
        return
    with _timed("tt_adam_fused_step"):
        L.check(L.load().tt_adam_fused_step(L.ctx(dev), arr, len(items), L.ptr(table), L.ptr(m), L.ptr(v), table.shape[0], table.shape[1],
                                            L.ptr(plan.unique_rows), L.ptr(grad_rows), L.ptr(plan.n_unique), plan.M, step,
                                            lr, b1, b2, eps, wd, L.ptr(hp_dev), L.stream(dev)), "tt_adam_fused_step")


def rowwise_adagrad_sparse(table, acc, plan: DedupPlan, grad_rows, lr, eps, wd, hp_dev=None):
    dev = table.device
    embed_grad_finish(plan)
    with _timed("tt_rowwise_adagrad_sparse_step"):
        L.check(L.load().tt_rowwise_adagrad_sparse_step(L.ctx(dev), L.ptr(table), L.ptr(acc), table.shape[0], table.shape[1],
                                                        L.ptr(plan.unique_rows), L.ptr(grad_rows), L.ptr(plan.n_unique), plan.M,
                                                        lr, eps, wd, L.ptr(hp_dev), L.stream(dev)), "tt_rowwise_adagrad_sparse_step")


def rowwise_adagrad_dense(table, acc, grad, lr, eps, wd, hp_dev=None):
    dev = table.device
    with _timed("tt_rowwise_adagrad_dense_step"):
        L.check(L.load().tt_rowwise_adagrad_dense_step(L.ctx(dev), L.ptr(table), L.ptr(acc), L.ptr(grad), table.shape[0], table.shape[1],
                                                       lr, eps, wd, L.ptr(hp_dev), L.stream(dev)), "tt_rowwise_adagrad_dense_step")


def adam_rowwise_adagrad_fused(items, step, lr, b1, b2, eps, wd, hp_dev, table, acc, plan: DedupPlan, grad_rows, t_lr, t_eps, t_wd,
                               t_hp_dev=None):
    dev = table.device
    arr = (L.AdamTensor * len(items))()
    for i, (p, g, mm, vv) in enumerate(items):
        arr[i] = L.AdamTensor(p.data_ptr(), g.data_ptr(), mm.data_ptr(), vv.data_ptr(), p.numel())
    if plan.finish_deferred is not None:
        if plan.finish_deferred.data_ptr() != grad_rows.data_ptr():
            raise RuntimeError("adam_rowwise_adagrad_fused: the plan's deferred gradient is not the one handed to the optimiser")
        ws, E = plan.grad_ws
        with _timed("tt_adam_rowwise_adagrad_fused_step"):
            L.check(L.load().tt_adam_rowwise_adagrad_fused_step_finish(
                L.ctx(dev), arr, len(items), step, lr, b1, b2, eps, wd, L.ptr(hp_dev), L.ptr(table), L.ptr(acc), table.shape[0],
                table.shape[1], L.ptr(plan.unique_rows), L.ptr(grad_rows), L.ptr(plan.n_unique), plan.M, L.ptr(plan.seg_offsets),
                L.ptr(ws), ws.numel(), t_lr, t_eps, t_wd, L.ptr(t_hp_dev), L.stream(dev)), "tt_adam_rowwise_adagrad_fused_step_finish")
        plan.finish_deferred = None
        return
    with _timed("tt_adam_rowwise_adagrad_fused_step"):
        L.check(L.load().tt_adam_rowwise_adagrad_fused_step(
            L.ctx(dev), arr, len(items), step, lr, b1, b2, eps, wd, L.ptr(hp_dev), L.ptr(table), L.ptr(acc), table.shape[0],
            table.shape[1], L.ptr(plan.unique_rows), L.ptr(grad_rows), L.ptr(plan.n_unique), plan.M, t_lr, t_eps, t_wd,
            L.ptr(t_hp_dev), L.stream(dev)), "tt_adam_rowwise_adagrad_fused_step")


def _fill(arr, tensors):
    for i, t in enumerate(tensors):
        arr[i] = t.data_ptr() if t is not None else 0


def tower_params_struct(din, h0, kcat_e, hidden, d_out, w_proj, b_proj, ws, bs, bn_w, bn_b, bn_rm, bn_rv, w_out, b_out,
                        bn_nbt=(), compute_dtype=TT_F32, x_dtype=TT_F32, dx_dtype=TT_F32, flags=0, w_proj_bf16=None, w_bf16=()):
    if len(hidden) > L.TT_MAX_HIDDEN:
        raise ValueError(f"at most {L.TT_MAX_HIDDEN} hidden blocks per tower are supported")
    p = L.TowerParams()
    p.din, p.h0, p.kcat_e, p.n_hidden, p.d_out = din, h0, kcat_e, len(hidden), d_out
    for i, h in enumerate(hidden):
        p.hidden[i] = h
    p.w_proj, p.b_proj, p.w_out, p.b_out = w_proj.data_ptr(), b_proj.data_ptr(), w_out.data_ptr(), b_out.data_ptr()
    _fill(p.w, ws); _fill(p.b, bs); _fill(p.bn_w, bn_w); _fill(p.bn_b, bn_b); _fill(p.bn_rm, bn_rm); _fill(p.bn_rv, bn_rv)
    _fill(p.bn_nbt, bn_nbt)
    p.compute_dtype, p.x_dtype, p.dx_dtype, p.flags = compute_dtype, x_dtype, dx_dtype, flags
    p.w_proj_bf16 = w_proj_bf16.data_ptr() if w_proj_bf16 is not None else 0
    _fill(p.w_bf16, w_bf16)
    return p


def adam_hparams(step, lr, b1, b2, eps, wd):
    out = (L.f32 * 6)()
    L.load().tt_adam_hparams(step, lr, b1, b2, eps, wd, C.byref(out))
    return list(out)


def tower_workspace(params, B, dev):
    nb = L.load().tt_tower_workspace_bytes(C.byref(params), B)
    return L.workspace(dev, nb)


def tower_fwd(params, acts, B, train, p_drop, seed, dev, seed_dev=None):
    ws = tower_workspace(params, B, dev)
    with _timed("tt_tower_mlp_fwd"):
        L.check(L.load().tt_tower_mlp_fwd(L.ctx(dev), C.byref(params), C.byref(acts), B, int(train), p_drop, seed, L.ptr(seed_dev), L.ptr(ws),
                                          ws.numel(), L.stream(dev)), "tt_tower_mlp_fwd")


def tower_bwd(params, acts, d_emb, grads, B, train, p_drop, seed, dev, seed_dev=None):
    ws = tower_workspace(params, B, dev)
    with _timed("tt_tower_mlp_bwd"):
        L.check(L.load().tt_tower_mlp_bwd(L.ctx(dev), C.byref(params), C.byref(acts), L.ptr(d_emb), C.byref(grads), B,
                                          int(train), p_drop, seed, L.ptr(seed_dev), L.ptr(ws), ws.numel(), L.stream(dev)), "tt_tower_mlp_bwd")


def _tower_workspaces(params_list, B, dev):
    lib = L.load()
    sizes = [(lib.tt_tower_workspace_bytes(C.byref(p), B) + 255) // 256 * 256 for p in params_list]
    buf = L.workspace(dev, sum(sizes))
    ptrs, off = (L.vp * len(sizes))(), 0
    for i, z in enumerate(sizes):
        ptrs[i] = buf.data_ptr() + off
        off += z
    return buf, ptrs, (L.sz * len(sizes))(*sizes)


def towers_fwd(params_list, acts_list, B, train, p_drop, seed, dev, seed_dev=None):
    n = len(params_list)
    _, wptrs, wsizes = _tower_workspaces(params_list, B, dev)
    P = (C.POINTER(L.TowerParams) * n)(*[C.pointer(p) for p in params_list])
    A = (C.POINTER(L.TowerActs) * n)(*[C.pointer(a) for a in acts_list])
    with _timed("tt_towers_mlp_fwd"):
        L.check(L.load().tt_towers_mlp_fwd(L.ctx(dev), n, P, A, B, int(train), p_drop, seed, L.ptr(seed_dev), wptrs, wsizes,
                                           L.stream(dev)), "tt_towers_mlp_fwd")


def towers_bwd(params_list, acts_list, d_embs, grads_list, B, train, p_drop, seed, dev, seed_dev=None):
    n = len(params_list)
    _, wptrs, wsizes = _tower_workspaces(params_list, B, dev)
    P = (C.POINTER(L.TowerParams) * n)(*[C.pointer(p) for p in params_list])
    A = (C.POINTER(L.TowerActs) * n)(*[C.pointer(a) for a in acts_list])
    G = (C.POINTER(L.TowerGrads) * n)(*[C.pointer(g) for g in grads_list])
    D = (L.vp * n)(*[d.data_ptr() for d in d_embs])
    with _timed("tt_towers_mlp_bwd"):
        L.check(L.load().tt_towers_mlp_bwd(L.ctx(dev), n, P, A, D, G, B, int(train), p_drop, seed, L.ptr(seed_dev), wptrs, wsizes,
                                           L.stream(dev)), "tt_towers_mlp_bwd")


def score_dir_fwd(A, Bm, inv_t, shift, diag_offset=0, want_sumscore=True):
    dev, Ra, Rb, D = A.device, A.shape[0], Bm.shape[0], A.shape[1]
    f = torch.empty((3, Ra), dtype=torch.float32, device=dev)
    rank = torch.empty(Ra, dtype=torch.int32, device=dev)
    with _timed("tt_score_dir_fwd"):
        L.check(L.load().tt_score_dir_fwd(L.ctx(dev), L.ptr(A), L.ptr(Bm), Ra, Rb, D, inv_t, shift, diag_offset, L.ptr(f[0]),
                                          L.ptr(f[1]), L.ptr(rank), L.ptr(f[2]) if want_sumscore else None, L.stream(dev)),
                "tt_score_dir_fwd")
    return f[0], f[1], rank, f[2]


def score_loss_finish(B, shift, rowsum, colsum, diag, row_rank, col_rank, sumscore):
    dev = rowsum.device
    out = torch.empty(8, dtype=torch.float32, device=dev)
    loss = torch.empty((), dtype=torch.float32, device=dev)
    with _timed("tt_score_loss_finish"):
        L.check(L.load().tt_score_loss_finish(L.ctx(dev), B, shift, L.ptr(rowsum), L.ptr(colsum), L.ptr(diag), L.ptr(row_rank),
                                              L.ptr(col_rank), L.ptr(sumscore), L.ptr(out), L.ptr(loss), L.stream(dev)),
                "tt_score_loss_finish")
    return out, loss


def score_dir_bwd(A, Bm, inv_t, shift, diag_offset, sumexp_a, sumexp_b, d_loss, scale):
    dev, Ra, Rb, D = A.device, A.shape[0], Bm.shape[0], A.shape[1]
    dA = torch.empty_like(A)
    with _timed("tt_score_dir_bwd"):
        L.check(L.load().tt_score_dir_bwd(L.ctx(dev), L.ptr(A), L.ptr(Bm), Ra, Rb, D, inv_t, shift, diag_offset, L.ptr(sumexp_a),
                                          L.ptr(sumexp_b), L.ptr(d_loss), scale, L.ptr(dA), L.stream(dev)), "tt_score_dir_bwd")
    return dA


def score_pack_bf16(X, scale: float = 1.0):
    dev, R, D = X.device, X.shape[0], X.shape[1]
    lib = L.load()
    buf = torch.empty(lib.tt_score_pack_bytes(R, D), dtype=torch.uint8, device=dev)
    with _timed("tt_score_pack_bf16"):
        L.check(lib.tt_score_pack_bf16(L.ctx(dev), L.ptr(X), R, D, scale, L.ptr(buf), L.stream(dev)), "tt_score_pack_bf16")
    return buf


def score_unit_scale(inv_t: float) -> float:
    return float(L.load().tt_score_unit_scale(inv_t))


def score_pack2_bf16(X0, X1, scale0: float = 1.0, scale1: float = 1.0):
    dev, D = X0.device, X0.shape[1]
    lib = L.load()
    b0 = torch.empty(lib.tt_score_pack_bytes(X0.shape[0], D), dtype=torch.uint8, device=dev)
    b1 = torch.empty(lib.tt_score_pack_bytes(X1.shape[0], D), dtype=torch.uint8, device=dev)
    with _timed("tt_score_pack_bf16"):
        L.check(lib.tt_score_pack2_bf16(L.ctx(dev), L.ptr(X0), X0.shape[0], L.ptr(b0), L.ptr(X1), X1.shape[0], L.ptr(b1), D,
                                        scale0, scale1, L.stream(dev)), "tt_score_pack2_bf16")
    return b0, b1


def score_pack2_bf16x3(X0, X1, scale0: float = 1.0, scale1: float = 1.0):
    dev, D = X0.device, X0.shape[1]
    lib = L.load()
# ... 418 lines not shown
```

Before: 35.38 million.

## Fuse sparse embedding gradient reduce with row-wise Adam table update

Defers the sparse embedding-gradient segment reduction until the optimizer step, then runs a combined entry point whose seg-reduce kernel applies Adam to the table, m and v rows for short segments right after summing each chunk. The later fused Adam kernel skips those already-updated rows, so the pass that re-reads grad_rows and the table state goes away. The cost is a more tangled backward/optimizer schedule: the optimizer step now runs inside the slab-defer window, and the gradient is still written out for the long-segment finish. The path is gated by a new table_tail option and only applies with Adam and no exchange.

```diff
diff --git a/include/twotower.h b/include/twotower.h
--- a/include/twotower.h
+++ b/include/twotower.h
@@ -42,6 +42,7 @@
 #define TT_OPT_LOOKUP_NT 7
 #define TT_OPT_CHAIN_SPIN 8
 #define TT_OPT_RETRIEVE_SPLITS 9
+#define TT_OPT_TABLE_TAIL 10
 int tt_ctx_set_option(tt_ctx* ctx, int32_t option, int32_t value);
 #define TT_DEVERR_CHAIN_TIMEOUT 1u
 #define TT_DEVERR_ROW_RANGE 2u
@@ -141,6 +142,13 @@
                               int64_t M, const int32_t* seg_offsets, void* grad_workspace, size_t grad_workspace_bytes,
                               int64_t step, float lr, float beta1, float beta2, float eps, float weight_decay,
                               const float* hparams_dev, tt_stream stream);
+
+int tt_embed_grad_adam_step(tt_ctx* ctx, const tt_grad_src* srcs, int32_t n_srcs, int64_t B, int32_t E,
+                            const int32_t* sorted_src, const int32_t* seg_offsets, const int32_t* unique_rows,
+                            const int32_t* n_unique, int64_t M, float* grad_rows, void* grad_workspace,
+                            size_t grad_workspace_bytes, const tt_adam_tensor* tensors, int32_t n_tensors, float* table,
+                            float* m, float* v, int64_t table_rows, int64_t step, float lr, float beta1, float beta2,
+                            float eps, float weight_decay, const float* hparams_dev, tt_stream stream);
 
 int tt_rowwise_adagrad_sparse_step(tt_ctx* ctx, float* table, float* sum, int64_t table_rows, int32_t E,
                                    const int32_t* unique_rows, const float* grad_rows, const int32_t* n_unique, int64_t M,
diff --git a/jodalrob-twotower_amd/_lib.py b/jodalrob-twotower_amd/_lib.py
--- a/jodalrob-twotower_amd/_lib.py
+++ b/jodalrob-twotower_amd/_lib.py
@@ -110,6 +110,8 @@
                                      f32, vp, vp]),
     "tt_adam_fused_step_finish": (C.c_int, [vp, C.POINTER(AdamTensor), i32, vp, vp, vp, i64, i32, vp, vp, vp, i64, vp, vp, sz, i64, f32,
                                             f32, f32, f32, f32, vp, vp]),
+    "tt_embed_grad_adam_step": (C.c_int, [vp, C.POINTER(GradSrc), i32, i64, i32, vp, vp, vp, vp, i64, vp, vp, sz, C.POINTER(AdamTensor),
+                                          i32, vp, vp, vp, i64, i64, f32, f32, f32, f32, f32, vp, vp]),
     "tt_rowwise_adagrad_sparse_step": (C.c_int, [vp, vp, vp, i64, i32, vp, vp, vp, i64, f32, f32, f32, vp, vp]),
     "tt_rowwise_adagrad_dense_step": (C.c_int, [vp, vp, vp, vp, i64, i32, f32, f32, f32, vp, vp]),
     "tt_adam_rowwise_adagrad_fused_step": (C.c_int, [vp, C.POINTER(AdamTensor), i32, i64, f32, f32, f32, f32, f32, vp, vp, vp, i64, i32,
@@ -242,6 +244,7 @@
 TT_OPT_LOOKUP_NT = 7
 TT_OPT_CHAIN_SPIN = 8
 TT_OPT_RETRIEVE_SPLITS = 9
+TT_OPT_TABLE_TAIL = 10
 
 
 def set_option(device: torch.device, option: int, value: int):
diff --git a/jodalrob-twotower_amd/cat_embed.py b/jodalrob-twotower_amd/cat_embed.py
--- a/jodalrob-twotower_amd/cat_embed.py
+++ b/jodalrob-twotower_amd/cat_embed.py
@@ -24,6 +24,7 @@
         self.grad: Optional[torch.Tensor] = None
         self.sparse_grad = None
         self.defer_long_finish = False
+        self.defer_grad_reduce = False
         self.members: List["CategoricalEmbedder"] = []
         self.version = 0
         self._grad_counters = None
@@ -117,7 +118,7 @@
         if self.grad_mode == "sparse":
             grad_rows = torch.empty((max(plan.M, 1), self.E), dtype=torch.float32, device=self.device)
             ops.embed_grad(plan, srcs, B, self.E, ops.TT_GRAD_SPARSE, grad_rows, short_segments, self.grad_counters(),
-                           defer_finish=self.defer_long_finish)
+                           defer_finish=self.defer_long_finish, defer_reduce=self.defer_grad_reduce)
             self.sparse_grad = (plan, grad_rows)
             return
         params = self.optim_parameters()
diff --git a/jodalrob-twotower_amd/csrc/tt_common.h b/jodalrob-twotower_amd/csrc/tt_common.h
--- a/jodalrob-twotower_amd/csrc/tt_common.h
+++ b/jodalrob-twotower_amd/csrc/tt_common.h
@@ -29,6 +29,7 @@
   int chain_spin;
   int retrieve_splits;
   int lookup_nt;
+  int table_tail;
   void* ho_exec;
   void* ho_node;
   void* ho_last;
diff --git a/jodalrob-twotower_amd/csrc/tt_ctx.hip b/jodalrob-twotower_amd/csrc/tt_ctx.hip
--- a/jodalrob-twotower_amd/csrc/tt_ctx.hip
+++ b/jodalrob-twotower_amd/csrc/tt_ctx.hip
@@ -80,6 +80,7 @@
   c->chained = 1;
   c->chain_spin = 1 << 22;
   c->retrieve_splits = 0;
+  c->table_tail = 1;
   c->dev_err = nullptr;
   c->ho_exec = c->ho_node = c->ho_last = nullptr;
   {
@@ -129,6 +130,7 @@
     case TT_OPT_FP8_GRAD: ctx->fp8_grad = value != 0; break;
     case TT_OPT_CHAINED: ctx->chained = value != 0; break;
     case TT_OPT_LOOKUP_NT: ctx->lookup_nt = value != 0; break;
+    case TT_OPT_TABLE_TAIL: ctx->table_tail = value != 0; break;
     case TT_OPT_CHAIN_SPIN:
       TT_CHECK_ARG(value >= 1, "tt_ctx_set_option: TT_OPT_CHAIN_SPIN needs a value >= 1");
       ctx->chain_spin = value;
diff --git a/jodalrob-twotower_amd/csrc/tt_embed.hip b/jodalrob-twotower_amd/csrc/tt_embed.hip
--- a/jodalrob-twotower_amd/csrc/tt_embed.hip
+++ b/jodalrob-twotower_amd/csrc/tt_embed.hip
@@ -846,6 +846,46 @@
   }
 };
 
+struct AdamK {
+  float lr_over_bc1, inv_sqrt_bc2, b1, b2, eps, wd;
+  const float* dev;
+};
+
+__device__ __forceinline__ AdamK adam_resolve(const AdamK& k) {
+  if (k.dev == nullptr) return k;
+  AdamK r;
+  r.lr_over_bc1 = k.dev[0]; r.inv_sqrt_bc2 = k.dev[1]; r.b1 = k.dev[2]; r.b2 = k.dev[3]; r.eps = k.dev[4]; r.wd = k.dev[5];
+  r.dev = nullptr;
+  return r;
+}
+
+__device__ __forceinline__ void adam1(float& p, float g, float& m, float& v, const AdamK& k) {
+  g = k.wd != 0.f ? __builtin_fmaf(k.wd, p, g) : g;
+  m = __builtin_fmaf(k.b1, m, (1.f - k.b1) * g);
+  v = __builtin_fmaf(k.b2, v, (1.f - k.b2) * g * g);
+  const float denom = __builtin_fmaf(sqrtf(v), k.inv_sqrt_bc2, k.eps);
+  p = __builtin_fmaf(-k.lr_over_bc1, m / denom, p);
+}
+
+struct RowAdam {
+  float* table;
+  float* m;
+  float* v;
+  int64_t table_rows;
+  AdamK k;
+};
+
+template <int VEC>
+__device__ __forceinline__ void load_row(const float* __restrict__ base, int64_t row, int32_t E, uint32_t chunk, Acc<VEC>& r) {
+  const float* p = base + row * E + chunk * VEC;
+  if (VEC == 4) {
+    const float4 t = *reinterpret_cast<const float4*>(p);
+    r.v[0] = t.x; r.v[1 % VEC] = t.y; r.v[2 % VEC] = t.z; r.v[3 % VEC] = t.w;
+  } else {
+    r.v[0] = p[0];
+  }
+}
+
 template <int VEC, int ESZ>
 __device__ __forceinline__ const char* grad_addr(const SideSet& a, uint32_t slot, uint32_t chunk) {
   const char* base = a.s[0].out;
@@ -1008,17 +1048,43 @@
   }
 }
 
-template <int VEC, int DT, int LGT>
+template <int VEC, int DT, int LGT, bool ADAM = false>
 __device__ __forceinline__ void seg_reduce_body(const SideSet& a, const int32_t* __restrict__ sorted_src,
                                                 const int32_t* __restrict__ seg, const int32_t* __restrict__ unique_rows,
                                                 const int32_t* __restrict__ n_unique, int32_t mode,
                                                 float* __restrict__ out, const GradWs& ws, uint32_t LG, bool all_short, bool planned,
-                                                uint32_t bid, uint32_t nblocks) {
+                                                uint32_t bid, uint32_t nblocks, const RowAdam& ra = RowAdam{}) {
   const uint32_t U = (uint32_t)*n_unique;
   const uint32_t gthread = bid * blockDim.x + threadIdx.x;
   const uint32_t lig = gthread % LG;
   const uint32_t ngroups = nblocks * blockDim.x / LG;
+  AdamK k{};
+  if (ADAM) k = adam_resolve(ra.k);
   for (uint32_t u = gthread / LG; u < U; u += ngroups) {
+    if (ADAM) {
+      const int32_t s0 = seg[u], s1 = seg[u + 1];
+      if (s1 - s0 > kLongSeg) continue;
+      const int64_t row = unique_rows[u];
+      const bool live = row < ra.table_rows;
+      for (uint32_t chunk = lig; chunk < a.C; chunk += LG) {
+        Acc<VEC> acc;
+        acc.zero();
+        sum_range<VEC, DT, LGT>(a, sorted_src, s0, s1, chunk, lig, acc);
+        write_row<VEC>(out, (int64_t)u, a.E, chunk, acc, false);
+        if (live) {
+          Acc<VEC> w, m, v;
+          load_row<VEC>(ra.table, row, a.E, chunk, w);
+          load_row<VEC>(ra.m, row, a.E, chunk, m);
+          load_row<VEC>(ra.v, row, a.E, chunk, v);
+#pragma unroll
+          for (int e = 0; e < VEC; ++e) adam1(w.v[e], acc.v[e], m.v[e], v.v[e], k);
+          write_row<VEC>(ra.table, row, a.E, chunk, w, false);
+          write_row<VEC>(ra.m, row, a.E, chunk, m, false);
+          write_row<VEC>(ra.v, row, a.E, chunk, v, false);
+        }
+      }
+      continue;
+    }
     const int32_t s0 = seg[u], s1 = seg[u + 1];
     if (planned && s1 - s0 > kLongSeg) continue;
     if (!all_short && s1 - s0 > kLongSeg) {
@@ -1105,12 +1171,13 @@
 #else
 #define TT_SEG_OCC
 #endif
-template <int VEC, int DT, int LGT>
+template <int VEC, int DT, int LGT, bool ADAM>
 __global__ __launch_bounds__(kSegThreads) TT_SEG_OCC void seg_reduce_chunk_slab_kernel(SideSet a, const int32_t* __restrict__ sorted_src,
                                                                         const int32_t* __restrict__ seg, const int32_t* __restrict__ unique_rows,
                                                                         const int32_t* __restrict__ n_unique, int32_t mode,
                                                                         float* __restrict__ out, GradWs ws, uint32_t LG, uint32_t g1,
-                                                                        SlabBatch sb, uint32_t nsx, uint32_t n_items, uint32_t ns) {
+                                                                        SlabBatch sb, uint32_t nsx, uint32_t n_items, uint32_t ns,
+                                                                        RowAdam ra) {
   const uint32_t g2 = gridDim.x - g1 - ns;
   const uint32_t gc = g2 < kChunkFirst ? g2 : kChunkFirst;
 #ifndef TT_SEG_LAYOUT
@@ -1127,7 +1194,7 @@
   b -= gc;
   if (b < r1) {
     TT_SEG_STAMP(0, 1);
-    seg_reduce_body<VEC, DT, LGT>(a, sorted_src, seg, unique_rows, n_unique, mode, out, ws, LG, false, true, b, g1);
+    seg_reduce_body<VEC, DT, LGT, ADAM>(a, sorted_src, seg, unique_rows, n_unique, mode, out, ws, LG, false, true, b, g1, ra);
     TT_SEG_STAMP(1, 1);
     return;
   }
@@ -1142,7 +1209,7 @@
   b -= ns;
   if (b < g1 - r1) {
     TT_SEG_STAMP(0, 1);
-    seg_reduce_body<VEC, DT, LGT>(a, sorted_src, seg, unique_rows, n_unique, mode, out, ws, LG, false, true, r1 + b, g1);
+    seg_reduce_body<VEC, DT, LGT, ADAM>(a, sorted_src, seg, unique_rows, n_unique, mode, out, ws, LG, false, true, r1 + b, g1, ra);
     TT_SEG_STAMP(1, 1);
     return;
   }
@@ -1212,27 +1279,6 @@
     float* o = out + orow * E + col;
     *o = mode == TT_GRAD_DENSE_ACC ? *o + tot : tot;
   });
-}
-
-struct AdamK {
-  float lr_over_bc1, inv_sqrt_bc2, b1, b2, eps, wd;
-  const float* dev;
-};
-
-__device__ __forceinline__ AdamK adam_resolve(const AdamK& k) {
-  if (k.dev == nullptr) return k;
-  AdamK r;
-  r.lr_over_bc1 = k.dev[0]; r.inv_sqrt_bc2 = k.dev[1]; r.b1 = k.dev[2]; r.b2 = k.dev[3]; r.eps = k.dev[4]; r.wd = k.dev[5];
-  r.dev = nullptr;
-  return r;
-}
-
-__device__ __forceinline__ void adam1(float& p, float g, float& m, float& v, const AdamK& k) {
-  g = k.wd != 0.f ? __builtin_fmaf(k.wd, p, g) : g;
-  m = __builtin_fmaf(k.b1, m, (1.f - k.b1) * g);
-  v = __builtin_fmaf(k.b2, v, (1.f - k.b2) * g * g);
-  const float denom = __builtin_fmaf(sqrtf(v), k.inv_sqrt_bc2, k.eps);
-  p = __builtin_fmaf(-k.lr_over_bc1, m / denom, p);
 }
 
 __global__ __launch_bounds__(kThreads) void adam_dense_kernel(float* __restrict__ p, const float* __restrict__ g,
@@ -2346,9 +2392,10 @@
 
 size_t tt_embed_grad_workspace_bytes(int64_t M, int32_t E) { return grad_layout(nullptr, M > 0 ? M : 1, E > 0 ? E : 1).bytes; }
 
-int tt_embed_grad_bwd(tt_ctx* ctx, const tt_grad_src* srcs, int32_t n_srcs, int64_t B, int32_t E, const int32_t* sorted_src,
-                      const int32_t* seg_offsets, const int32_t* unique_rows, const int32_t* n_unique, int64_t M, int32_t mode,
-                      float* out, int32_t* counters, void* workspace, size_t workspace_bytes, tt_stream stream) {
+static int embed_grad_bwd_impl(tt_ctx* ctx, const tt_grad_src* srcs, int32_t n_srcs, int64_t B, int32_t E, const int32_t* sorted_src,
+                               const int32_t* seg_offsets, const int32_t* unique_rows, const int32_t* n_unique, int64_t M, int32_t mode,
+                               float* out, int32_t* counters, void* workspace, size_t workspace_bytes, tt_stream stream,
+                               const RowAdam* ra) {
   TT_CHECK_ARG(ctx && srcs && out, "tt_embed_grad_bwd: NULL argument");
   TT_CHECK_ARG(n_srcs >= 1 && n_srcs <= TT_MAX_SIDES, "tt_embed_grad_bwd: n_srcs=%d", n_srcs);
   const bool all_short = (mode & TT_GRAD_SHORT_SEGMENTS) != 0;
@@ -2356,6 +2403,7 @@
   const bool defer = (mode & TT_GRAD_DEFER_FINISH) != 0;
   mode &= ~(TT_GRAD_SHORT_SEGMENTS | TT_GRAD_PLANNED | TT_GRAD_DEFER_FINISH);
   TT_CHECK_ARG(!defer || (planned && mode == TT_GRAD_SPARSE), "tt_embed_grad_bwd: TT_GRAD_DEFER_FINISH needs TT_GRAD_PLANNED | TT_GRAD_SPARSE");
+  TT_CHECK_ARG(!ra || defer, "tt_embed_grad_bwd: the row Adam needs TT_GRAD_PLANNED | TT_GRAD_SPARSE | TT_GRAD_DEFER_FINISH");
   TT_CHECK_ARG(mode >= TT_GRAD_SPARSE && mode <= TT_GRAD_DENSE_ACC, "tt_embed_grad_bwd: bad mode %d", mode);
   TT_CHECK_ARG(E >= 1 && B >= 0, "tt_embed_grad_bwd: bad E/B");
   if (M == 0) return TT_OK;
@@ -2367,7 +2415,7 @@
   SideSet a{};
   a.n = n_srcs;
   a.E = E;
-  bool vec4 = (E % 4 == 0) && tt_aligned(out, 16);
+  bool vec4 = (E % 4 == 0) && tt_aligned(out, 16) && (!ra || (tt_aligned(ra->table, 16) && tt_aligned(ra->m, 16) && tt_aligned(ra->v, 16)));
   int64_t slots = 0;
   for (int i = 0; i < n_srcs; ++i) {
     const tt_grad_src& s = srcs[i];
@@ -2407,18 +2455,24 @@
     tt_set_error("tt_embed_grad_bwd: E=%d too wide for the long-row finish (max %d)", E, kFinishMaxFloats * (int)LG / kThreads);
     return TT_ERR_UNSUPPORTED;
   }
+  const SlabBatch no_slabs{};
+  const RowAdam rad = ra ? *ra : RowAdam{};
+#define TT_SEG_SLAB_ARGS                                                                                                        \
+  a, sorted_src, seg_offsets, unique_rows, n_unique, mode, out, gl.ws, LG, (uint32_t)g1s, slabs ? slabs->sb : no_slabs,         \
+      (uint32_t)nsxs, (uint32_t)(slabs ? slabs->n : 0), (uint32_t)nss, rad
 #define TT_SEG_LAUNCH(V, D, G)                                                                                                  \
   do {                                                                                                                          \
-    if (planned && slabs) {                                                                                                     \
+    if (planned && (slabs || ra)) {                                                                                             \
       const int sc = kSegThreads / kThreads;                                                                                  \
-      const int g1s = (int)tt_cdiv(g1, sc), g2s = (int)tt_cdiv(g2, sc), nsxs = (int)tt_cdiv(nsx, sc);                           \
-      const int nss = tt_slab_role_blocks(slabs, nsxs);                                                                         \
-      seg_reduce_chunk_slab_kernel<V, D, G><<<nss + g1s + g2s, kSegThreads, 0, st>>>(                                           \
-          a, sorted_src, seg_offsets, unique_rows, n_unique, mode, out, gl.ws, LG, (uint32_t)g1s, slabs->sb, (uint32_t)nsxs,    \
-          (uint32_t)slabs->n, (uint32_t)nss);                                                                                   \
+      const int g1s = (int)tt_cdiv(g1, sc), g2s = (int)tt_cdiv(g2, sc), nsxs = slabs ? (int)tt_cdiv(nsx, sc) : 0;               \
+      const int nss = slabs ? tt_slab_role_blocks(slabs, nsxs) : 0;                                                             \
+      if (ra) seg_reduce_chunk_slab_kernel<V, D, G, true><<<nss + g1s + g2s, kSegThreads, 0, st>>>(TT_SEG_SLAB_ARGS);           \
+      else seg_reduce_chunk_slab_kernel<V, D, G, false><<<nss + g1s + g2s, kSegThreads, 0, st>>>(TT_SEG_SLAB_ARGS);             \
       TT_LAUNCH_CHECK();                                                                                                        \
-      slabs->n = 0;                                                                                                             \
-      slabs->maxtotal = 1;                                                                                                      \
+      if (slabs) {                                                                                                              \
+        slabs->n = 0;                                                                                                           \
+        slabs->maxtotal = 1;                                                                                                    \
+      }                                                                                                                         \
       if (!defer) seg_long_finish_kernel<V><<<g3, kThreads, 0, st>>>(E, a.C, seg_offsets, unique_rows, mode, out, gl.ws, LG);   \
       break;                                                                                                                    \
     }                                                                                                                           \
@@ -2451,8 +2505,16 @@
   else TT_SEG_LAUNCH(1, TT_BF16, 0);
 #undef TT_SEG_LAUNCH_G
 #undef TT_SEG_LAUNCH
+#undef TT_SEG_SLAB_ARGS
   TT_LAUNCH_CHECK();
   return TT_OK;
+}
+
+int tt_embed_grad_bwd(tt_ctx* ctx, const tt_grad_src* srcs, int32_t n_srcs, int64_t B, int32_t E, const int32_t* sorted_src,
+                      const int32_t* seg_offsets, const int32_t* unique_rows, const int32_t* n_unique, int64_t M, int32_t mode,
+                      float* out, int32_t* counters, void* workspace, size_t workspace_bytes, tt_stream stream) {
+  return embed_grad_bwd_impl(ctx, srcs, n_srcs, B, E, sorted_src, seg_offsets, unique_rows, n_unique, M, mode, out, counters, workspace,
+                             workspace_bytes, stream, nullptr);
 }
 
 void tt_adam_hparams(int64_t step, float lr, float beta1, float beta2, float eps, float weight_decay, float out6[6]) {
@@ -2533,7 +2595,7 @@
                            int64_t table_rows, int32_t E, const int32_t* unique_rows, float* grad_rows, const int32_t* n_unique, int64_t M,
                            const int32_t* seg_offsets, void* grad_workspace, size_t grad_workspace_bytes, int64_t step, float lr,
                            float beta1, float beta2, float eps, float weight_decay, const float* hparams_dev, tt_stream stream,
-                           const char* who) {
+                           const char* who, bool rows_done = false) {
   if (int rc = tt_riders_flush(ctx, reinterpret_cast<hipStream_t>(stream))) return rc;
   if (ctx && ctx->deferred && ctx->deferred->n > 0)
     if (int rc = tt_gemm_deferred_flush(ctx, reinterpret_cast<hipStream_t>(stream))) return rc;
@@ -2569,7 +2631,7 @@
     }
     const GradLayout gl = grad_layout(reinterpret_cast<char*>(grad_workspace), M, E);
     const int nlb = (int)(gl.max_long < (int64_t)ctx->num_cus * 8 ? gl.max_long : (int64_t)ctx->num_cus * 8);
-    const int grid = nd + nlb + grid_for(ctx, M * LG);
+    const int grid = nd + nlb + (rows_done ? 0 : grid_for(ctx, M * LG));
     if (vec4) adam_fused_kernel<4, true><<<grid, kThreads, 0, st>>>(a, table, m, v, E, C, unique_rows, grad_rows, n_unique, k, LG, table_rows, seg_offsets, gl.ws, nlb);
     else adam_fused_kernel<1, true><<<grid, kThreads, 0, st>>>(a, table, m, v, E, C, unique_rows, grad_rows, n_unique, k, LG, table_rows, seg_offsets, gl.ws, nlb);
     TT_LAUNCH_CHECK();
@@ -2599,6 +2661,25 @@
   return adam_fused_impl(ctx, tensors, n_tensors, table, m, v, table_rows, E, unique_rows, grad_rows, n_unique, M, seg_offsets,
                          grad_workspace, grad_workspace_bytes, step, lr, beta1, beta2, eps, weight_decay, hparams_dev, stream,
                          "tt_adam_fused_step_finish");
+}
+
+int tt_embed_grad_adam_step(tt_ctx* ctx, const tt_grad_src* srcs, int32_t n_srcs, int64_t B, int32_t E, const int32_t* sorted_src,
+                            const int32_t* seg_offsets, const int32_t* unique_rows, const int32_t* n_unique, int64_t M, float* grad_rows,
+                            void* grad_workspace, size_t grad_workspace_bytes, const tt_adam_tensor* tensors, int32_t n_tensors,
+                            float* table, float* m, float* v, int64_t table_rows, int64_t step, float lr, float beta1, float beta2,
+                            float eps, float weight_decay, const float* hparams_dev, tt_stream stream) {
+  const char* who = "tt_embed_grad_adam_step";
+  TT_CHECK_ARG(ctx && table && m && v && grad_workspace, "%s: NULL argument", who);
+  TT_CHECK_ARG(tensors && n_tensors >= 1 && n_tensors <= kAdamMulti, "%s: n_tensors=%d not in [1,%d]", who, n_tensors, kAdamMulti);
+  TT_CHECK_ARG(step >= 1 && E >= 1 && M >= 1 && table_rows >= 1, "%s: bad step/E/M/table_rows", who);
+  const int32_t mode = TT_GRAD_SPARSE | TT_GRAD_PLANNED | TT_GRAD_DEFER_FINISH;
+  RowAdam ra{table, m, v, table_rows, make_adam(step, lr, beta1, beta2, eps, weight_decay, hparams_dev)};
+  if (int rc = embed_grad_bwd_impl(ctx, srcs, n_srcs, B, E, sorted_src, seg_offsets, unique_rows, n_unique, M, mode, grad_rows, nullptr,
+                                   grad_workspace, grad_workspace_bytes, stream, ctx->table_tail ? &ra : nullptr))
+    return rc;
+  return adam_fused_impl(ctx, tensors, n_tensors, table, m, v, table_rows, E, unique_rows, grad_rows, n_unique, M, seg_offsets,
+                         grad_workspace, grad_workspace_bytes, step, lr, beta1, beta2, eps, weight_decay, hparams_dev, stream, who,
+                         ctx->table_tail != 0);
 }
 
 static AdagradK make_adagrad(float lr, float eps, float wd, const float* dev) {
diff --git a/jodalrob-twotower_amd/graph.py b/jodalrob-twotower_amd/graph.py
--- a/jodalrob-twotower_amd/graph.py
+++ b/jodalrob-twotower_amd/graph.py
@@ -173,10 +173,12 @@
         self.opt.zero_grad(set_to_none=True)
         defer = self._defer_long
         stores = list(getattr(self.opt, "_stores", ()))
+        ex = getattr(self.task, "exchange", None)
         for st in stores:
             st.defer_long_finish = defer
+            g = self.opt._group_of_store(st)
+            st.defer_grad_reduce = defer and ex is None and g is not None and g.get("table_optimizer", "adam") == "adam"
         dev = self._dev.device
-        ex = getattr(self.task, "exchange", None)
         slabs = self._defer_slabs
         riders = self._defer_riders and self._ingest is not None and (ex is None or not getattr(self.task, "sync_bn", False))
         for t, _, sh in self._shadows:
@@ -190,10 +192,10 @@
                 L.set_defer_slab_reduce(dev, True)
             try:
                 loss.backward(self._ones)
+                self.opt.step()
             finally:
                 if slabs:
                     L.set_defer_slab_reduce(dev, False)
-            self.opt.step()
             for st in stores:
                 if st.sparse_grad is not None:
                     ops.embed_grad_finish(st.sparse_grad[0])
@@ -206,6 +208,7 @@
                 L.set_defer_riders(dev, False)
             for st in stores:
                 st.defer_long_finish = False
+                st.defer_grad_reduce = False
         return res
 
     def _eager_once(self):
diff --git a/jodalrob-twotower_amd/ops.py b/jodalrob-twotower_amd/ops.py
--- a/jodalrob-twotower_amd/ops.py
+++ b/jodalrob-twotower_amd/ops.py
@@ -166,6 +166,7 @@
     staging: object = None
     grad_ws: object = None
     finish_deferred: object = None
+    reduce_deferred: object = None
 
 
 def dedup_plan(rows: torch.Tensor, table_rows: int) -> DedupPlan:
@@ -229,7 +230,7 @@
 
 
 def embed_grad(plan: DedupPlan, srcs: Sequence[tuple], B: int, E: int, mode: int, out: torch.Tensor, short_segments: bool = False,
-               counters: Optional[torch.Tensor] = None, defer_finish: bool = False):
+               counters: Optional[torch.Tensor] = None, defer_finish: bool = False, defer_reduce: bool = False):
     if short_segments:
         mode |= L.TT_GRAD_SHORT_SEGMENTS
     dev = out.device
@@ -246,17 +247,38 @@
     else:
         ws = L.workspace(dev, nb)
         deferred = False
+    plan.finish_deferred = out if deferred else None
+    if deferred and defer_reduce:
+        plan.reduce_deferred = (arr, [d for d, _ in srcs], B, E)
+        return
+    plan.reduce_deferred = None
     with _timed("tt_embed_grad_bwd"):
         L.check(lib.tt_embed_grad_bwd(L.ctx(dev), arr, len(srcs), B, E, L.ptr(plan.sorted_src), L.ptr(plan.seg_offsets),
                                       L.ptr(plan.unique_rows), L.ptr(plan.n_unique), plan.M, mode, L.ptr(out),
                                       L.ptr(counters), L.ptr(ws), ws.numel(), L.stream(dev)), "tt_embed_grad_bwd")
-    plan.finish_deferred = out if deferred else None
+
+
+def run_deferred_reduce(plan: DedupPlan):
+    rd = plan.reduce_deferred
+    if rd is None:
+        return
+    arr, srcs, B, E = rd
+    out = plan.finish_deferred
+    ws = plan.grad_ws[0]
+    dev = out.device
+    mode = L.TT_GRAD_SPARSE | L.TT_GRAD_PLANNED | L.TT_GRAD_DEFER_FINISH
+    with _timed("tt_embed_grad_bwd"):
+        L.check(L.load().tt_embed_grad_bwd(L.ctx(dev), arr, len(srcs), B, E, L.ptr(plan.sorted_src), L.ptr(plan.seg_offsets),
+                                           L.ptr(plan.unique_rows), L.ptr(plan.n_unique), plan.M, mode, L.ptr(out), None,
+                                           L.ptr(ws), ws.numel(), L.stream(dev)), "tt_embed_grad_bwd")
+    plan.reduce_deferred = None
 
 
 def embed_grad_finish(plan: DedupPlan):
     out = plan.finish_deferred
     if out is None:
         return
+    run_deferred_reduce(plan)
     ws, E = plan.grad_ws
     dev = out.device
     with _timed("tt_embed_grad_finish"):
@@ -302,6 +324,16 @@
         if plan.finish_deferred.data_ptr() != grad_rows.data_ptr():
             raise RuntimeError("adam_fused: the plan's deferred gradient is not the one handed to the optimiser")
         ws, E = plan.grad_ws
+        if plan.reduce_deferred is not None:
+            garr, srcs, B, _ = plan.reduce_deferred
+            with _timed("tt_embed_grad_adam_step"):
+                L.check(L.load().tt_embed_grad_adam_step(
+                    L.ctx(dev), garr, len(srcs), B, E, L.ptr(plan.sorted_src), L.ptr(plan.seg_offsets), L.ptr(plan.unique_rows),
+                    L.ptr(plan.n_unique), plan.M, L.ptr(grad_rows), L.ptr(ws), ws.numel(), arr, len(items), L.ptr(table), L.ptr(m),
+                    L.ptr(v), table.shape[0], step, lr, b1, b2, eps, wd, L.ptr(hp_dev), L.stream(dev)), "tt_embed_grad_adam_step")
+            plan.reduce_deferred = None
+            plan.finish_deferred = None
+            return
         with _timed("tt_adam_fused_step"):
             L.check(L.load().tt_adam_fused_step_finish(L.ctx(dev), arr, len(items), L.ptr(table), L.ptr(m), L.ptr(v), table.shape[0],
                                                        table.shape[1], L.ptr(plan.unique_rows), L.ptr(grad_rows), L.ptr(plan.n_unique),
@@ -340,6 +372,7 @@
     if plan.finish_deferred is not None:
         if plan.finish_deferred.data_ptr() != grad_rows.data_ptr():
             raise RuntimeError("adam_rowwise_adagrad_fused: the plan's deferred gradient is not the one handed to the optimiser")
+        run_deferred_reduce(plan)
         ws, E = plan.grad_ws
         with _timed("tt_adam_rowwise_adagrad_fused_step"):
             L.check(L.load().tt_adam_rowwise_adagrad_fused_step_finish(
```

After: 35.45 million, median of 6. No clear change (+0.2%).
